# wangqiaoli/geometric_mapping

Measured on AMD Instinct MI355X. Metric: points/sec full segment+fit, 1M-pt synthetic tunnel frame, higher is better.
Workload: dtype f32; 1 GPU; 1000000-pt synthetic tunnel frame (R=2 m, L=12 m, sigma=0.01), rows resident in HBM; k_regime=fixed-k (~256 neighbours), mode=frames, frames_in_flight=4, GPU_MAX_HW_QUEUES=4, ransac_model=cylinder, H=1024, tau=0.03 (extension), parallelism=framesx1

## Files before the change

geometric_mapping_amd/_lib.py:

```python
from __future__ import annotations

import ctypes as C
import importlib.util
import os
import re

_HERE = os.path.dirname(os.path.abspath(__file__))
LIB_PATH = os.path.join(_HERE, "libgm_hip.so")
if os.environ.get("GM_LIB_PATH"):
    LIB_PATH = os.environ["GM_LIB_PATH"]
HEADER_PATH = os.path.join(os.path.dirname(_HERE), "include", "gm_hip.h")

GM_OK = 0
GM_ERR_INVALID_ARG = 1
GM_ERR_TOO_FEW_POINTS = 2
GM_ERR_DEVICE = 3
GM_ERR_OOM = 4
GM_ERR_CAPACITY = 5
GM_ERR_NOT_READY = 6
GM_ERR_UNSUPPORTED = 7
GM_ERR_COMM = 8
GM_GROUP_LOOPBACK = 1
GM_GROUP_N_TIMINGS = 5

# ... 236 lines not shown
    return C.CDLL(path, mode=C.RTLD_GLOBAL)


def load():
    global _lib
    if _lib is not None:
        return _lib
    _preload_hip_runtime()
    if not os.path.exists(LIB_PATH):
        raise FileNotFoundError(
            f"{LIB_PATH} is missing: build it with `python -c 'import __graft_entry__ as g; g.build()'` "
            "(make -C geometric_mapping_amd/csrc).  There is no CPU fallback.")
    L = C.CDLL(LIB_PATH)
    vp, u32, u32p, fp, dp, i32p, u8p = (C.c_void_p, C.c_uint32, C.POINTER(C.c_uint32), C.POINTER(C.c_float),
                                         C.POINTER(C.c_double), C.POINTER(C.c_int32), C.POINTER(C.c_uint8))
    cfgp, cloudp, resp = C.POINTER(Config), C.POINTER(Cloud), C.POINTER(FrameResult)
    fitp = C.POINTER(CylinderFit)
    sprmp, scellp, sinfop = C.POINTER(SurfaceParams), C.POINTER(SurfaceCell), C.POINTER(SurfaceInfo)
    wprmp, wrawp, waddp, winfop = C.POINTER(WallParams), C.POINTER(WallRawCell), C.POINTER(WallAddInfo), C.POINTER(WallInfo)
    u64, u64p = C.c_uint64, C.POINTER(C.c_uint64)
    wregp, wrprmp, wrinfop, wrmetp = (C.POINTER(WallRegion), C.POINTER(WallRegionParams), C.POINTER(WallRegionsInfo),
                                      C.POINTER(WallRegionMetrics))
    wcprmp, wcptp, wcinfop = C.POINTER(WallCloudParams), C.POINTER(WallCloudPoint), C.POINTER(WallCloudInfo)
    wkprmp, wkptp, wkinfop = C.POINTER(WallCheckParams), C.POINTER(WallCheckPoint), C.POINTER(WallCheckInfo)
    woprmp, wobjp, woinfop, wometp = (C.POINTER(WallObjectParams), C.POINTER(WallObject), C.POINTER(WallObjectsInfo),
                                      C.POINTER(WallObjectMetrics))
    proto = {
        "gm_create": (C.c_int, [cfgp, C.POINTER(vp)]),
        "gm_destroy": (None, [vp]),
        "gm_default_config": (None, [cfgp]),
        "gm_host_alloc": (C.c_int, [vp, C.c_size_t, C.POINTER(vp)]),
        "gm_host_free": (C.c_int, [vp, vp]),
        "gm_host_register": (C.c_int, [vp, vp, C.c_size_t]),
        "gm_host_unregister": (C.c_int, [vp, vp]),
        "gm_abi_version": (u32, []),
        "gm_debug_live_buffers": (C.c_longlong, []),
        "gm_status_string": (C.c_char_p, [C.c_int]),
        "gm_last_error": (C.c_char_p, [vp]),
        "gm_process_frame": (C.c_int, [vp, cloudp, resp]),
        "gm_submit_frame": (C.c_int, [vp, u32, cloudp]),
        "gm_wait_frame": (C.c_int, [vp, u32, resp]),
        "gm_poll_frame": (C.c_int, [vp, u32]),
        "gm_set_cloud_output": (C.c_int, [vp, u32, fp, u32]),
        "gm_get_cropped_xyz": (C.c_int, [vp, u32, fp, u32, u32p]),
        "gm_get_normals": (C.c_int, [vp, u32, fp, u32, u32p]),
        "gm_get_voxel_centroids": (C.c_int, [vp, u32, fp, u32, u32p]),
        "gm_get_voxel_nearest": (C.c_int, [vp, u32, i32p, u32, u32p]),
        "gm_get_voxel_normals": (C.c_int, [vp, u32, fp, u32, u32p]),
        "gm_get_neighbor_counts": (C.c_int, [vp, u32, i32p, u32, u32p]),
        "gm_get_labels": (C.c_int, [vp, u32, u8p, u32, u32p]),
        "gm_chop_cloud": (C.c_int, [vp, cloudp, C.c_double, fp, u32, u32p]),
        "gm_get_normals_stage": (C.c_int, [vp, fp, u32, C.c_double, fp, fp, u32, u32p]),
        "gm_get_local_frame": (C.c_int, [vp, fp, u32, C.c_double, fp, fp, dp]),
        "gm_voxel_grid": (C.c_int, [vp, fp, u32, C.c_double, fp, u32, u32p, u32p]),
        "gm_nearest": (C.c_int, [vp, fp, u32, fp, u32, i32p]),
        "gm_solve_local_frame": (C.c_int, [dp, fp, fp]),
        "gm_set_owned_range": (C.c_int, [vp, C.c_double, C.c_double]),
        "gm_ext_available": (C.c_int, []),
        "gm_score_frame": (C.c_int, [vp, u32, C.c_int, fp, u32, C.c_double, u32, i32p]),
        "gm_score_planes": (C.c_int, [vp, fp, u32, u8p, u32, fp, u32, C.c_double, i32p]),
        "gm_score_cylinders": (C.c_int, [vp, fp, u32, u8p, u32, fp, u32, C.c_double, i32p]),
        "gm_plane_hypotheses": (C.c_int, [vp, fp, u32, u8p, u32, C.c_uint64, u32, fp]),
        "gm_cylinder_hypotheses": (C.c_int, [vp, fp, fp, u32, u8p, u32, C.c_uint64, u32, fp]),
        "gm_segment_moments": (C.c_int, [vp, fp, fp, u8p, u32, u32, dp]),
        "gm_get_compressed_map": (C.c_int, [vp, u32, vp, C.c_size_t, C.POINTER(C.c_size_t)]),
        "gm_get_cylinder_fit": (C.c_int, [vp, u32, fitp]),
        "gm_fit_cylinder": (C.c_int, [vp, fp, u32, u8p, u32, fp, C.c_double, fitp, u8p]),
        "gm_surface_default_params": (None, [sprmp]),
        "gm_set_surface_params": (C.c_int, [vp, sprmp]),
        "gm_get_surface_map": (C.c_int, [vp, u32, sinfop, scellp, u32, u32p]),
        "gm_get_surface_points": (C.c_int, [vp, u32, fp, i32p, u32, u32p]),
        "gm_surface_map": (C.c_int, [vp, fp, u32, u8p, fp, sprmp, sinfop, scellp, u32, fp, i32p]),
        "gm_wall_default_params": (None, [wprmp]),
        "gm_wall_map_create": (C.c_int, [vp, wprmp, C.POINTER(vp)]),
        "gm_wall_map_destroy": (None, [vp]),
        "gm_wall_map_add_frame": (C.c_int, [vp, vp, u32, dp, waddp]),
        "gm_wall_map_add_points": (C.c_int, [vp, fp, u32, u8p, dp, waddp, fp, i32p]),
        "gm_wall_map_sync": (C.c_int, [vp]),
        "gm_wall_map_info": (C.c_int, [vp, winfop]),
        "gm_wall_map_read": (C.c_int, [vp, u32, u32, scellp, u64, u64p]),
        "gm_wall_map_read_raw": (C.c_int, [vp, u32, u32, wrawp, u64, u64p]),
        "gm_wall_map_add_raw": (C.c_int, [vp, u32, u32, wrawp]),
        "gm_wall_map_clear": (C.c_int, [vp, u32, u32]),
        "gm_wall_region_default_params": (None, [wrprmp]),
        "gm_wall_map_regions": (C.c_int, [vp, vp, u32, u32, wrprmp, wrinfop, wregp, u32, u32p, i32p]),
        "gm_wall_region_metrics": (C.c_int, [wprmp, wregp, wrmetp]),
        "gm_wall_cloud_default_params": (None, [wcprmp]),
        "gm_wall_cloud_directions": (C.c_int, [wprmp, wcprmp, dp, u32, u32p]),
        "gm_wall_map_cloud": (C.c_int, [vp, u32, u32, wcprmp, wcinfop, wcptp, u64, u64p]),
        "gm_wall_check_default_params": (None, [wkprmp]),
        "gm_wall_check_classify": (C.c_int, [wkprmp, wrawp, C.c_float, C.POINTER(C.c_int64), u32p]),
        "gm_wall_map_check_frame": (C.c_int, [vp, vp, u32, dp, wkprmp, waddp]),
        "gm_wall_map_get_check": (C.c_int, [vp, u32, wkinfop, wkptp, u32, u32p]),
        "gm_wall_map_check_points": (C.c_int, [vp, fp, u32, u8p, dp, wkprmp, waddp, wkinfop, wkptp, u32, u32p, fp, i32p, i32p, u8p]),
        "gm_wall_object_default_params": (None, [woprmp]),
        "gm_wall_map_check_objects": (C.c_int, [vp, u32, woprmp, woinfop, wobjp, u32, u32p, i32p, u32]),
        "gm_wall_check_objects": (C.c_int, [vp, wkptp, u32, C.c_int64, woprmp, woinfop, wobjp, u32, u32p, i32p]),
        "gm_wall_object_metrics": (C.c_int, [wprmp, woprmp, wobjp, wometp]),
        "gm_group_create": (C.c_int, [cfgp, i32p, u32, u32, C.POINTER(vp)]),
        "gm_group_destroy": (None, [vp]),
        "gm_group_size": (u32, [vp]),
        "gm_group_ctx": (vp, [vp, u32]),
        "gm_group_last_error": (C.c_char_p, [vp]),
        "gm_group_process_frame": (C.c_int, [vp, cloudp, resp]),
        "gm_group_get_cropped_xyz": (C.c_int, [vp, fp, u32, u32p]),
        "gm_group_get_voxel_centroids": (C.c_int, [vp, fp, u32, u32p]),
# ... 20 lines not shown
```

geometric_mapping_amd/api.py:

```python
from __future__ import annotations

import ctypes as C

import numpy as np

from . import _lib
from ._lib import (GM_CFG_CYLINDER_FIT, GM_CFG_DEFAULT, GM_CFG_KEEP_COUNTS, GM_CFG_STAGE_TIMING, GM_CFG_VOXEL_GRID,
                   GM_CLOUD_BIGENDIAN, GM_CLOUD_DEVICE, GM_CLOUD_PINNED, GM_ERR_CAPACITY, GM_ERR_NOT_READY, GM_OK, Cloud, Config,
                   CylinderFit, FrameResult, GmError, STAGE_NAMES)

__all__ = ["GeometricMapping", "GeometricMappingGroup", "WallMap", "GmError", "solve_local_frame", "decode_compressed_map",
           "GM_CFG_CYLINDER_FIT"]


def _f32(a):
    return a.ctypes.data_as(C.POINTER(C.c_float))


class GeometricMapping:

    def __init__(self, boxFilterBound=5.0, voxelGridLeafSize=0.5, neighborRadius=0.5, weightingFactor=0.2,
                 device=0, flags=GM_CFG_DEFAULT, n_slots=1, max_points=0,
                 ransac_hypotheses=1024, ransac_threshold=0.03, ransac_seed=1):
        self._L = _lib.load()
# ... 182 lines not shown

    def labels(self, slot=0):
        return self._fetch(self._L.gm_get_labels, slot, 1, np.uint8)

    def compressed_map(self, slot=0):
        n = C.c_size_t(0)
        st = self._L.gm_get_compressed_map(self._ctx, slot, None, 0, C.byref(n))
        if st not in (GM_OK, GM_ERR_CAPACITY):
            self._check(st)
        buf = np.zeros(n.value, dtype=np.uint8)
        self._check(self._L.gm_get_compressed_map(self._ctx, slot, buf.ctypes.data, n.value, C.byref(n)))
        return buf

    def set_owned_range(self, lo, hi):
        self._check(self._L.gm_set_owned_range(self._ctx, float(lo), float(hi)))

    def chopCloud(self, bound, cloud):
        c, keep = self._as_cloud(cloud)
        cap = max(c.n_points, 1)
        out = np.empty((cap, 4), dtype=np.float32)
        n = C.c_uint32(0)
        self._check(self._L.gm_chop_cloud(self._ctx, C.byref(c), float(bound), _f32(out), cap, C.byref(n)))
        out = out[:n.value]
        return out[:, :3].copy(), out[:, 3].copy().view(np.int32)

    def getNormals(self, neighborRadius, cloud):
        xyz = np.ascontiguousarray(cloud, dtype=np.float32)
        if xyz.ndim != 2 or xyz.shape[1] != 3:
            raise ValueError("cloud must be [n,3]")
        n0 = xyz.shape[0]
        cap = max(n0, 1)
        oc = np.empty((cap, 4), dtype=np.float32)
        on = np.empty((cap, 4), dtype=np.float32)
        n = C.c_uint32(0)
        self._check(self._L.gm_get_normals_stage(self._ctx, _f32(xyz), n0, float(neighborRadius), _f32(oc), _f32(on),
                                                 cap, C.byref(n)))
        oc, on = oc[:n.value], on[:n.value]
        return on.copy(), oc[:, :3].copy(), oc[:, 3].copy().view(np.int32)

    def getLocalFrame(self, cloudSize, weightingFactor, cloud_normals):
        nrm = np.ascontiguousarray(cloud_normals, dtype=np.float32)
        if nrm.ndim != 2 or nrm.shape[1] != 4:
            raise ValueError("normals must be [n,4] (nx,ny,nz,curvature)")
        if cloudSize > nrm.shape[0]:
            raise ValueError("cloudSize exceeds the normals cloud (the reference's .at() would throw)")
        ev = np.zeros(3, dtype=np.float32)
        V = np.zeros(9, dtype=np.float32)
        sc = np.zeros(6, dtype=np.float64)
        self._check(self._L.gm_get_local_frame(self._ctx, _f32(nrm), int(cloudSize), float(weightingFactor), _f32(ev),
                                               _f32(V), sc.ctypes.data_as(C.POINTER(C.c_double))))
        M = np.array([[sc[0], sc[1], sc[2]], [sc[1], sc[3], sc[4]], [sc[2], sc[4], sc[5]]])
        return ev, V.reshape(3, 3).T.copy(), M

    def voxelGrid(self, leafSize, cloud):
        xyz = np.ascontiguousarray(cloud, dtype=np.float32)
        if xyz.ndim != 2 or xyz.shape[1] != 3:
            raise ValueError("cloud must be [n,3]")
        cap = max(xyz.shape[0], 1)
        out = np.empty((cap, 4), dtype=np.float32)
        n = C.c_uint32(0)
        fl = C.c_uint32(0)
        self._check(self._L.gm_voxel_grid(self._ctx, _f32(xyz), xyz.shape[0], float(leafSize), _f32(out), cap,
                                          C.byref(n), C.byref(fl)))
        out = out[:n.value]
        return out[:, :3].copy(), out[:, 3].astype(np.int32), bool(fl.value & _lib.GM_RES_VOXEL_PASSTHROUGH)


    @staticmethod
    def _u8(a):
        if a is None:
            return None, None
        a = np.ascontiguousarray(a, dtype=np.uint8)
        return a, a.ctypes.data_as(C.POINTER(C.c_uint8))

    def nearest(self, cloud, queries):
        xyz = np.ascontiguousarray(cloud, dtype=np.float32)
        q = np.ascontiguousarray(queries, dtype=np.float32)
        idx = np.empty(max(len(q), 1), dtype=np.int32)
        self._check(self._L.gm_nearest(self._ctx, _f32(xyz), len(xyz), _f32(q), len(q),
                                       idx.ctypes.data_as(C.POINTER(C.c_int32))))
        return idx[:len(q)].copy()

    def plane_hypotheses(self, cloud, seed, H, labels=None, want=0):
        xyz = np.ascontiguousarray(cloud, dtype=np.float32)
        lab, lp = self._u8(labels)
        out = np.empty((H, 4), dtype=np.float32)
        self._check(self._L.gm_plane_hypotheses(self._ctx, _f32(xyz), len(xyz), lp, want, seed, H, _f32(out)))
        return out

    def cylinder_hypotheses(self, cloud, normals, seed, H, labels=None, want=0):
        xyz = np.ascontiguousarray(cloud, dtype=np.float32)
        nrm = np.ascontiguousarray(normals, dtype=np.float32)
        lab, lp = self._u8(labels)
        out = np.empty((H, 7), dtype=np.float32)
        self._check(self._L.gm_cylinder_hypotheses(self._ctx, _f32(xyz), _f32(nrm), len(xyz), lp, want, seed, H, _f32(out)))
        return out

    def _score(self, fn, cloud, hyp, tau, labels, want):
        xyz = np.ascontiguousarray(cloud, dtype=np.float32)
        hyp = np.ascontiguousarray(hyp, dtype=np.float32)
        lab, lp = self._u8(labels)
        cnt = np.zeros(len(hyp), dtype=np.int32)
        self._check(fn(self._ctx, _f32(xyz), len(xyz), lp, want, _f32(hyp), len(hyp), float(tau),
                       cnt.ctypes.data_as(C.POINTER(C.c_int32))))
        return cnt

# ... 693 lines not shown
```

geometric_mapping_amd/csrc/gm_api.hip:

```cpp
#include <math.h>
#include <stdlib.h>
#include <string.h>

#include <limits>
#include <new>

#include "gm_compact.hpp"
#include "gm_internal.hpp"

using namespace gm;

namespace {

thread_local std::string g_create_err;

#define GM_HIP(ctx, call)                                                                 \
    do {                                                                                  \
        hipError_t e__ = (call);                                                          \
        if (e__ != hipSuccess) {                                                          \
            (ctx)->err = std::string(#call) + ": " + hipGetErrorString(e__);              \
            return (e__ == hipErrorOutOfMemory) ? GM_ERR_OOM : GM_ERR_DEVICE;             \
        }                                                                                 \
    } while (0)

// ... 104 lines not shown
    const double dim = b - a + 1.0;
    if (std::isfinite(dim) && dim >= 1.0 && dim * dim * dim <= (double)kVoxDenseMaxCells && fabs(a) < 1e9) {
        vd.enabled = 1;
        vd.i_lo = (int32_t)a;
        vd.dim = (int32_t)dim;
        const double ext = fmax((double)hi - (double)lo, 1e-30);
        int k = (int)floor(log2(9.0e18 / (ext * 268435456.0)));
        if (k > 40) k = 40;
        if (k < 8 || n_cap > 268435456u) { vd.enabled = 0; k = 0; }
        vd.scale = ldexp(1.0, k);
        vd.inv_scale = ldexp(1.0, -k);
    }
    return vd;
}

int bits_for(uint64_t count)
{
    int b = 1;
    while ((1ull << b) < count && b < 32) ++b;
    return b;
}

int voxel_key_bits(double lo, double hi, double leaf)
{
    const float inv = 1.0f / (float)leaf;
    double d = floor((double)((float)hi * inv)) - floor((double)((float)lo * inv)) + 2.0;
    if (!(d > 0) || !std::isfinite(d)) return 32;
    double prod = d * d * d;
    if (prod > 2147483647.0) return 32;
    return bits_for((uint64_t)prod);
}

gm_status ensure_capacity(gm_ctx *ctx, Slot &sl, uint32_t n, size_t raw_bytes, bool need_raw)
{
    uint32_t *gen = &sl.alloc_gen;
    if (need_raw && raw_bytes > sl.raw_cap) {
        const size_t cap = raw_bytes + raw_bytes / 4 + 4096;
        sl.raw_cap = 0;
        GM_HIP(ctx, sl.h_raw.reserve(cap));
        GM_HIP(ctx, sl.d_raw.reserve(cap));
        sl.raw_cap = cap;
    }
    if (n <= sl.cap) return GM_OK;
    GM_HIP(ctx, hipStreamSynchronize(sl.stream));
    uint32_t cap = n + n / 4 + 1024;
    if (cap < ctx->cfg.max_points) cap = ctx->cfg.max_points;
    cap = (cap + 3u) & ~3u;
    sl.cap = 0;
    GM_HIP(ctx, sl.crop4.reserve(cap, gen));
    GM_HIP(ctx, sl.keys_a.reserve(cap, gen)); GM_HIP(ctx, sl.keys_b.reserve(cap, gen));
    GM_HIP(ctx, sl.vals_a.reserve(cap, gen)); GM_HIP(ctx, sl.vals_b.reserve(cap, gen));
    GM_HIP(ctx, sl.spts4.reserve(cap, gen)); GM_HIP(ctx, sl.normals4.reserve(cap, gen));
    GM_HIP(ctx, sl.counts.reserve(cap, gen));
    GM_HIP(ctx, sl.valid4.reserve(cap, gen)); GM_HIP(ctx, sl.vnorm4.reserve(cap, gen));
    GM_HIP(ctx, sl.seg_start.reserve(cap, gen)); GM_HIP(ctx, sl.vox4.reserve(cap, gen));
    GM_HIP(ctx, sl.vox_nn.reserve(cap, gen)); GM_HIP(ctx, sl.labels.reserve(cap, gen)); GM_HIP(ctx, sl.inl_mask.reserve(cap, gen));
    sl.tiles_cap = cap + 2u;
    sl.tile_seg = cap / 2u + 2u;
    GM_HIP(ctx, sl.tiles.reserve((size_t)(kTileListClasses - 1) * sl.tile_seg + sl.tiles_cap, gen));
    GM_HIP(ctx, sl.row_bounds.reserve((size_t)1024 * 1024, gen));
    sl.blk_cap = compact_records(cap > kVoxDenseMaxCells ? cap : kVoxDenseMaxCells) + 1;
    GM_HIP(ctx, sl.tile_partials.reserve((size_t)compact_blocks(cap) * 6, gen));
    GM_HIP(ctx, sl.blk.reserve((size_t)sl.blk_cap + 1, gen));
    GM_HIP(ctx, hipMemsetAsync(sl.blk, 0, sizeof(unsigned long long) * ((size_t)sl.blk_cap + 1), sl.stream));
    {
        static const char *e = getenv("GM_TEST_SCAN_EPOCH");
        sl.scan_epoch = e ? (uint32_t)strtoul(e, nullptr, 0) : 0u;
    }
    GM_HIP(ctx, sl.sort.totals.reserve(radix_totals_bytes() / sizeof(uint32_t), gen));
    sl.sort.rec_words = (radix_record_words_max(cap) + 1u) & ~(size_t)1u;
    GM_HIP(ctx, sl.sort.rec.reserve(sl.sort.rec_words, gen));
    GM_HIP(ctx, sl.sort.ticket.reserve(4, gen));
    GM_HIP(ctx, hipMemsetAsync(sl.sort.ticket, 0, 16, sl.stream));
    sl.tile_rec_words = (size_t)(tile_cutter_blocks(cap) + 1) * (size_t)kTileListClasses;
    GM_HIP(ctx, sl.tile_rec.reserve(sl.tile_rec_words, gen));
    GM_HIP(ctx, hipMemsetAsync(sl.tile_rec, 0, sizeof(unsigned long long) * sl.tile_rec_words, sl.stream));
    sl.cap = cap;
    return GM_OK;
}

gm_status check_layout(gm_ctx *ctx, const gm_cloud *c)
{
    const uint64_t step = c->point_step;
    if (c->n_points && (step < 12 || (uint64_t)c->off_x + 4 > step || (uint64_t)c->off_y + 4 > step ||
                        (uint64_t)c->off_z + 4 > step))
        return fail(ctx, GM_ERR_INVALID_ARG, "gm_cloud: x/y/z offsets do not fit in point_step");
    return GM_OK;
}

gm_status make_rows(gm_ctx *ctx, const gm_cloud *c, const uint8_t *dev_data, RowLayout &rows)
{
    const gm_status lst = check_layout(ctx, c);
    if (lst != GM_OK) return lst;
    memset(&rows, 0, sizeof(rows));
    rows.data = dev_data;
    rows.step = c->point_step; rows.ox = c->off_x; rows.oy = c->off_y; rows.oz = c->off_z;
    rows.bswap = (c->flags & GM_CLOUD_BIGENDIAN) ? 1u : 0u;
    const bool al4 = ((c->point_step | c->off_x | c->off_y | c->off_z) & 3u) == 0 && (((uintptr_t)dev_data) & 3u) == 0;
    const bool al16 = al4 && c->point_step == 16 && c->off_x == 0 && c->off_y == 4 && c->off_z == 8 &&
                      (((uintptr_t)dev_data) & 15u) == 0;
    rows.mode = al16 ? 0u : (al4 ? 1u : 2u);
    return GM_OK;
}

void record(gm_ctx *ctx, Slot &sl, int idx)
{
    if (ctx->cfg.flags & GM_CFG_STAGE_TIMING) hipEventRecord(sl.ev[idx], sl.stream);
}

gm_status reset_counters(gm_ctx *ctx, Slot &sl)
{
    GM_HIP(ctx, hipMemsetAsync(sl.ctr, 0, sizeof(DevCounters), sl.stream));
    return GM_OK;
}

// ... 12 lines not shown
    return hipSuccess;
}

static uint32_t size_bucket(uint32_t n)
{
    if (n == 0) return 0;
    uint32_t p2 = 1024;
    while (p2 < n && p2 < 0x80000000u) p2 <<= 1;
    const uint32_t step = p2 / 16 < 1024u ? 1024u : p2 / 16;
    const uint64_t b = ((uint64_t)n + step - 1) / step * step;
    return b > 0xFFFFFFFFull ? 0xFFFFFFFFu : (uint32_t)b;
}

static gm_status enqueue_launches(gm_ctx *ctx, Slot &sl, const RowLayout &rows, uint32_t n, uint32_t ns, const GridParams &g,
                                  const VoxDense &vd, float lo, float hi)
{
    const gm_config &cf = ctx->cfg;
    hipStream_t s = sl.stream;
    const uint32_t *n_dev = nullptr;
    if (sl.capturing) {
        sl.scan_seq = 0;
        GM_HIP(ctx, hipMemcpyAsync(sl.frame_in, sl.h_frame_in, 4 * sizeof(uint32_t), hipMemcpyHostToDevice, s));
        n_dev = sl.frame_in;
    }
    {
        ZeroJobs z;
        memset(&z, 0, sizeof(z));
        z.ptr[0] = sl.ctr; z.words8[0] = sizeof(DevCounters) / 8;
        if (vd.enabled) { z.ptr[1] = sl.vox_table; z.words8[1] = (uint64_t)vd.dim * vd.dim * vd.dim * sizeof(VoxCell) / 8; }
        if (sl.row_bounds) { z.ptr[2] = sl.row_bounds; z.words8[2] = (uint64_t)g.ny * (uint64_t)g.nz; }
        if (sl.sort.totals) {
            z.ptr[3] = sl.sort.totals; z.words8[3] = radix_totals_bytes() / 8;
            z.ptr[4] = sl.sort.rec; z.words8[4] = (radix_record_words(ns, cell_key_bits(g)) + 1) / 2;
        }
        z.frame_counter = sl.frame_in + 4;
        launch_zero_fill(z, s);
    }
    launch_crop(rows, n, lo, hi, g, sl, s, ns, n_dev, true);
    const bool cloud_overlap = sl.cloud_out && n && !sl.capturing && sl.cloud_out_dev;
    if (cloud_overlap) {
        GM_HIP(ctx, hipEventRecord(sl.ev_crop, s));
        GM_HIP(ctx, hipStreamWaitEvent(sl.copy_stream, sl.ev_crop, 0));
        GM_HIP(ctx, hipMemcpyAsync(sl.cloud_out, sl.crop4, (size_t)n * sizeof(float4), hipMemcpyDeviceToHost, sl.copy_stream));
    }
    record(ctx, sl, 2);
    launch_grid_and_normals(g, vd, sl, ns, (cf.flags & GM_CFG_KEEP_COUNTS) != 0, true, s);
    record(ctx, sl, 3);
    uint32_t row_tile = kCpTile;
    const uint32_t nparts = launch_compact_valid(sl, ns, cf.weightingFactor, s, &row_tile);
    bool cloud_copy_pending = false;
    if (cloud_overlap) {
        GM_HIP(ctx, hipEventRecord(sl.ev_valid, s));
        GM_HIP(ctx, hipStreamWaitEvent(sl.copy_stream, sl.ev_valid, 0));
        launch_rows_to_host(sl.valid4, sl.cloud_out_dev, &sl.ctr->first_drop_enc, &sl.ctr->n_valid, sl.copy_stream);
        GM_HIP(ctx, hipEventRecord(sl.ev_copied, sl.copy_stream));
        cloud_copy_pending = true;
    } else if (sl.cloud_out && n) {
        const size_t frozen = (size_t)(ns < sl.cloud_out_cap ? ns : sl.cloud_out_cap) * sizeof(float4);
        GM_HIP(ctx, hipMemcpyAsync(sl.cloud_out, sl.valid4, frozen, hipMemcpyDeviceToHost, s));
    }
    record(ctx, sl, 4);
    record(ctx, sl, 5);
    sl.vox_sort_path = (cf.flags & GM_CFG_VOXEL_GRID) && !vd.enabled;
    if (cf.flags & GM_CFG_VOXEL_GRID) {
        if (vd.enabled) {
            launch_voxel_dense_finalize(vd, sl, s);
        } else {
            launch_minmax(sl.valid4, &sl.ctr->n_valid, ns, sl.ctr, s);
            launch_voxel_grid(sl, ns, (float)cf.voxelGridLeafSize, voxel_key_bits(lo, hi, cf.voxelGridLeafSize), s);
        }
    }
    record(ctx, sl, 6);
    if (cf.flags & (GM_CFG_RANSAC_PLANE | GM_CFG_RANSAC_CYLINDER)) {
        const gm_status st = gm_enqueue_ransac(ctx, sl, ns, nparts, row_tile);
        if (st != GM_OK) return st;
    }
    if ((cf.flags & GM_CFG_NEAREST) && (cf.flags & GM_CFG_VOXEL_GRID)) {
        const uint32_t nq_cap = vd.enabled ? (uint32_t)vd.dim * vd.dim * vd.dim : ns;
        launch_nearest(sl.valid4, &sl.ctr->n_valid, ns, sl.vox4, &sl.ctr->n_voxels, nq_cap < ns ? nq_cap : ns, sl.nn_best,
                       sl.vox_nn, s, sl.vnorm4, sl.vox_nrm4);
    }
    record(ctx, sl, 7);
    if (!(cf.flags & (GM_CFG_RANSAC_PLANE | GM_CFG_RANSAC_CYLINDER)))
        launch_frame_finalize(sl.tile_partials, nparts, row_tile, sl, s);
    if (cloud_copy_pending) GM_HIP(ctx, hipStreamWaitEvent(s, sl.ev_copied, 0));
    GM_HIP(ctx, hipMemcpyAsync(sl.h_out, sl.d_out, sizeof(FrameOut), hipMemcpyDeviceToHost, s));
    return GM_OK;
}

gm_status enqueue_frame(gm_ctx *ctx, Slot &sl, const gm_cloud *cloud, bool blocking_call)
{
    const uint32_t n = cloud->n_points;
    const uint32_t ns = size_bucket(n);
    const size_t raw_bytes = (size_t)n * cloud->point_step;
    const bool on_dev = (cloud->flags & GM_CLOUD_DEVICE) != 0;
    if (n && !cloud->data) return fail(ctx, GM_ERR_INVALID_ARG, "gm_cloud.data is NULL");
    if (sl.cloud_out && n > sl.cloud_out_cap) return fail(ctx, GM_ERR_CAPACITY, "gm_set_cloud_output: the frame has more points than the cloud buffer has rows");
    gm_status st = check_layout(ctx, cloud);
    if (st != GM_OK) return st;
    st = ensure_capacity(ctx, sl, ns ? ns : 1u, raw_bytes, !on_dev);
    if (st != GM_OK) return st;
    if (ctx->cfg.flags & (GM_CFG_RANSAC_PLANE | GM_CFG_RANSAC_CYLINDER | GM_CFG_NEAREST)) {
        st = gm_ensure_ext(ctx, sl, ctx->cfg.ransac_hypotheses ? ctx->cfg.ransac_hypotheses : 1);
        if (st != GM_OK) return st;
    }
    if (ctx->cfg.flags & GM_CFG_SURFACE_MAP) {
        st = gm_ensure_surface(ctx, sl);
        if (st != GM_OK) return st;
    }
    hipStream_t s = sl.stream;
    sl.n_in = n;
    if ((++sl.frames_enqueued & 0x7FFFFFu) == 0u && sl.blk) {
        GM_HIP(ctx, hipMemsetAsync(sl.blk, 0, sizeof(unsigned long long) * (size_t)sl.blk_cap, s));
        GM_HIP(ctx, hipMemsetAsync(sl.tile_rec, 0, sizeof(unsigned long long) * sl.tile_rec_words, s));
    }
    record(ctx, sl, 0);
    const uint8_t *dev_rows = (const uint8_t *)cloud->data;
    if (!on_dev && n) {
        static const char *zc = getenv("GM_PINNED_ZERO_COPY");
        const int zmode = zc ? atoi(zc) : 0;
        void *mapped = nullptr;
        if ((cloud->flags & GM_CLOUD_PINNED) && (zmode == 2 || (zmode == 1 && blocking_call)) &&
            hipHostGetDevicePointer(&mapped, const_cast<void *>(cloud->data), 0) == hipSuccess && mapped) {
            dev_rows = (const uint8_t *)mapped;
        } else {
            (void)hipGetLastError();
            GM_HIP(ctx, upload_rows(sl, cloud, raw_bytes, blocking_call, s));
            dev_rows = sl.d_raw;
        }
    }
    record(ctx, sl, 1);
    RowLayout rows;
    st = make_rows(ctx, cloud, dev_rows, rows);
// ... 184 lines not shown
    GM_HIP(ctx, sl.score_partial.reserve(4096, gen));
    GM_HIP(ctx, sl.cnt_plane.reserve(HH, gen)); GM_HIP(ctx, sl.cnt_cyl.reserve(HH, gen));
    GM_HIP(ctx, sl.best_plane.reserve(2, gen)); GM_HIP(ctx, sl.best_cyl.reserve(2, gen));
    GM_HIP(ctx, sl.mom_partial.reserve((size_t)kScatterBlocks * 16 * 2, gen));
    GM_HIP(ctx, sl.mom_plane.reserve(16, gen)); GM_HIP(ctx, sl.mom_cyl.reserve(16, gen));
    GM_HIP(ctx, sl.nn_best.reserve(pts, gen));
    GM_HIP(ctx, sl.vox_nrm4.reserve(pts, gen));
    GM_HIP(ctx, sl.fit_partial.reserve((size_t)kFitBlocks * 24, gen)); GM_HIP(ctx, sl.fit_ticket.reserve(1, gen));
    GM_HIP(ctx, sl.fit_work.reserve(1, gen)); GM_HIP(ctx, sl.fit_init.reserve(8, gen)); GM_HIP(ctx, sl.fit_stage.reserve(1, gen));
    GM_HIP(ctx, hipMemset(sl.fit_ticket, 0, sizeof(uint32_t)));
    GM_HIP(ctx, hipMemset(sl.score_partial, 0, sizeof(uint32_t) * 4096));
    GM_HIP(ctx, hipMemset(sl.best_plane, 0xFF, 8));
    GM_HIP(ctx, hipMemset(sl.best_cyl, 0xFF, 8));
    sl.ext_H = HH; sl.ext_cap = sl.cap;
    return GM_OK;
}

gm_status gm_ensure_surface(gm_ctx *ctx, Slot &sl)
{
    uint32_t *gen = &sl.alloc_gen;
    if (!sl.surf_table) {
        GM_HIP(ctx, hipStreamSynchronize(sl.stream));
        GM_HIP(ctx, sl.surf_prm.reserve(2, gen)); GM_HIP(ctx, sl.surf_cells.reserve(GM_SURF_MAX_CELLS, gen));
        GM_HIP(ctx, sl.surf_info.reserve(1, gen)); GM_HIP(ctx, sl.surf_fit.reserve(1, gen));
        GM_HIP(ctx, hipMemsetAsync(sl.surf_info, 0, sizeof(gm_surface_info), sl.stream));
        const SurfParams prm[2] = {surface_device_params(ctx->surf), surface_device_params(ctx->surf)};
        GM_HIP(ctx, hipMemcpyAsync(sl.surf_prm, prm, sizeof(prm), hipMemcpyHostToDevice, sl.stream));
        GM_HIP(ctx, sl.surf_table.reserve(surface_table_bytes(), gen));
        GM_HIP(ctx, hipMemsetAsync(sl.surf_table, 0, surface_table_bytes(), sl.stream));
        GM_HIP(ctx, hipStreamSynchronize(sl.stream));
    }
    if (sl.surf_cap < sl.cap || !sl.surf_res) {
        GM_HIP(ctx, hipStreamSynchronize(sl.stream));
        const uint32_t pts = sl.cap ? sl.cap : 1u;
        sl.surf_cap = 0;
        GM_HIP(ctx, sl.surf_res.reserve(pts, gen)); GM_HIP(ctx, sl.surf_cell.reserve(pts, gen));
        sl.surf_cap = sl.cap;
    }
    return GM_OK;
}

gm_status gm_enqueue_ransac(gm_ctx *ctx, Slot &sl, uint32_t n_cap, uint32_t scatter_rows, uint32_t row_tile)
{
    const gm_config &cf = ctx->cfg;
    const bool do_plane = (cf.flags & GM_CFG_RANSAC_PLANE) != 0, do_cyl = (cf.flags & GM_CFG_RANSAC_CYLINDER) != 0;
    if (!do_plane && !do_cyl) return GM_OK;
    const uint32_t H = cf.ransac_hypotheses;
    hipStream_t s = sl.stream;
    const uint32_t *n_ptr = &sl.ctr->n_valid;
    bool first = true;
    uint32_t mom_rows = 0;
    if (do_plane) {
        uint8_t *lab = first ? nullptr : sl.labels;
        launch_plane_hypotheses(sl.valid4, lab, 0, n_ptr, n_cap, cf.ransac_seed, H, sl.hyp_plane, sl.cnt_plane, s);
        const uint32_t *fsel = nullptr; const int32_t *fcnt = nullptr; uint32_t fk = 0; bool fmask = false, frep = false;
        launch_score_preemptive(0, sl.valid4, lab, 0, n_ptr, n_cap, sl.hyp_plane, sl.band, H, cf.ransac_threshold,
                                sl.score_partial, sl.cnt_plane, sl.best_plane, true, &fsel, &fcnt, &fk, s, sl.inl_mask, &fmask, &frep);
        mom_rows = launch_label(0, sl.valid4, sl.labels, 0, 1, n_ptr, n_cap, sl.hyp_plane, sl.band, sl.best_plane,
                                cf.ransac_threshold, first ? 1 : 0, fsel, fcnt, fk, s, sl.vnorm4, sl.mom_partial, fmask ? sl.inl_mask : nullptr, frep);
        first = false;
    }
    if (do_cyl) {
        uint8_t *lab = first ? nullptr : sl.labels;
        launch_cylinder_hypotheses(sl.valid4, sl.vnorm4, lab, 0, n_ptr, n_cap, cf.ransac_seed + 1, H, sl.hyp_cyl,
                                   sl.cnt_cyl, sl.band, cf.ransac_threshold, s);
        const uint32_t *fsel = nullptr; const int32_t *fcnt = nullptr; uint32_t fk = 0; bool fmask = false, frep = false;
        launch_score_preemptive(1, sl.valid4, lab, 0, n_ptr, n_cap, sl.hyp_cyl, sl.band, H, cf.ransac_threshold,
                                sl.score_partial, sl.cnt_cyl, sl.best_cyl, true, &fsel, &fcnt, &fk, s, sl.inl_mask, &fmask, &frep);
        mom_rows = launch_label(1, sl.valid4, sl.labels, 0, 2, n_ptr, n_cap, sl.hyp_cyl, sl.band, sl.best_cyl,
                                cf.ransac_threshold, first ? 1 : 0, fsel, fcnt, fk, s, sl.vnorm4, sl.mom_partial, fmask ? sl.inl_mask : nullptr, frep);
        first = false;
        if (cf.flags & GM_CFG_CYLINDER_FIT) {
            CylFitArgs a;
            a.pts = sl.valid4; a.labels = sl.labels; a.out = sl.labels;
            a.want = 0; a.want2 = 2; a.mask_mode = 0;
            a.n_ptr = n_ptr; a.n_host = n_cap;
            a.init = sl.hyp_cyl; a.best = sl.best_cyl;
            a.work = sl.fit_work; a.fit = &sl.d_out->fit; a.partial = sl.fit_partial; a.ticket = sl.fit_ticket;
            a.tau = cf.ransac_threshold;
            launch_cylinder_fit(a, s);
            if (cf.flags & GM_CFG_SURFACE_MAP) {
                SurfArgs m;
                m.pts = sl.valid4; m.labels = sl.labels; m.n_ptr = n_ptr; m.n_host = n_cap;
                m.fit = &sl.d_out->fit; m.prm = sl.surf_prm;
                m.table = sl.surf_table; m.cells = sl.surf_cells; m.info = sl.surf_info; m.res = sl.surf_res; m.cell = sl.surf_cell;
                launch_surface_map(m, n_cap, s);
            }
        }
    }
    launch_ext_finalize(sl.hyp_plane, do_plane ? sl.best_plane : nullptr, sl.hyp_cyl, do_cyl ? sl.best_cyl : nullptr,
                        sl.mom_plane, sl.mom_cyl, &sl.d_out->ext, sl.mom_partial, mom_rows, s, sl.tile_partials, scatter_rows, row_tile,
                        sl.ctr, sl.voxp, sl.d_out);
    return GM_OK;
}

}

extern "C" {

int gm_debug_graph_captures(gm_ctx *ctx, uint32_t slot)
{
    if (!ctx || slot >= ctx->n_slots) return -1;
    return (int)ctx->slots[slot].graph_captures;
}

long long gm_debug_live_buffers(void) { return g_live_buffers.load(std::memory_order_relaxed); }

gm_status gm_host_alloc(gm_ctx *ctx, size_t bytes, void **out)
{
    if (!ctx || !out) return fail(ctx, GM_ERR_INVALID_ARG, "gm_host_alloc: NULL argument");
    *out = nullptr;
    if (hipSetDevice(ctx->cfg.device) != hipSuccess) return fail(ctx, GM_ERR_DEVICE, "hipSetDevice failed");
    if (hipHostMalloc(out, bytes ? bytes : 1, hipHostMallocDefault) != hipSuccess) {
        *out = nullptr;
        return fail(ctx, GM_ERR_OOM, "gm_host_alloc: hipHostMalloc failed");
    }
    return GM_OK;
}

gm_status gm_host_free(gm_ctx *ctx, void *ptr)
{
    if (!ptr) return GM_OK;
    if (hipHostFree(ptr) != hipSuccess) return fail(ctx, GM_ERR_INVALID_ARG, "gm_host_free: not a gm_host_alloc pointer");
    return GM_OK;
}

gm_status gm_host_register(gm_ctx *ctx, void *ptr, size_t bytes)
{
    if (!ctx || !ptr || !bytes) return fail(ctx, GM_ERR_INVALID_ARG, "gm_host_register: NULL argument");
    if (hipSetDevice(ctx->cfg.device) != hipSuccess) return fail(ctx, GM_ERR_DEVICE, "hipSetDevice failed");
    if (hipHostRegister(ptr, bytes, hipHostRegisterDefault) != hipSuccess) {
        (void)hipGetLastError();
        return fail(ctx, GM_ERR_INVALID_ARG, "gm_host_register: hipHostRegister failed (already registered, or not host memory)");
    }
    return GM_OK;
}
// ... 193 lines not shown
    if (!sl.submitted) return GM_ERR_NOT_READY;
    if (sl.complete) return GM_OK;
    if (hipSetDevice(ctx->device) != hipSuccess) return fail(ctx, GM_ERR_DEVICE, "hipSetDevice failed");
    const hipError_t e = hipStreamQuery(sl.stream);
    if (e == hipSuccess) return GM_OK;
    if (e == hipErrorNotReady) { (void)hipGetLastError(); return GM_ERR_NOT_READY; }
    ctx->err = std::string("hipStreamQuery: ") + hipGetErrorString(e);
    return GM_ERR_DEVICE;
}

gm_status gm_set_cloud_output(gm_ctx *ctx, uint32_t slot, float *xyzw, uint32_t capacity)
{
    if (!ctx) return GM_ERR_INVALID_ARG;
    if (slot >= ctx->n_slots) return fail(ctx, GM_ERR_INVALID_ARG, "slot out of range");
    if (hipSetDevice(ctx->device) != hipSuccess) return fail(ctx, GM_ERR_DEVICE, "hipSetDevice failed");
    Slot &sl = ctx->slots[slot];
    if (sl.submitted && !sl.complete) GM_HIP(ctx, hipStreamSynchronize(sl.stream));
    if (xyzw) {
        hipPointerAttribute_t a;
        if (hipPointerGetAttributes(&a, xyzw) != hipSuccess || a.type != hipMemoryTypeHost) {
            (void)hipGetLastError();
            return fail(ctx, GM_ERR_INVALID_ARG, "gm_set_cloud_output: the buffer must be page-locked (gm_host_alloc / gm_host_register)");
        }
    }
    if (xyzw && !sl.copy_stream) {
        GM_HIP(ctx, hipStreamCreateWithFlags(&sl.copy_stream, hipStreamNonBlocking));
        GM_HIP(ctx, hipEventCreateWithFlags(&sl.ev_crop, hipEventDisableTiming));
        GM_HIP(ctx, hipEventCreateWithFlags(&sl.ev_valid, hipEventDisableTiming));
        GM_HIP(ctx, hipEventCreateWithFlags(&sl.ev_copied, hipEventDisableTiming));
    }
    sl.cloud_out_dev = nullptr;
    if (xyzw) {
        void *dp = nullptr;
        if (hipHostGetDevicePointer(&dp, xyzw, 0) == hipSuccess) sl.cloud_out_dev = reinterpret_cast<float4 *>(dp);
        else (void)hipGetLastError();
    }
    sl.cloud_out = reinterpret_cast<float4 *>(xyzw);
    sl.cloud_out_cap = xyzw ? capacity : 0u;
    return GM_OK;
}

gm_status gm_process_frame(gm_ctx *ctx, const gm_cloud *cloud, gm_frame_result *res)
{
    gm_status st = submit(ctx, 0, cloud, true);
    if (st != GM_OK) return st;
    return gm_wait_frame(ctx, 0, res);
}

gm_status gm_get_cropped_xyz(gm_ctx *ctx, uint32_t slot, float *xyzw, uint32_t capacity, uint32_t *n_out)
{
    gm_status st = check_slot(ctx, slot);
    if (st != GM_OK) return st;
    Slot &sl = ctx->slots[slot];
    return fetch(ctx, slot, (const float4 *)sl.valid4, sl.last.n_valid, (float4 *)xyzw, capacity, n_out);
}

gm_status gm_get_normals(gm_ctx *ctx, uint32_t slot, float *nxyzc, uint32_t capacity, uint32_t *n_out)
{
    gm_status st = check_slot(ctx, slot);
    if (st != GM_OK) return st;
    Slot &sl = ctx->slots[slot];
    return fetch(ctx, slot, (const float4 *)sl.vnorm4, sl.last.n_valid, (float4 *)nxyzc, capacity, n_out);
}

gm_status gm_get_voxel_centroids(gm_ctx *ctx, uint32_t slot, float *xyzc, uint32_t capacity, uint32_t *n_out)
{
    gm_status st = check_slot(ctx, slot);
    if (st != GM_OK) return st;
    Slot &sl = ctx->slots[slot];
    if (!(ctx->cfg.flags & GM_CFG_VOXEL_GRID)) return fail(ctx, GM_ERR_NOT_READY, "context created without GM_CFG_VOXEL_GRID");
    return fetch(ctx, slot, (const float4 *)sl.vox4, sl.last.n_voxels, (float4 *)xyzc, capacity, n_out);
}

gm_status gm_get_neighbor_counts(gm_ctx *ctx, uint32_t slot, int32_t *counts, uint32_t capacity, uint32_t *n_out)
{
    gm_status st = check_slot(ctx, slot);
    if (st != GM_OK) return st;
    Slot &sl = ctx->slots[slot];
    if (!(ctx->cfg.flags & GM_CFG_KEEP_COUNTS)) return fail(ctx, GM_ERR_NOT_READY, "context created without GM_CFG_KEEP_COUNTS");
    return fetch(ctx, slot, (const int32_t *)sl.counts, sl.last.n_cropped, counts, capacity, n_out);
}


gm_status gm_chop_cloud(gm_ctx *ctx, const gm_cloud *cloud, double bound, float *xyzw_out, uint32_t capacity,
                        uint32_t *n_out)
{
    Slot *slp;
    gm_status st = begin_stage(ctx, slp);
    if (st != GM_OK) return st;
    if (!cloud) return fail(ctx, GM_ERR_INVALID_ARG, "cloud is NULL");
    if (!std::isfinite(bound) || bound < 0) return fail(ctx, GM_ERR_INVALID_ARG, "bound must be finite and >= 0");
    Slot &sl = *slp;
    const uint32_t n = cloud->n_points;
    const size_t raw_bytes = (size_t)n * cloud->point_step;
    const bool on_dev = (cloud->flags & GM_CLOUD_DEVICE) != 0;
    if (n && !cloud->data) return fail(ctx, GM_ERR_INVALID_ARG, "gm_cloud.data is NULL");
    st = check_layout(ctx, cloud);
    if (st != GM_OK) return st;
    st = ensure_capacity(ctx, sl, n ? n : 1u, raw_bytes, !on_dev);
    if (st != GM_OK) return st;
    st = reset_counters(ctx, sl);
    if (st != GM_OK) return st;
    const uint8_t *dev_rows = (const uint8_t *)cloud->data;
    if (!on_dev && n) {
        GM_HIP(ctx, upload_rows(sl, cloud, raw_bytes, true, sl.stream));
        dev_rows = sl.d_raw;
    }
    RowLayout rows;
    st = make_rows(ctx, cloud, dev_rows, rows);
    if (st != GM_OK) return st;
    const float lo = (float)(-bound), hi = (float)bound;
    const GridParams g = make_grid(lo, lo, lo, hi - lo, hi - lo, hi - lo, ctx->cfg.neighborRadius, n);
    launch_crop(rows, n, lo, hi, g, sl, sl.stream);
    uint32_t m = 0;
    GM_HIP(ctx, hipMemcpyAsync(&m, &sl.ctr->n_cropped, 4, hipMemcpyDeviceToHost, sl.stream));
    GM_HIP(ctx, hipStreamSynchronize(sl.stream));
    return fetch(ctx, 0, (const float4 *)sl.crop4, m, (float4 *)xyzw_out, capacity, n_out);
}

gm_status gm_get_normals_stage(gm_ctx *ctx, const float *xyz, uint32_t n, double radius, float *xyzw_out,
                               float *nxyzc_out, uint32_t capacity, uint32_t *n_out)
{
    Slot *slp;
    gm_status st = begin_stage(ctx, slp);
    if (st != GM_OK) return st;
    if (n && !xyz) return fail(ctx, GM_ERR_INVALID_ARG, "xyz is NULL");
    if (!radius_ok(radius)) return fail(ctx, GM_ERR_INVALID_ARG, "radius must be 0 or within [1e-15, 1e15]");
    Slot &sl = *slp;
    const size_t raw_bytes = (size_t)n * 12;
    st = ensure_capacity(ctx, sl, n, raw_bytes, true);
    if (st != GM_OK) return st;
    st = reset_counters(ctx, sl);
    if (st != GM_OK) return st;
    float mn[3] = {3e38f, 3e38f, 3e38f}, mx[3] = {-3e38f, -3e38f, -3e38f};
    for (uint32_t i = 0; i < n; ++i) {
        const float *p = xyz + 3 * (size_t)i;
        if (!(std::isfinite(p[0]) && std::isfinite(p[1]) && std::isfinite(p[2]))) continue;
        for (int k = 0; k < 3; ++k) { mn[k] = fminf(mn[k], p[k]); mx[k] = fmaxf(mx[k], p[k]); }
    }
    if (mn[0] > mx[0]) { for (int k = 0; k < 3; ++k) { mn[k] = 0; mx[k] = 0; } }
    if (n) {
        memcpy(sl.h_raw, xyz, raw_bytes);
        GM_HIP(ctx, hipMemcpyAsync(sl.d_raw, sl.h_raw, raw_bytes, hipMemcpyHostToDevice, sl.stream));
    }
    gm_cloud c = {sl.d_raw, n, 12, 0, 4, 8, GM_CLOUD_DEVICE};
    RowLayout rows;
    st = make_rows(ctx, &c, sl.d_raw, rows);
    if (st != GM_OK) return st;
    const GridParams g = make_grid(mn[0], mn[1], mn[2], mx[0] - mn[0], mx[1] - mn[1], mx[2] - mn[2], radius, n);
    const float big = std::numeric_limits<float>::max();
    launch_crop(rows, n, -big, big, g, sl, sl.stream);
    VoxDense vd_off;
    memset(&vd_off, 0, sizeof(vd_off));
    vd_off.own_lo = -std::numeric_limits<float>::infinity();
    vd_off.own_hi = std::numeric_limits<float>::infinity();
    launch_grid_and_normals(g, vd_off, sl, n, (ctx->cfg.flags & GM_CFG_KEEP_COUNTS) != 0, false, sl.stream);
    launch_compact_valid(sl, n, 1.0, sl.stream);
    uint32_t m[2] = {0, 0};
    GM_HIP(ctx, hipMemcpyAsync(m, &sl.ctr->n_cropped, 8, hipMemcpyDeviceToHost, sl.stream));
    GM_HIP(ctx, hipStreamSynchronize(sl.stream));
    GM_HIP(ctx, hipGetLastError());
    sl.last.n_cropped = m[0];
    sl.last.n_valid = m[1];
    sl.submitted = true;
    sl.complete = true;
    st = fetch(ctx, 0, (const float4 *)sl.valid4, m[1], (float4 *)xyzw_out, capacity, n_out);
    if (st != GM_OK) return st;
    return fetch(ctx, 0, (const float4 *)sl.vnorm4, m[1], (float4 *)nxyzc_out, capacity, n_out);
}

gm_status gm_get_local_frame(gm_ctx *ctx, const float *nxyzc, uint32_t n, double wf, float eigenvalues[3],
                             float eigenvectors[9], double scatter6[6])
{
    Slot *slp;
    gm_status st = begin_stage(ctx, slp);
    if (st != GM_OK) return st;
    if (n && !nxyzc) return fail(ctx, GM_ERR_INVALID_ARG, "normals pointer is NULL");
    if (!(wf != 0.0)) return fail(ctx, GM_ERR_INVALID_ARG, "weighting factor must be non-zero");
    Slot &sl = *slp;
    st = ensure_capacity(ctx, sl, n, 0, false);
    if (st != GM_OK) return st;
    st = reset_counters(ctx, sl);
    if (st != GM_OK) return st;
    if (n) GM_HIP(ctx, hipMemcpyAsync(sl.vnorm4, nxyzc, (size_t)n * 16, hipMemcpyHostToDevice, sl.stream));
    const uint32_t np = launch_scatter_partials(sl.vnorm4, nullptr, n, wf, sl, sl.stream);
    launch_frame_finalize(sl.partials, np, 0, sl, sl.stream);
    GM_HIP(ctx, hipMemcpyAsync(sl.h_out, sl.d_out, sizeof(FrameOut), hipMemcpyDeviceToHost, sl.stream));
    GM_HIP(ctx, hipStreamSynchronize(sl.stream));
    GM_HIP(ctx, hipGetLastError());
    if (eigenvalues) for (int k = 0; k < 3; ++k) eigenvalues[k] = sl.h_out->evals[k];
    if (eigenvectors) for (int k = 0; k < 9; ++k) eigenvectors[k] = sl.h_out->evecs[k];
    if (scatter6) for (int k = 0; k < 6; ++k) scatter6[k] = sl.h_out->scatter[k];
    return GM_OK;
}

gm_status gm_voxel_grid(gm_ctx *ctx, const float *xyz, uint32_t n, double leaf, float *xyzc_out, uint32_t capacity,
                        uint32_t *n_out, uint32_t *status_flags)
{
    Slot *slp;
    gm_status st = begin_stage(ctx, slp);
    if (st != GM_OK) return st;
    if (n && !xyz) return fail(ctx, GM_ERR_INVALID_ARG, "xyz is NULL");
    if (!(leaf > 0.0) || !std::isfinite(leaf)) return fail(ctx, GM_ERR_INVALID_ARG, "leaf must be finite and > 0");
    Slot &sl = *slp;
    st = ensure_capacity(ctx, sl, n, (size_t)n * 16, true);
    if (st != GM_OK) return st;
    st = reset_counters(ctx, sl);
    if (st != GM_OK) return st;
    float mn = 3e38f, mx = -3e38f;
    float4 *stage = (float4 *)sl.h_raw.p;
    for (uint32_t i = 0; i < n; ++i) {
        const float *p = xyz + 3 * (size_t)i;
        stage[i] = make_float4(p[0], p[1], p[2], 0.f);
        for (int k = 0; k < 3; ++k) { mn = fminf(mn, p[k]); mx = fmaxf(mx, p[k]); }
    }
    if (n) GM_HIP(ctx, hipMemcpyAsync(sl.valid4, stage, (size_t)n * 16, hipMemcpyHostToDevice, sl.stream));
    GM_HIP(ctx, hipMemcpyAsync(&sl.ctr->vox_n, &n, 4, hipMemcpyHostToDevice, sl.stream));
    launch_minmax(sl.valid4, nullptr, n, sl.ctr, sl.stream);
    launch_voxel_grid(sl, n, (float)leaf, n ? voxel_key_bits(mn, mx, leaf) : 1, sl.stream);
    uint32_t V = 0, pass = 0;
    GM_HIP(ctx, hipMemcpyAsync(&V, &sl.ctr->n_voxels, 4, hipMemcpyDeviceToHost, sl.stream));
    GM_HIP(ctx, hipMemcpyAsync(&pass, &sl.voxp->passthrough, 4, hipMemcpyDeviceToHost, sl.stream));
    GM_HIP(ctx, hipStreamSynchronize(sl.stream));
    GM_HIP(ctx, hipGetLastError());
    if (status_flags) *status_flags = pass ? GM_RES_VOXEL_PASSTHROUGH : 0u;
    return fetch(ctx, 0, (const float4 *)sl.vox4, V, (float4 *)xyzc_out, capacity, n_out);
}

gm_status gm_solve_local_frame(const double scatter6[6], float eigenvalues[3], float eigenvectors[9])
{
    if (!scatter6 || !eigenvalues || !eigenvectors) return GM_ERR_INVALID_ARG;
    double w[3], V[9];
    eig3_sym_eigen_signs(scatter6, w, V);
    for (int k = 0; k < 3; ++k) eigenvalues[k] = (float)w[k];
    for (int k = 0; k < 9; ++k) eigenvectors[k] = (float)V[k];
    return GM_OK;
}

}
```

geometric_mapping_amd/csrc/gm_compact.hpp:

```cpp
#pragma once

#include "gm_device.hpp"

namespace gm {

struct NoPayload {};

#ifndef GM_CPTHREADS
#define GM_CPTHREADS 512
#endif
constexpr int kCpThreads = GM_CPTHREADS;
#ifndef GM_CPITEMS
#define GM_CPITEMS 8
#endif
constexpr int kCpItems = GM_CPITEMS;
constexpr int kCpTile = kCpThreads * kCpItems;
constexpr int kCpWaves = kCpThreads / kWave;

inline uint32_t compact_blocks(uint32_t n) { return (n + kCpTile - 1) / kCpTile; }
constexpr int kCpMinTile = 2048;
inline uint32_t compact_records(uint32_t n) { return (n + kCpMinTile - 1) / kCpMinTile; }
inline uint32_t compact_grid(uint32_t n) { return compact_blocks(n); }

template <class Pred, class Emit, int THREADS = kCpThreads, int ITEMS = kCpItems>
__global__ __launch_bounds__(THREADS) void k_compact(Pred pred, Emit emit, const uint32_t *__restrict__ n_ptr,
                                                            uint32_t n_host, ScanState st,
                                                            uint32_t *__restrict__ total_out,
                                                            uint32_t *__restrict__ total_out2)
{
    static_assert(THREADS * ITEMS >= kCpMinTile, "tile below the size the record arrays are laid out for");
    constexpr uint64_t kAggregate = 1ull << 32, kInclusive = 2ull << 32;
    __shared__ uint32_t lb_sum[(THREADS / kWave)], lb_state[(THREADS / kWave)];
    __shared__ uint32_t wcnt[(THREADS / kWave)];
    const uint32_t n = n_ptr ? *n_ptr : n_host;
    const uint32_t ntiles = (n + (uint32_t)(THREADS * ITEMS) - 1u) / (uint32_t)(THREADS * ITEMS);
    const int w = threadIdx.x / kWave, lane = lane_id();
    const uint32_t epoch = scan_epoch(st);
    const uint64_t tag = (uint64_t)epoch << 34;
    if (n == 0) {
        if (blockIdx.x == 0 && threadIdx.x == 0) {
            if (total_out) *total_out = 0;
            if (total_out2) *total_out2 = 0;
        }
        return;
    }
    __shared__ uint32_t s_tile;
    if constexpr (Emit::kHasPrepare) emit.prepare();
#ifdef GM_CP_DIAG_NOTICKET
    if (threadIdx.x == 0) s_tile = blockIdx.x;
#else
    if (threadIdx.x == 0) {
        const uint32_t t = atomicAdd(st.ticket, 1u);
        if (t == gridDim.x - 1) atomicExch(st.ticket, 0u);
        s_tile = t;
    }
#endif
    __syncthreads();
    const uint32_t tile = s_tile;
    if (tile < ntiles) {
        const uint32_t base = tile * (uint32_t)(THREADS * ITEMS);
        uint64_t mask[ITEMS];
        typename Pred::Payload pay[ITEMS];
        const uint32_t wbase = base + (uint32_t)w * (uint32_t)(kWave * ITEMS);
        uint32_t wtotal = 0;
#pragma unroll
        for (int j = 0; j < ITEMS; ++j) {
            const uint32_t i = wbase + j * kWave + lane;
            const bool v = (i < n) && pred(i, pay[j]);
            mask[j] = __ballot(v);
            wtotal += (uint32_t)__popcll(mask[j]);
        }
        if (lane == 0) wcnt[w] = wtotal;
        __syncthreads();
        uint32_t total = 0, woff = 0;
#pragma unroll
        for (int k = 0; k < (THREADS / kWave); ++k) {
            const uint32_t c = wcnt[k];
            if (k < w) woff += c;
            total += c;
        }
        if (threadIdx.x == 0)
            __hip_atomic_store(&st.status[tile], tag | (tile == 0 ? kInclusive : kAggregate) | total, __ATOMIC_RELAXED,
                               __HIP_MEMORY_SCOPE_AGENT);
        uint32_t before = 0;
#ifdef GM_CP_DIAG_NOLOOKBACK
        before = base;
        if (false) {
#else
        if (tile > 0) {
#endif
            int32_t top = (int32_t)tile - 1;
            for (;;) {
                const int32_t idx = top - (int32_t)threadIdx.x;
                const uint64_t sv = idx >= 0 ? __hip_atomic_load(&st.status[idx], __ATOMIC_RELAXED, __HIP_MEMORY_SCOPE_AGENT)
                                             : (tag | kInclusive);
                const bool ready = (sv >> 34) == (uint64_t)epoch && ((sv >> 32) & 3u) != 0u;
                const bool incl = ready && ((sv >> 32) & 3u) == 2u;
                const uint64_t im = __ballot(incl), rm = __ballot(ready);
                const int first = im ? (int)__builtin_ctzll(im) : kWave;
                const uint64_t need = first >= kWave - 1 ? ~0ull : ((2ull << first) - 1ull);
                const uint32_t part = wave_sum(lane <= first ? (uint32_t)sv : 0u);
                __syncthreads();
                if (lane == 0) { lb_sum[w] = part; lb_state[w] = ((rm & need) != need) ? 2u : (im ? 1u : 0u); }
                __syncthreads();
                uint32_t acc = 0;
                bool retry = false, done = false;
#pragma unroll
                for (int k = 0; k < (THREADS / kWave); ++k) {
                    if (!done && !retry) {
                        if (lb_state[k] == 2u) retry = true;
                        else { acc += lb_sum[k]; done = lb_state[k] == 1u; }
                    }
                }
                if (retry) { __builtin_amdgcn_s_sleep(2); continue; }
                before += acc;
                if (done) break;
                top -= THREADS;
            }
            if (threadIdx.x == 0)
                __hip_atomic_store(&st.status[tile], tag | kInclusive | (uint64_t)(before + total), __ATOMIC_RELAXED,
                                   __HIP_MEMORY_SCOPE_AGENT);
        }
        if (threadIdx.x == 0 && tile == ntiles - 1) {
#ifdef GM_CP_DIAG_NOLOOKBACK
            if (total_out) *total_out = 0;
            if (total_out2) *total_out2 = 0;
#else
            if (total_out) *total_out = before + total;
            if (total_out2) *total_out2 = before + total;
#endif
        }
        uint32_t running = before + woff;
#pragma unroll
        for (int j = 0; j < ITEMS; ++j) {
            const uint32_t i = wbase + j * kWave + lane;
            if ((mask[j] >> lane) & 1ull) emit(i, running + (uint32_t)__popcll(mask[j] & lanemask_lt()), pay[j]);
            running += (uint32_t)__popcll(mask[j]);
        }
        if constexpr (Emit::kHasFinish) emit.finish(tile);
    }
}

}
```

geometric_mapping_amd/csrc/gm_ext.hip:

```cpp
#include <math.h>
#include <string.h>

#include <vector>

#include "gm_internal.hpp"

using namespace gm;

namespace {

#define GMX_HIP(ctx, call)                                                           \
    do {                                                                             \
        hipError_t e__ = (call);                                                     \
        if (e__ != hipSuccess) {                                                     \
            (ctx)->err = std::string(#call) + ": " + hipGetErrorString(e__);         \
            return (e__ == hipErrorOutOfMemory) ? GM_ERR_OOM : GM_ERR_DEVICE;        \
        }                                                                            \
    } while (0)

gm_status upload_xyz(gm_ctx *ctx, Slot &sl, const float *xyz, uint32_t n, float4 *dst)
{
    if (!n) return GM_OK;
    float4 *stage = (float4 *)sl.h_raw.p;
    for (uint32_t i = 0; i < n; ++i) stage[i] = make_float4(xyz[3 * (size_t)i], xyz[3 * (size_t)i + 1], xyz[3 * (size_t)i + 2], 0.f);
    GMX_HIP(ctx, hipMemcpyAsync(dst, stage, (size_t)n * 16, hipMemcpyHostToDevice, sl.stream));
    GMX_HIP(ctx, hipStreamSynchronize(sl.stream));
    return GM_OK;
}

gm_status prepare(gm_ctx *ctx, Slot *&sl, uint32_t n, uint32_t H)
{
    gm_status st = gm_begin_stage(ctx, sl);
    if (st != GM_OK) return st;
    st = gm_ensure_capacity(ctx, *sl, n, (size_t)n * 16, true);
    if (st != GM_OK) return st;
    return gm_ensure_ext(ctx, *sl, H ? H : 1);
}

gm_status upload_labels(gm_ctx *ctx, Slot &sl, const uint8_t *labels, uint32_t n)
{
    if (labels && n) GMX_HIP(ctx, hipMemcpyAsync(sl.labels, labels, n, hipMemcpyHostToDevice, sl.stream));
    return GM_OK;
}

gm_status score(gm_ctx *ctx, int model, const float *xyz, uint32_t n, const uint8_t *labels, uint32_t want,
                const float *hyp, uint32_t H, double tau, int32_t *counts)
{
    Slot *slp;
    if (!ctx) return GM_ERR_INVALID_ARG;
    if ((n && !xyz) || !hyp || !counts) return gm_fail(ctx, GM_ERR_INVALID_ARG, "NULL argument");
    gm_status st = prepare(ctx, slp, n, H);
    if (st != GM_OK) return st;
    Slot &sl = *slp;
    st = upload_xyz(ctx, sl, xyz, n, sl.valid4);
    if (st != GM_OK) return st;
    st = upload_labels(ctx, sl, labels, n);
    if (st != GM_OK) return st;
    const int w = model == 0 ? 4 : 7;
    float *stage = (float *)sl.h_raw.p;
    if ((size_t)H * 32 > sl.raw_cap) {
        st = gm_ensure_capacity(ctx, sl, n, (size_t)H * 32, true);
        if (st != GM_OK) return st;
        stage = (float *)sl.h_raw.p;
    }
    memset(stage, 0, (size_t)H * 32);
    for (uint32_t h = 0; h < H; ++h)
        for (int k = 0; k < w; ++k) stage[8 * (size_t)h + k] = hyp[(size_t)w * h + k];
    float *dh = model == 0 ? sl.hyp_plane : sl.hyp_cyl;
    GMX_HIP(ctx, hipMemcpyAsync(dh, stage, (size_t)H * 32, hipMemcpyHostToDevice, sl.stream));
    launch_score(model, sl.valid4, labels ? sl.labels : nullptr, want, nullptr, n, dh, sl.band, H, tau, sl.score_partial,
                 sl.cnt_plane, sl.best_plane, sl.stream);
    GMX_HIP(ctx, hipMemcpyAsync(counts, sl.cnt_plane, (size_t)H * 4, hipMemcpyDeviceToHost, sl.stream));
    GMX_HIP(ctx, hipStreamSynchronize(sl.stream));
    GMX_HIP(ctx, hipGetLastError());
    return GM_OK;
}

}

namespace gm {
gm_status gm_upload_xyz(gm_ctx *ctx, Slot &sl, const float *xyz, uint32_t n, float4 *dst) { return upload_xyz(ctx, sl, xyz, n, dst); }
}

extern "C" {

int gm_ext_available(void) { return 1; }

gm_status gm_score_planes(gm_ctx *ctx, const float *xyz, uint32_t n, const uint8_t *labels, uint32_t want,
                          const float *hyp4, uint32_t H, double tau, int32_t *counts)
{
    return score(ctx, 0, xyz, n, labels, want, hyp4, H, tau, counts);
}

gm_status gm_score_cylinders(gm_ctx *ctx, const float *xyz, uint32_t n, const uint8_t *labels, uint32_t want,
                             const float *hyp7, uint32_t H, double tau, int32_t *counts)
{
    return score(ctx, 1, xyz, n, labels, want, hyp7, H, tau, counts);
}

gm_status gm_score_frame(gm_ctx *ctx, uint32_t slot, int model, const float *hyp, uint32_t H, double tau,
                         uint32_t unlabelled_only, int32_t *counts)
{
    gm_status st = gm_check_slot(ctx, slot);
    if (st != GM_OK) return st;
    if (!hyp || !counts || (model != 0 && model != 1)) return gm_fail(ctx, GM_ERR_INVALID_ARG, "gm_score_frame: bad argument");
    if (unlabelled_only && !(ctx->cfg.flags & (GM_CFG_RANSAC_PLANE | GM_CFG_RANSAC_CYLINDER)))
        return gm_fail(ctx, GM_ERR_NOT_READY, "unlabelled_only needs a context created with a GM_CFG_RANSAC_* flag");
    Slot &sl = ctx->slots[slot];
    st = gm_ensure_ext(ctx, sl, H);
    if (st != GM_OK) return st;
    const int w = model == 0 ? 4 : 7;
    std::vector<float> rows((size_t)H * 8, 0.f);
    for (uint32_t h = 0; h < H; ++h)
        for (int k = 0; k < w; ++k) rows[8 * (size_t)h + k] = hyp[(size_t)w * h + k];
    float *dh = model == 0 ? sl.hyp_plane : sl.hyp_cyl;
    GMX_HIP(ctx, hipMemcpyAsync(dh, rows.data(), rows.size() * 4, hipMemcpyHostToDevice, sl.stream));
    GMX_HIP(ctx, hipStreamSynchronize(sl.stream));
    launch_score(model, sl.valid4, unlabelled_only ? sl.labels : nullptr, 0, &sl.ctr->n_valid, sl.last.n_valid, dh, sl.band,
                 H, tau, nullptr, sl.cnt_plane, sl.score_partial + 600, sl.stream);
    GMX_HIP(ctx, hipMemcpyAsync(counts, sl.cnt_plane, (size_t)H * 4, hipMemcpyDeviceToHost, sl.stream));
    GMX_HIP(ctx, hipStreamSynchronize(sl.stream));
    GMX_HIP(ctx, hipGetLastError());
    return GM_OK;
}

gm_status gm_plane_hypotheses(gm_ctx *ctx, const float *xyz, uint32_t n, const uint8_t *labels, uint32_t want,
                              uint64_t seed, uint32_t H, float *hyp4)
{
    Slot *slp;
    if (!ctx) return GM_ERR_INVALID_ARG;
    if ((n && !xyz) || !hyp4) return gm_fail(ctx, GM_ERR_INVALID_ARG, "NULL argument");
    gm_status st = prepare(ctx, slp, n, H);
    if (st != GM_OK) return st;
    Slot &sl = *slp;
    st = upload_xyz(ctx, sl, xyz, n, sl.valid4);
    if (st != GM_OK) return st;
    st = upload_labels(ctx, sl, labels, n);
    if (st != GM_OK) return st;
    launch_plane_hypotheses(sl.valid4, labels ? sl.labels : nullptr, want, nullptr, n, seed, H, sl.hyp_plane, nullptr,
                            sl.stream);
    if ((size_t)H * 32 > sl.raw_cap) {
        st = gm_ensure_capacity(ctx, sl, n, (size_t)H * 32, true);
        if (st != GM_OK) return st;
    }
    float *stage = (float *)sl.h_raw.p;
    GMX_HIP(ctx, hipMemcpyAsync(stage, sl.hyp_plane, (size_t)H * 32, hipMemcpyDeviceToHost, sl.stream));
    GMX_HIP(ctx, hipStreamSynchronize(sl.stream));
    GMX_HIP(ctx, hipGetLastError());
    for (uint32_t h = 0; h < H; ++h)
        for (int k = 0; k < 4; ++k) hyp4[4 * (size_t)h + k] = stage[8 * (size_t)h + k];
    return GM_OK;
}

gm_status gm_cylinder_hypotheses(gm_ctx *ctx, const float *xyz, const float *nxyzc, uint32_t n, const uint8_t *labels,
                                 uint32_t want, uint64_t seed, uint32_t H, float *hyp7)
{
    Slot *slp;
    if (!ctx) return GM_ERR_INVALID_ARG;
    if ((n && (!xyz || !nxyzc)) || !hyp7) return gm_fail(ctx, GM_ERR_INVALID_ARG, "NULL argument");
    gm_status st = prepare(ctx, slp, n, H);
    if (st != GM_OK) return st;
    Slot &sl = *slp;
    st = upload_xyz(ctx, sl, xyz, n, sl.valid4);
    if (st != GM_OK) return st;
    if (n) GMX_HIP(ctx, hipMemcpyAsync(sl.vnorm4, nxyzc, (size_t)n * 16, hipMemcpyHostToDevice, sl.stream));
    st = upload_labels(ctx, sl, labels, n);
    if (st != GM_OK) return st;
    launch_cylinder_hypotheses(sl.valid4, sl.vnorm4, labels ? sl.labels : nullptr, want, nullptr, n, seed, H, sl.hyp_cyl,
                               nullptr, nullptr, 0.0, sl.stream);
    if ((size_t)H * 32 > sl.raw_cap) {
        st = gm_ensure_capacity(ctx, sl, n, (size_t)H * 32, true);
        if (st != GM_OK) return st;
    }
    float *stage = (float *)sl.h_raw.p;
    GMX_HIP(ctx, hipMemcpyAsync(stage, sl.hyp_cyl, (size_t)H * 32, hipMemcpyDeviceToHost, sl.stream));
    GMX_HIP(ctx, hipStreamSynchronize(sl.stream));
    GMX_HIP(ctx, hipGetLastError());
    for (uint32_t h = 0; h < H; ++h)
        for (int k = 0; k < 7; ++k) hyp7[7 * (size_t)h + k] = stage[8 * (size_t)h + k];
    return GM_OK;
}

gm_status gm_segment_moments(gm_ctx *ctx, const float *xyz, const float *nxyzc, const uint8_t *labels, uint32_t n,
                             uint32_t label, double mom16[16])
{
    Slot *slp;
    if (!ctx) return GM_ERR_INVALID_ARG;
    if ((n && !xyz) || !mom16) return gm_fail(ctx, GM_ERR_INVALID_ARG, "NULL argument");
    gm_status st = prepare(ctx, slp, n, 1);
    if (st != GM_OK) return st;
    Slot &sl = *slp;
    st = upload_xyz(ctx, sl, xyz, n, sl.valid4);
    if (st != GM_OK) return st;
    if (n && nxyzc) GMX_HIP(ctx, hipMemcpyAsync(sl.vnorm4, nxyzc, (size_t)n * 16, hipMemcpyHostToDevice, sl.stream));
    st = upload_labels(ctx, sl, labels, n);
    if (st != GM_OK) return st;
    launch_segment_moments(sl.valid4, nxyzc ? sl.vnorm4 : nullptr, labels ? sl.labels : nullptr, label, nullptr, n,
                           sl.mom_partial, sl.mom_plane, sl.stream);
    GMX_HIP(ctx, hipMemcpyAsync(mom16, sl.mom_plane, 16 * sizeof(double), hipMemcpyDeviceToHost, sl.stream));
    GMX_HIP(ctx, hipStreamSynchronize(sl.stream));
    GMX_HIP(ctx, hipGetLastError());
    return GM_OK;
}

gm_status gm_nearest(gm_ctx *ctx, const float *xyz, uint32_t n, const float *queries, uint32_t nq, int32_t *idx_out)
{
    Slot *slp;
    if (!ctx) return GM_ERR_INVALID_ARG;
    if ((n && !xyz) || (nq && (!queries || !idx_out))) return gm_fail(ctx, GM_ERR_INVALID_ARG, "NULL argument");
    const uint32_t m = n > nq ? n : nq;
    gm_status st = prepare(ctx, slp, m, 1);
    if (st != GM_OK) return st;
    Slot &sl = *slp;
    st = upload_xyz(ctx, sl, xyz, n, sl.valid4);
    if (st != GM_OK) return st;
    st = upload_xyz(ctx, sl, queries, nq, sl.vox4);
    if (st != GM_OK) return st;
    launch_nearest(sl.valid4, nullptr, n, sl.vox4, nullptr, nq, sl.nn_best, sl.vox_nn, sl.stream);
    if (nq) GMX_HIP(ctx, hipMemcpyAsync(idx_out, sl.vox_nn, (size_t)nq * 4, hipMemcpyDeviceToHost, sl.stream));
    GMX_HIP(ctx, hipStreamSynchronize(sl.stream));
    GMX_HIP(ctx, hipGetLastError());
    return GM_OK;
}

static gm_status fetch_bytes(gm_ctx *ctx, Slot &sl, const void *dev, uint32_t avail, size_t elem, void *out,
                             uint32_t capacity, uint32_t *n_out)
{
    if (n_out) *n_out = avail;
    if (avail > capacity) return gm_fail(ctx, GM_ERR_CAPACITY, "output buffer too small");
    if (!avail) return GM_OK;
    if (!out) return gm_fail(ctx, GM_ERR_INVALID_ARG, "output pointer is NULL");
    GMX_HIP(ctx, hipMemcpyAsync(out, dev, (size_t)avail * elem, hipMemcpyDeviceToHost, sl.stream));
    GMX_HIP(ctx, hipStreamSynchronize(sl.stream));
    return GM_OK;
}

gm_status gm_get_voxel_nearest(gm_ctx *ctx, uint32_t slot, int32_t *idx, uint32_t capacity, uint32_t *n_out)
{
    gm_status st = gm_check_slot(ctx, slot);
    if (st != GM_OK) return st;
    if ((ctx->cfg.flags & (GM_CFG_NEAREST | GM_CFG_VOXEL_GRID)) != (GM_CFG_NEAREST | GM_CFG_VOXEL_GRID))
        return gm_fail(ctx, GM_ERR_NOT_READY, "context created without GM_CFG_NEAREST | GM_CFG_VOXEL_GRID");
    Slot &sl = ctx->slots[slot];
    return fetch_bytes(ctx, sl, sl.vox_nn, sl.last.n_voxels, 4, idx, capacity, n_out);
}

gm_status gm_get_voxel_normals(gm_ctx *ctx, uint32_t slot, float *nxyzc, uint32_t capacity, uint32_t *n_out)
{
    gm_status st = gm_check_slot(ctx, slot);
    if (st != GM_OK) return st;
    if ((ctx->cfg.flags & (GM_CFG_NEAREST | GM_CFG_VOXEL_GRID)) != (GM_CFG_NEAREST | GM_CFG_VOXEL_GRID))
        return gm_fail(ctx, GM_ERR_NOT_READY, "context created without GM_CFG_NEAREST | GM_CFG_VOXEL_GRID");
    Slot &sl = ctx->slots[slot];
    return fetch_bytes(ctx, sl, sl.vox_nrm4, sl.last.n_voxels, 16, nxyzc, capacity, n_out);
}

gm_status gm_get_labels(gm_ctx *ctx, uint32_t slot, uint8_t *labels, uint32_t capacity, uint32_t *n_out)
{
    gm_status st = gm_check_slot(ctx, slot);
    if (st != GM_OK) return st;
    if (!(ctx->cfg.flags & (GM_CFG_RANSAC_PLANE | GM_CFG_RANSAC_CYLINDER)))
        return gm_fail(ctx, GM_ERR_NOT_READY, "context created without a GM_CFG_RANSAC_* flag");
    Slot &sl = ctx->slots[slot];
    return fetch_bytes(ctx, sl, sl.labels, sl.last.n_valid, 1, labels, capacity, n_out);
}

gm_status gm_get_cylinder_fit(gm_ctx *ctx, uint32_t slot, gm_cylinder_fit *out)
{
    if (!ctx) return GM_ERR_INVALID_ARG;
    if (!(ctx->cfg.flags & GM_CFG_CYLINDER_FIT))
        return gm_fail(ctx, GM_ERR_UNSUPPORTED, "gm_get_cylinder_fit: context created without GM_CFG_CYLINDER_FIT");
    gm_status st = gm_check_slot(ctx, slot);
    if (st != GM_OK) return st;
    if (!out) return gm_fail(ctx, GM_ERR_INVALID_ARG, "gm_get_cylinder_fit: NULL argument");
    *out = ctx->slots[slot].last_fit;
    return GM_OK;
}

gm_status gm_fit_cylinder(gm_ctx *ctx, const float *xyz, uint32_t n, const uint8_t *labels, uint32_t want,
                          const float init7[7], double tau, gm_cylinder_fit *out, uint8_t *inlier_out)
{
    Slot *slp;
    if (!ctx) return GM_ERR_INVALID_ARG;
    if ((n && !xyz) || !init7 || !out) return gm_fail(ctx, GM_ERR_INVALID_ARG, "gm_fit_cylinder: NULL argument");
    if (!(tau > 0.0) || !isfinite(tau)) return gm_fail(ctx, GM_ERR_INVALID_ARG, "gm_fit_cylinder: tau must be > 0");
    gm_status st = prepare(ctx, slp, n, 1);
    if (st != GM_OK) return st;
    Slot &sl = *slp;
    st = upload_xyz(ctx, sl, xyz, n, sl.valid4);
    if (st != GM_OK) return st;
    st = upload_labels(ctx, sl, labels, n);
    if (st != GM_OK) return st;
    float row[8] = {0, 0, 0, 0, 0, 0, 0, 0};
    for (int k = 0; k < 7; ++k) row[k] = init7[k];
    GMX_HIP(ctx, hipMemcpyAsync(sl.fit_init, row, sizeof(row), hipMemcpyHostToDevice, sl.stream));
    if (n) GMX_HIP(ctx, hipMemsetAsync(sl.inl_mask, 0, n, sl.stream));
    CylFitArgs a;
    a.pts = sl.valid4; a.labels = labels ? sl.labels : nullptr; a.out = sl.inl_mask;
    a.want = want; a.want2 = want; a.mask_mode = 1;
    a.n_ptr = nullptr; a.n_host = n;
    a.init = sl.fit_init; a.best = nullptr;
    a.work = sl.fit_work; a.fit = sl.fit_stage; a.partial = sl.fit_partial; a.ticket = sl.fit_ticket;
    a.tau = tau;
    launch_cylinder_fit(a, sl.stream);
    gm_cylinder_fit f;
    GMX_HIP(ctx, hipMemcpyAsync(&f, sl.fit_stage, sizeof(f), hipMemcpyDeviceToHost, sl.stream));
    if (inlier_out && n) GMX_HIP(ctx, hipMemcpyAsync(inlier_out, sl.inl_mask, n, hipMemcpyDeviceToHost, sl.stream));
    GMX_HIP(ctx, hipStreamSynchronize(sl.stream));
    GMX_HIP(ctx, hipGetLastError());
    f.struct_size = (uint32_t)sizeof(gm_cylinder_fit);
    *out = f;
    return GM_OK;
}


void gm_surface_default_params(gm_surface_params *p)
{
    if (!p) return;
    memset(p, 0, sizeof(*p));
    p->struct_size = (uint32_t)sizeof(gm_surface_params);
    p->n_stations = 40;
    p->n_sectors = 90;
    p->station_length = 0.25;
    p->t_min = -5.0;
    p->gate = 0.25;
    p->up[2] = 1.0;
    p->forward[0] = 1.0;
}

gm_status gm_set_surface_params(gm_ctx *ctx, const gm_surface_params *p)
{
    if (!ctx) return GM_ERR_INVALID_ARG;
    if (gm_check_surface_params(p) != GM_OK)
        return gm_fail(ctx, GM_ERR_INVALID_ARG, "gm_set_surface_params: NULL, struct_size mismatch or a parameter outside its limits");
    for (uint32_t i = 0; i < ctx->n_slots; ++i)
        if (ctx->slots[i].submitted && !ctx->slots[i].complete)
            return gm_fail(ctx, GM_ERR_NOT_READY, "gm_set_surface_params: a slot holds a submitted frame that has not been waited for");
    if (hipSetDevice(ctx->device) != hipSuccess) return gm_fail(ctx, GM_ERR_DEVICE, "hipSetDevice failed");
    ctx->surf = *p;
    const SurfParams d = surface_device_params(*p);
    for (uint32_t i = 0; i < ctx->n_slots; ++i) {
        Slot &sl = ctx->slots[i];
        if (!sl.surf_prm) continue;
        GMX_HIP(ctx, hipMemcpyAsync(sl.surf_prm, &d, sizeof(d), hipMemcpyHostToDevice, sl.stream));
        GMX_HIP(ctx, hipStreamSynchronize(sl.stream));
    }
    return GM_OK;
}

gm_status gm_get_surface_map(gm_ctx *ctx, uint32_t slot, gm_surface_info *info, gm_surface_cell *cells, uint32_t capacity,
                             uint32_t *n_out)
// ... 9 lines not shown
    GMX_HIP(ctx, hipMemcpyAsync(&inf, sl.surf_info, sizeof(inf), hipMemcpyDeviceToHost, sl.stream));
    GMX_HIP(ctx, hipStreamSynchronize(sl.stream));
    *info = inf;
    const uint32_t nc = inf.n_stations * inf.n_sectors;
    if (n_out) *n_out = nc;
    if (nc > capacity) return gm_fail(ctx, GM_ERR_CAPACITY, "gm_get_surface_map: cell buffer too small");
    if (!nc) return GM_OK;
    if (!cells) return gm_fail(ctx, GM_ERR_INVALID_ARG, "gm_get_surface_map: NULL cells");
    GMX_HIP(ctx, hipMemcpyAsync(cells, sl.surf_cells, (size_t)nc * sizeof(gm_surface_cell), hipMemcpyDeviceToHost, sl.stream));
    GMX_HIP(ctx, hipStreamSynchronize(sl.stream));
    return GM_OK;
}

gm_status gm_get_surface_points(gm_ctx *ctx, uint32_t slot, float *residual, int32_t *cell, uint32_t capacity, uint32_t *n_out)
{
    if (!ctx) return GM_ERR_INVALID_ARG;
    if (!(ctx->cfg.flags & GM_CFG_SURFACE_MAP))
        return gm_fail(ctx, GM_ERR_UNSUPPORTED, "gm_get_surface_points: context created without GM_CFG_SURFACE_MAP");
    gm_status st = gm_check_slot(ctx, slot);
    if (st != GM_OK) return st;
    Slot &sl = ctx->slots[slot];
    const uint32_t n = sl.last.n_valid;
    if (n_out) *n_out = n;
    if (n > capacity) return gm_fail(ctx, GM_ERR_CAPACITY, "gm_get_surface_points: output buffer too small");
    if (!n) return GM_OK;
    if (residual) GMX_HIP(ctx, hipMemcpyAsync(residual, sl.surf_res, (size_t)n * 4, hipMemcpyDeviceToHost, sl.stream));
    if (cell) GMX_HIP(ctx, hipMemcpyAsync(cell, sl.surf_cell, (size_t)n * 4, hipMemcpyDeviceToHost, sl.stream));
    GMX_HIP(ctx, hipStreamSynchronize(sl.stream));
    return GM_OK;
}

gm_status gm_surface_map(gm_ctx *ctx, const float *xyz, uint32_t n, const uint8_t *labels, const float model7[7],
                         const gm_surface_params *p, gm_surface_info *info, gm_surface_cell *cells, uint32_t capacity,
                         float *residual, int32_t *cell)
{
    if (!ctx) return GM_ERR_INVALID_ARG;
    if ((n && !xyz) || !model7 || !info) return gm_fail(ctx, GM_ERR_INVALID_ARG, "gm_surface_map: NULL argument");
    gm_surface_params prm;
    if (p) prm = *p;
    else gm_surface_default_params(&prm);
    if (gm_check_surface_params(&prm) != GM_OK)
        return gm_fail(ctx, GM_ERR_INVALID_ARG, "gm_surface_map: struct_size mismatch or a parameter outside its limits");
    const uint32_t nc = prm.n_stations * prm.n_sectors;
    if (nc > capacity) return gm_fail(ctx, GM_ERR_CAPACITY, "gm_surface_map: cell buffer too small");
    if (!cells) return gm_fail(ctx, GM_ERR_INVALID_ARG, "gm_surface_map: NULL cells");
    Slot *slp;
    gm_status st = gm_begin_stage(ctx, slp);
    if (st != GM_OK) return st;
    Slot &sl = *slp;
    st = gm_ensure_capacity(ctx, sl, n ? n : 1u, (size_t)(n ? n : 1u) * 16, true);
    if (st != GM_OK) return st;
    st = gm_ensure_surface(ctx, sl);
    if (st != GM_OK) return st;
    st = upload_xyz(ctx, sl, xyz, n, sl.valid4);
    if (st != GM_OK) return st;
    st = upload_labels(ctx, sl, labels, n);
    if (st != GM_OK) return st;
    gm_cylinder_fit f;
    memset(&f, 0, sizeof(f));
    f.status = GM_FIT_OK;
    for (int k = 0; k < 7; ++k) f.model[k] = model7[k];
    const SurfParams d = surface_device_params(prm);
    GMX_HIP(ctx, hipMemcpyAsync(sl.surf_fit, &f, sizeof(f), hipMemcpyHostToDevice, sl.stream));
    GMX_HIP(ctx, hipMemcpyAsync(sl.surf_prm + 1, &d, sizeof(d), hipMemcpyHostToDevice, sl.stream));
    SurfArgs a;
    a.pts = sl.valid4; a.labels = labels ? sl.labels : nullptr; a.n_ptr = nullptr; a.n_host = n;
    a.fit = sl.surf_fit; a.prm = sl.surf_prm + 1;
    a.table = sl.surf_table; a.cells = sl.surf_cells; a.info = sl.surf_info; a.res = sl.surf_res; a.cell = sl.surf_cell;
    launch_surface_map(a, n, sl.stream);
    GMX_HIP(ctx, hipGetLastError());
    gm_surface_info inf;
    GMX_HIP(ctx, hipMemcpyAsync(&inf, sl.surf_info, sizeof(inf), hipMemcpyDeviceToHost, sl.stream));
    GMX_HIP(ctx, hipMemcpyAsync(cells, sl.surf_cells, (size_t)nc * sizeof(gm_surface_cell), hipMemcpyDeviceToHost, sl.stream));
    if (residual && n) GMX_HIP(ctx, hipMemcpyAsync(residual, sl.surf_res, (size_t)n * 4, hipMemcpyDeviceToHost, sl.stream));
    if (cell && n) GMX_HIP(ctx, hipMemcpyAsync(cell, sl.surf_cell, (size_t)n * 4, hipMemcpyDeviceToHost, sl.stream));
    GMX_HIP(ctx, hipStreamSynchronize(sl.stream));
    *info = inf;
    return GM_OK;
}

gm_status gm_get_compressed_map(gm_ctx *ctx, uint32_t slot, void *buf, size_t capacity, size_t *n_bytes)
{
    gm_status st = gm_check_slot(ctx, slot);
    if (st != GM_OK) return st;
    Slot &sl = ctx->slots[slot];
    const gm_frame_result &r = sl.last;
    uint32_t nprim = 0;
    const bool has_plane = (ctx->cfg.flags & GM_CFG_RANSAC_PLANE) && r.plane_inliers > 0 && isfinite(r.plane[0]);
    const bool has_cyl = (ctx->cfg.flags & GM_CFG_RANSAC_CYLINDER) && r.cylinder_inliers > 0 && isfinite(r.cylinder[0]);
    nprim = (has_plane ? 1u : 0u) + (has_cyl ? 1u : 0u);
    const uint32_t nvox = (ctx->cfg.flags & GM_CFG_VOXEL_GRID) ? r.n_voxels : 0;
    const size_t need = sizeof(gm_map_header) + (size_t)nprim * sizeof(gm_map_primitive) + (size_t)nvox * 16;
    if (n_bytes) *n_bytes = need;
    if (need > capacity) return gm_fail(ctx, GM_ERR_CAPACITY, "map buffer too small");
    if (!buf) return gm_fail(ctx, GM_ERR_INVALID_ARG, "map buffer is NULL");
    uint8_t *p = (uint8_t *)buf;
    gm_map_header h;
    memset(&h, 0, sizeof(h));
    memcpy(h.magic, "GMAP", 4);
    h.version = 1;
    h.n_primitives = nprim;
    h.n_voxels = nvox;
    h.leaf = (float)ctx->cfg.voxelGridLeafSize;
    h.bound = (float)ctx->cfg.boxFilterBound;
    h.n_points = r.n_valid;
    for (int k = 0; k < 3; ++k) { h.eigenvalues[k] = r.eigenvalues[k]; h.center_axis[k] = r.center_axis[k]; }
    memcpy(p, &h, sizeof(h)); p += sizeof(h);
    if (has_plane) {
        gm_map_primitive q;
        memset(&q, 0, sizeof(q));
        q.type = 1; q.inliers = r.plane_inliers;
        for (int k = 0; k < 4; ++k) q.params[k] = (float)r.plane_refit[k];
        memcpy(p, &q, sizeof(q)); p += sizeof(q);
    }
    if (has_cyl) {
        gm_map_primitive q;
        memset(&q, 0, sizeof(q));
        q.type = 2; q.inliers = r.cylinder_inliers;
        for (int k = 0; k < 7; ++k) q.params[k] = r.cylinder[k];
// ... 15 lines not shown
```

geometric_mapping_amd/csrc/gm_group.hip:

```cpp
#include <dlfcn.h>
#include <math.h>
#include <rccl/rccl.h>
#include <stddef.h>
#include <stdlib.h>
#include <string.h>

#include <algorithm>
#include <chrono>
#include <deque>
#include <limits>
#include <new>
#include <string>
#include <thread>
#include <vector>

#include "gm_internal.hpp"

using namespace gm;

namespace {

constexpr int kRecLen = 24;

struct Rccl {
// ... 612 lines not shown
    }
    const uint32_t total = G.last.n_valid;
    if (n_out) *n_out = total;
    if (total > capacity) return gfail(grp, GM_ERR_CAPACITY, "output buffer too small");
    if (!total) return GM_OK;
    if (!labels) return gfail(grp, GM_ERR_INVALID_ARG, "output pointer is NULL");
    std::vector<MergedRow> all;
    const gm_status st = merged_rows(G, true, all);
    if (st != GM_OK) return st;
    for (size_t i = 0; i < all.size() && i < capacity; ++i) labels[i] = all[i].label;
    return GM_OK;
}

gm_status gm_group_get_voxel_centroids(gm_group *grp, float *xyzc, uint32_t capacity, uint32_t *n_out)
{
    if (!grp) return GM_ERR_INVALID_ARG;
    gm_group &G = *grp;
    if (!G.have_frame) { if (n_out) *n_out = 0; return gfail(grp, GM_ERR_NOT_READY, "gm_group: no completed sharded frame"); }
    if (!(G.cfg.flags & GM_CFG_VOXEL_GRID)) return gfail(grp, GM_ERR_NOT_READY, "group created without GM_CFG_VOXEL_GRID");
    const uint32_t V = (uint32_t)(G.vox_cen.size() / 4);
    if (n_out) *n_out = V;
    if (V > capacity) return gfail(grp, GM_ERR_CAPACITY, "output buffer too small");
    if (V && !xyzc) return gfail(grp, GM_ERR_INVALID_ARG, "output pointer is NULL");
    if (V) memcpy(xyzc, G.vox_cen.data(), (size_t)V * 16);
    return GM_OK;
}

gm_status gm_group_get_voxel_normals(gm_group *grp, float *nxyzc, uint32_t capacity, uint32_t *n_out)
{
    if (!grp) return GM_ERR_INVALID_ARG;
    gm_group &G = *grp;
    if (!G.have_frame) { if (n_out) *n_out = 0; return gfail(grp, GM_ERR_NOT_READY, "gm_group: no completed sharded frame"); }
    if ((G.cfg.flags & (GM_CFG_NEAREST | GM_CFG_VOXEL_GRID)) != (GM_CFG_NEAREST | GM_CFG_VOXEL_GRID))
        return gfail(grp, GM_ERR_NOT_READY, "group created without GM_CFG_NEAREST | GM_CFG_VOXEL_GRID");
    const uint32_t V = (uint32_t)(G.vox_cen.size() / 4);
    if (n_out) *n_out = V;
    if (V > capacity) return gfail(grp, GM_ERR_CAPACITY, "output buffer too small");
    if (!V) return GM_OK;
    if (!nxyzc) return gfail(grp, GM_ERR_INVALID_ARG, "output pointer is NULL");
    if (!G.vox_nrm_valid) {
        G.vox_nrm.assign((size_t)V * 4, std::numeric_limits<float>::quiet_NaN());
        std::vector<unsigned long long> best_key(V, ~0ull);
        std::vector<unsigned long long> keys;
        std::vector<float> nrm, pts;
        for (uint32_t r = 0; r < G.n; ++r) {
            gm_ctx *c = G.ctx[r];
            Slot &sl = c->slots[0];
            if (hipSetDevice(G.devices[r]) != hipSuccess) return gfail(grp, GM_ERR_DEVICE, "hipSetDevice failed");
            if (sl.last.n_valid == 0) continue;
            for (uint32_t q0 = 0; q0 < V; q0 += sl.cap) {
                const uint32_t nq = V - q0 < sl.cap ? V - q0 : sl.cap;
                if (hipMemcpyAsync(sl.vox4, &G.vox_cen[(size_t)q0 * 4], (size_t)nq * 16, hipMemcpyHostToDevice, sl.stream) != hipSuccess)
                    return gfail(grp, GM_ERR_DEVICE, "gm_group: upload of the merged centroids failed");
                launch_nearest(sl.valid4, &sl.ctr->n_valid, sl.cap, sl.vox4, nullptr, nq, sl.nn_best, sl.vox_nn, sl.stream, sl.vnorm4, sl.vox_nrm4);
                hipLaunchKernelGGL(k_gather_nearest, dim3((nq + 255) / 256), dim3(256), 0, sl.stream, (const int32_t *)sl.vox_nn, nq,
                                   (const float4 *)sl.valid4, sl.spts4);
                keys.resize(nq); nrm.resize((size_t)nq * 4); pts.resize((size_t)nq * 4);
                if (hipMemcpyAsync(keys.data(), sl.nn_best, (size_t)nq * 8, hipMemcpyDeviceToHost, sl.stream) != hipSuccess ||
                    hipMemcpyAsync(nrm.data(), sl.vox_nrm4, (size_t)nq * 16, hipMemcpyDeviceToHost, sl.stream) != hipSuccess ||
                    hipMemcpyAsync(pts.data(), sl.spts4, (size_t)nq * 16, hipMemcpyDeviceToHost, sl.stream) != hipSuccess ||
                    hipStreamSynchronize(sl.stream) != hipSuccess)
                    return gfail(grp, GM_ERR_DEVICE, "gm_group: nearest-point search failed");
                for (uint32_t i = 0; i < nq; ++i) {
                    if (keys[i] == ~0ull) continue;
                    uint32_t local;
                    memcpy(&local, &pts[4 * (size_t)i + 3], 4);
                    if (local >= G.row_ids[r].size()) return gfail(grp, GM_ERR_DEVICE, "gm_group: a rank's row index is out of range");
                    const unsigned long long k = (keys[i] & 0xFFFFFFFF00000000ull) | G.row_ids[r][local];
                    if (k < best_key[q0 + i]) {
                        best_key[q0 + i] = k;
                        memcpy(&G.vox_nrm[4 * (size_t)(q0 + i)], &nrm[4 * (size_t)i], 16);
                    }
                }
            }
        }
        G.vox_near.assign(V, -1);
        {
            std::vector<uint32_t> valid_rows;
            valid_rows.reserve(G.last.n_valid);
            std::vector<float> buf;
            for (uint32_t r = 0; r < G.n; ++r) {
                uint32_t m = G.ctx[r]->slots[0].last.n_valid;
                buf.resize((size_t)(m ? m : 1) * 4);
                const gm_status st = gm_get_cropped_xyz(G.ctx[r], 0, buf.data(), m ? m : 1, &m);
                if (st != GM_OK) return gfail(grp, st, gm_last_error(G.ctx[r]));
                for (uint32_t i = 0; i < m; ++i) {
                    uint32_t local;
                    memcpy(&local, &buf[4 * (size_t)i + 3], 4);
                    if (local < G.row_ids[r].size()) valid_rows.push_back(G.row_ids[r][local]);
                }
            }
            std::sort(valid_rows.begin(), valid_rows.end());
            for (uint32_t i = 0; i < V; ++i) {
                if (best_key[i] == ~0ull) continue;
                const uint32_t row = (uint32_t)(best_key[i] & 0xFFFFFFFFull);
                G.vox_near[i] = (int32_t)(std::lower_bound(valid_rows.begin(), valid_rows.end(), row) - valid_rows.begin());
            }
        }
        G.vox_nrm_valid = true;
    }
    memcpy(nxyzc, G.vox_nrm.data(), (size_t)V * 16);
    return GM_OK;
}

gm_status gm_group_get_voxel_nearest(gm_group *grp, int32_t *idx, uint32_t capacity, uint32_t *n_out)
{
    if (!grp) return GM_ERR_INVALID_ARG;
    gm_group &G = *grp;
    if (!G.have_frame) { if (n_out) *n_out = 0; return gfail(grp, GM_ERR_NOT_READY, "gm_group: no completed sharded frame"); }
// ... 6 lines not shown
        std::vector<float> tmp((size_t)V * 4);
        const gm_status st = gm_group_get_voxel_normals(grp, tmp.data(), V, nullptr);
        if (st != GM_OK) return st;
    }
    memcpy(idx, G.vox_near.data(), (size_t)V * 4);
    return GM_OK;
}

gm_status gm_group_fit_cylinder(gm_group *grp, const float init7[7], gm_cylinder_fit *out)
{
    if (!grp) return GM_ERR_INVALID_ARG;
    gm_group &G = *grp;
    if (G.dead) return gfail(grp, GM_ERR_COMM, "gm_group: an earlier collective failed; destroy the group");
    if (!out) return gfail(grp, GM_ERR_INVALID_ARG, "gm_group_fit_cylinder: NULL argument");
    if (!G.have_frame) return gfail(grp, GM_ERR_NOT_READY, "gm_group: no completed sharded frame");
    G.have_fit = false;
    const uint32_t R = G.n;
    const double tau = G.cfg.ransac_threshold;
    if (!(tau > 0.0) || !std::isfinite(tau)) return gfail(grp, GM_ERR_INVALID_ARG, "gm_group_fit_cylinder: ransac_threshold must be > 0");
    G.fitr.resize(R);
    for (uint32_t r = 0; r < R; ++r) {
        gm_group::FitRank &f = G.fitr[r];
        if (f.rows) continue;
        if (hipSetDevice(G.devices[r]) != hipSuccess) return gfail(grp, GM_ERR_DEVICE, "hipSetDevice failed");
        hipError_t e = f.partial.reserve((size_t)kFitBlocks * kFitRowLen);
        if (e == hipSuccess) e = f.ticket.reserve(1);
        if (e == hipSuccess) e = hipMemset(f.ticket, 0, sizeof(uint32_t));
        if (e == hipSuccess) e = f.work.reserve(1);
        if (e == hipSuccess) e = f.fit.reserve(1);
        if (e == hipSuccess) e = f.rows8.reserve(16);
        if (e == hipSuccess) e = f.plane_best.reserve(1);
        if (e == hipSuccess) e = f.row.reserve((size_t)4 * kFitRowLen);
        if (e == hipSuccess) e = f.rows.reserve((size_t)4 * kFitRowLen * R);
        if (e != hipSuccess) return gfail(grp, GM_ERR_OOM, "gm_group_fit_cylinder: device allocation failed");
    }
    if (G.h_fit.reserve(R) != hipSuccess) return gfail(grp, GM_ERR_OOM, "gm_group_fit_cylinder: hipHostMalloc failed");
    const float nanf_ = std::numeric_limits<float>::quiet_NaN();
    float rows8[16];
    for (int k = 0; k < 16; ++k) rows8[k] = 0.f;
    const bool has_cyl = (G.cfg.flags & GM_CFG_RANSAC_CYLINDER) && G.last.cylinder_inliers > 0;
    for (int k = 0; k < 7; ++k) rows8[k] = init7 ? init7[k] : (has_cyl ? G.last.cylinder[k] : nanf_);
    bool has_plane = (G.cfg.flags & GM_CFG_RANSAC_PLANE) && G.last.plane_inliers > 0;
    for (int k = 0; k < 4; ++k) { rows8[8 + k] = G.last.plane[k]; has_plane = has_plane && std::isfinite(G.last.plane[k]); }
    const uint32_t plane_best = has_plane ? 0u : 0xFFFFFFFFu;
    std::vector<CylFitArgs> args(R);
    auto fail_enqueued = [&](gm_status s, const std::string &msg) { drain(G); return gfail(grp, s, msg); };
    for (uint32_t r = 0; r < R; ++r) {
        gm_group::FitRank &f = G.fitr[r];
        Slot &sl = G.ctx[r]->slots[0];
        if (hipSetDevice(G.devices[r]) != hipSuccess ||
            hipMemcpyAsync(f.rows8, rows8, sizeof(rows8), hipMemcpyHostToDevice, sl.stream) != hipSuccess ||
            hipMemcpyAsync(f.plane_best, &plane_best, sizeof(uint32_t), hipMemcpyHostToDevice, sl.stream) != hipSuccess)
            return fail_enqueued(GM_ERR_DEVICE, "gm_group_fit_cylinder: upload of the starting rows failed");
        launch_label(0, sl.valid4, sl.labels, 0, 1, &sl.ctr->n_valid, sl.last.n_valid, f.rows8 + 8, nullptr, f.plane_best,
                     tau, 1, nullptr, nullptr, 0, sl.stream);
        CylFitArgs &a = args[r];
        a.pts = sl.valid4; a.labels = sl.labels; a.out = sl.labels;
        a.want = 0; a.want2 = 0; a.mask_mode = 0;
        a.n_ptr = &sl.ctr->n_valid; a.n_host = sl.last.n_valid;
        a.init = f.rows8; a.best = nullptr;
        a.work = f.work; a.fit = f.fit; a.partial = f.partial; a.ticket = f.ticket;
        a.tau = tau;
    }
    for (int pass = 0; pass < 4; ++pass) {
        for (uint32_t r = 0; r < R; ++r) {
            hipSetDevice(G.devices[r]);
            hipStream_t s = G.ctx[r]->slots[0].stream;
            CylFitArgs a = args[r];
            a.rank_row = G.fitr[r].row + (size_t)pass * kFitRowLen;
            launch_cylinder_fit_pass(a, pass, s);
            if (G.loopback) hipEventRecord(G.ev[r], s);
        }
        if (!G.loopback) {
            ncclResult_t rc = G.rccl.GroupStart();
            for (uint32_t r = 0; r < R && rc == ncclSuccess; ++r) {
                hipSetDevice(G.devices[r]);
                rc = G.rccl.AllGather(G.fitr[r].row + (size_t)pass * kFitRowLen, G.fitr[r].rows + (size_t)pass * kFitRowLen * R, kFitRowLen,
                                      ncclDouble, G.comms[r], G.ctx[r]->slots[0].stream);
            }
            const ncclResult_t rc2 = G.rccl.GroupEnd();
            if (rc == ncclSuccess) rc = rc2;
            if (rc != ncclSuccess) {
                G.dead = true;
                return gfail(grp, GM_ERR_COMM, std::string("ncclAllGather: ") + G.rccl.GetErrorString(rc));
            }
        } else {
            for (uint32_t r = 0; r < R; ++r) {
                hipSetDevice(G.devices[r]);
                hipStream_t s = G.ctx[r]->slots[0].stream;
                double *dst = G.fitr[r].rows + (size_t)pass * kFitRowLen * R;
                for (uint32_t q = 0; q < R; ++q) {
                    if (q != r) hipStreamWaitEvent(s, G.ev[q], 0);
                    hipMemcpyAsync(dst + (size_t)q * kFitRowLen, G.fitr[q].row + (size_t)pass * kFitRowLen, sizeof(double) * kFitRowLen,
                                   hipMemcpyDeviceToDevice, s);
                }
            }
        }
        for (uint32_t r = 0; r < R; ++r) {
            hipSetDevice(G.devices[r]);
            launch_cylinder_fit_merge(args[r], pass, G.fitr[r].rows + (size_t)pass * kFitRowLen * R, R, G.ctx[r]->slots[0].stream);
        }
    }
    for (uint32_t r = 0; r < R; ++r) {
        hipSetDevice(G.devices[r]);
        if (hipMemcpyAsync(&G.h_fit[r], G.fitr[r].fit, sizeof(gm_cylinder_fit), hipMemcpyDeviceToHost, G.ctx[r]->slots[0].stream) != hipSuccess)
            return fail_enqueued(GM_ERR_DEVICE, "gm_group_fit_cylinder: D2H of a rank's fit failed");
    }
    for (uint32_t r = 0; r < R; ++r) {
        hipSetDevice(G.devices[r]);
        if (hipStreamSynchronize(G.ctx[r]->slots[0].stream) != hipSuccess || hipGetLastError() != hipSuccess)
// ... 82 lines not shown
```

geometric_mapping_amd/csrc/gm_internal.hpp:

```cpp
#pragma once

#include <hip/hip_runtime.h>
#include <stdint.h>

#include <string>
#include <vector>

#include "../../include/gm_hip.h"
#include "gm_dev_array.hpp"
#include "gm_device.hpp"

namespace gm {

struct RowLayout {
    const uint8_t *data;
    const uint8_t *const *data_at;
    uint32_t step, ox, oy, oz;
    uint32_t mode;
    uint32_t bswap;
};

struct SortScratch {
    DevArray<uint32_t> totals;
    DevArray<uint32_t> rec;
    size_t rec_words = 0;
    DevArray<uint32_t> ticket;
};

struct SortPlan { int passes, bits; };

struct Slot {
    hipStream_t stream = nullptr;
    hipEvent_t ev[GM_N_STAGES + 1] = {};
    hipEvent_t ev_k0 = nullptr, ev_k1 = nullptr;
    uint32_t cap = 0;
    size_t raw_cap = 0;
    HostArray<uint8_t> h_raw;
    DevArray<uint8_t> d_raw;
    DevArray<float4> crop4;
    DevArray<uint32_t> keys_a, keys_b, vals_a, vals_b;
    DevArray<float4> spts4;
    uint32_t *skeys = nullptr;
    DevArray<float4> normals4;
    DevArray<int32_t> counts;
    DevArray<float4> valid4;
    DevArray<float4> vnorm4;
    DevArray<uint2> tiles;
    uint32_t tiles_cap = 0;
    uint32_t tile_seg = 0;
    DevArray<uint2> row_bounds;
    DevArray<unsigned long long> blk;
    uint32_t blk_cap = 0;
    uint32_t scan_epoch = 0;
    uint32_t scan_seq = 0;
    uint32_t frames_enqueued = 0;
    bool capturing = false;
    bool kernel_timed = false;
    DevArray<uint32_t> frame_in;
    HostArray<uint32_t> h_frame_in;
    static constexpr int kGraphs = 4;
    hipGraphExec_t graph_exec[kGraphs] = {};
    unsigned char graph_key[kGraphs][512] = {};
    uint32_t graph_key_len[kGraphs] = {};
    uint64_t graph_used[kGraphs] = {};
    uint64_t graph_clock = 0;
    uint32_t graph_captures = 0;
    uint32_t alloc_gen = 0;
    SortScratch sort;
    DevArray<unsigned long long> tile_rec;
    size_t tile_rec_words = 0;
    DevArray<uint32_t> seg_start;
    DevArray<float4> vox4;
    DevArray<VoxCell> vox_table;
    DevArray<int32_t> vox_nn;
    DevArray<double> partials;
    DevArray<double> tile_partials;
    DevArray<uint8_t> labels;
    DevArray<uint8_t> inl_mask;
    DevArray<DevCounters> ctr;
    DevArray<VoxelParams> voxp;
    DevArray<FrameOut> d_out;
    HostArray<FrameOut> h_out;
    uint32_t ext_H = 0, ext_cap = 0;
    DevArray<float> hyp_plane, hyp_cyl;
    DevArray<float2> band;
    DevArray<uint32_t> score_partial;
    DevArray<int32_t> cnt_plane, cnt_cyl;
    DevArray<uint32_t> best_plane, best_cyl;
    DevArray<double> mom_partial;
    DevArray<double> mom_plane, mom_cyl;
    DevArray<unsigned long long> nn_best;
    DevArray<float4> vox_nrm4;
    DevArray<double> fit_partial;
    DevArray<uint32_t> fit_ticket;
    DevArray<CylFitWork> fit_work;
    DevArray<float> fit_init;
    DevArray<gm_cylinder_fit> fit_stage;
    gm_cylinder_fit last_fit = {};
    DevArray<SurfParams> surf_prm;
// ... 23 lines not shown
    if (sl.capturing) {
        st.epoch = sl.scan_seq++ & 31u;
        st.frame_ptr = sl.frame_in + 4;
    } else {
        if (sl.scan_epoch >= 0x1FFFFFFEu) {
            (void)hipMemsetAsync(sl.blk, 0, sizeof(unsigned long long) * (size_t)sl.blk_cap, sl.stream);
            if (sl.tile_rec) (void)hipMemsetAsync(sl.tile_rec, 0, sizeof(unsigned long long) * sl.tile_rec_words, sl.stream);
            sl.scan_epoch = 0;
        }
        sl.scan_epoch += 1u;
        st.epoch = sl.scan_epoch;
        st.frame_ptr = nullptr;
    }
    st.ticket = reinterpret_cast<uint32_t *>(sl.blk + sl.blk_cap);
    return st;
}

}

struct gm_ctx {
    gm_config cfg;
    int device = 0;
    uint32_t n_slots = 1;
    gm::Slot *slots = nullptr;
    double own_lo, own_hi;
    bool force_voxel_sort = false;
    gm_surface_params surf;
    std::vector<gm_wall_map *> walls;
    std::string err;
};

namespace gm {

constexpr int kScatterBlocks = 1024;


void launch_crop(const RowLayout &rows, uint32_t n, float lo, float hi, const GridParams &g, Slot &sl, hipStream_t s,
                 uint32_t n_size = 0, const uint32_t *n_dev = nullptr, bool count_digits = false);
size_t radix_totals_bytes();
size_t radix_record_words(uint32_t n_cap, int key_bits);
size_t radix_record_words_max(uint32_t n_cap);
SortPlan radix_plan(int key_bits);
int cell_key_bits(const GridParams &g);
int launch_radix_sort(uint32_t *keys_a, uint32_t *vals_a, uint32_t *keys_b, uint32_t *vals_b,
                      const uint32_t *n_ptr, uint32_t n_cap, int key_bits, Slot &sl, bool prepared,
                      hipStream_t s, const float4 *rows_in = nullptr, float4 *rows_out = nullptr);
void launch_grid_and_normals(const GridParams &g, const VoxDense &vd, Slot &sl, uint32_t n_cap, bool keep_counts,
                             bool scratch_cleared, hipStream_t s);
struct ZeroJobs { void *ptr[6]; uint64_t words8[6]; uint32_t *frame_counter; };
void launch_zero_fill(const ZeroJobs &jobs, hipStream_t s);
uint32_t max_tiles(uint32_t n_cap, const GridParams &g);
uint32_t tile_cutter_blocks(uint32_t n_cap);
uint32_t launch_compact_valid(Slot &sl, uint32_t n_cap, double weightingFactor, hipStream_t s, uint32_t *row_tile = nullptr);
uint32_t launch_scatter_partials(const float4 *vnorm4, const uint32_t *n_ptr, uint32_t n_cap, double wf, Slot &sl,
                                 hipStream_t s);
void launch_rows_to_host(const float4 *src, float4 *dst_mapped, const uint32_t *begin_enc, const uint32_t *end_ptr, hipStream_t s);
void launch_frame_finalize(const double *partials, uint32_t n_partials, uint32_t row_tile, Slot &sl, hipStream_t s);
void launch_voxel_grid(Slot &sl, uint32_t n_cap, float leaf, int key_bits, hipStream_t s);
void launch_voxel_dense_finalize(const VoxDense &vd, Slot &sl, hipStream_t s);
constexpr uint32_t kVoxDenseMaxCells = 1u << 18;
constexpr uint32_t kMaxHypotheses = 8192;
uint32_t score_blocks(uint32_t n_cap);
void launch_plane_hypotheses(const float4 *pts, const uint8_t *labels, uint32_t want, const uint32_t *n_ptr,
                             uint32_t n_host, uint64_t seed, uint32_t H, float *hyp8, int32_t *zero_counts,
                             hipStream_t s);
void launch_cylinder_hypotheses(const float4 *pts, const float4 *nrm, const uint8_t *labels, uint32_t want,
                                const uint32_t *n_ptr, uint32_t n_host, uint64_t seed, uint32_t H, float *hyp8,
                                int32_t *zero_counts, float2 *band, double tau, hipStream_t s);
void launch_score(int model, const float4 *pts, const uint8_t *labels, uint32_t want, const uint32_t *n_ptr,
                  uint32_t n_cap, const float *hyp8, float2 *band, uint32_t H, double tau, uint32_t *partial,
                  int32_t *counts, uint32_t *best, hipStream_t s);
bool launch_score_preemptive(int model, const float4 *pts, const uint8_t *labels, uint32_t want,
                             const uint32_t *n_ptr, uint32_t n_cap, const float *hyp8, float2 *band, uint32_t H,
                             double tau, uint32_t *scratch, int32_t *counts, uint32_t *best, bool prepared,
                             const uint32_t **sel_out, const int32_t **cnt_out, uint32_t *k_out, hipStream_t s,
                             uint8_t *masks = nullptr, bool *masks_written = nullptr, bool *replicated_counts = nullptr);
uint32_t launch_label(int model, const float4 *pts, uint8_t *labels, uint32_t want, uint32_t label, const uint32_t *n_ptr,
                      uint32_t n_cap, const float *hyp8, const float2 *band, uint32_t *best, double tau, int init,
                      const uint32_t *sel, const int32_t *counts_k, uint32_t K, hipStream_t s,
                      const float4 *nrm = nullptr, double *mom_partial = nullptr,
                      const uint8_t *masks = nullptr, bool replicated_counts = false);
void launch_segment_moments(const float4 *pts, const float4 *nrm, const uint8_t *labels, uint32_t label,
                            const uint32_t *n_ptr, uint32_t n_cap, double *partial, double *mom16, hipStream_t s);
void launch_ext_finalize(const float *hyp_plane, const uint32_t *best_plane, const float *hyp_cyl,
                         const uint32_t *best_cyl, double *mom_plane, double *mom_cyl, FrameExt *ext,
                         const double *partial32, uint32_t mom_rows, hipStream_t s,
                         const double *scatter_partials = nullptr, uint32_t scatter_rows = 0, uint32_t row_tile = 0,
                         const DevCounters *ctr = nullptr, const VoxelParams *voxp = nullptr, FrameOut *frame_out = nullptr);
constexpr uint32_t kFitBlocks = 512;
constexpr int kFitRowLen = 24;
struct CylFitArgs {
    const float4 *pts;
    const uint8_t *labels;
    uint8_t *out;
    uint32_t want, want2, mask_mode;
    const uint32_t *n_ptr;
    uint32_t n_host;
    const float *init;
    const uint32_t *best;
    CylFitWork *work;
    gm_cylinder_fit *fit;
    double *partial;
    uint32_t *ticket;
    double tau;
    double *rank_row = nullptr;
};
void launch_cylinder_fit(const CylFitArgs &a, hipStream_t s);
// ... 212 lines not shown
```

geometric_mapping_amd/csrc/gm_wall.hip:

```cpp
#include <math.h>
#include <stdio.h>
#include <stdlib.h>
#include <string.h>

#include <algorithm>

#include "gm_compact.hpp"
#include "gm_internal.hpp"

using namespace gm;

#define GMW_HIP(ctx, call)                                                           \
    do {                                                                             \
        hipError_t e__ = (call);                                                     \
        if (e__ != hipSuccess) {                                                     \
            (ctx)->err = std::string(#call) + ": " + hipGetErrorString(e__);         \
            return (e__ == hipErrorOutOfMemory) ? GM_ERR_OOM : GM_ERR_DEVICE;        \
        }                                                                            \
    } while (0)
#define GMW_OK(call)                       \
    do {                                   \
        const gm_status s__ = (call);      \
        if (s__ != GM_OK) return s__;      \
    } while (0)
// ... 231 lines not shown
    GMW_HIP(ctx, hipStreamSynchronize(m->stream));
    return GM_OK;
}

gm_status check_window(gm_wall_map *m, uint32_t station0, uint32_t n, uint64_t capacity, uint64_t *n_out, const char *who)
{
    if ((uint64_t)station0 + n > m->prm.n_stations)
        return gm_fail(m->ctx, GM_ERR_INVALID_ARG, "gm_wall_map: the window leaves [0, n_stations]");
    const uint64_t nc = (uint64_t)n * m->prm.n_sectors;
    if (n_out) *n_out = nc;
    if (nc > capacity) return gm_fail(m->ctx, GM_ERR_CAPACITY, who);
    return GM_OK;
}

void free_map(gm_wall_map *m)
{
    hipSetDevice(m->ctx->device);
    for (uint32_t i = 0; i < m->ctx->n_slots; ++i)
        if (m->pending[i] && m->ctx->slots[i].stream) hipStreamSynchronize(m->ctx->slots[i].stream);
    for (WallCheckSlot &c : m->checks) {
        if (c.outstanding) hipEventSynchronize(c.done);
        if (c.done) hipEventDestroy(c.done);
        if (c.adds) hipEventDestroy(c.adds);
    }
    if (m->stream) { hipStreamSynchronize(m->stream); hipStreamDestroy(m->stream); }
    delete m;
}

struct StageCall {
    gm_wall_map *map;
    uint32_t n;
    float *residual;
    int32_t *cell, *delta;
    uint8_t *cls;
    Slot *sl = nullptr;
    gm_status open()
    {
        gm_ctx *ctx = map->ctx;
        GMW_OK(gm_begin_stage(ctx, sl));
        GMW_OK(gm_ensure_capacity(ctx, *sl, n ? n : 1u, (size_t)(n ? n : 1u) * 16, true));
        if (residual || cell) {
            GMW_HIP(ctx, map->pt_res.reserve(n));
            GMW_HIP(ctx, map->pt_cell.reserve(n));
        }
        if (delta || cls) {
            GMW_HIP(ctx, map->ck_delta.reserve(n));
            GMW_HIP(ctx, map->ck_cls.reserve(n));
        }
        return GM_OK;
    }
    gm_status upload(const float *xyz, const uint8_t *labels, WallArgs &w)
    {
        gm_ctx *ctx = map->ctx;
        GMW_OK(gm_upload_xyz(ctx, *sl, xyz, n, sl->valid4));
        if (labels && n) GMW_HIP(ctx, hipMemcpyAsync(sl->labels, labels, n, hipMemcpyHostToDevice, sl->stream));
        w.pts = sl->valid4;
        w.labels = labels ? sl->labels : nullptr;
        w.n_ptr = nullptr;
        w.n_host = n;
        w.res = residual ? map->pt_res.p : nullptr;
        w.cell = cell ? map->pt_cell.p : nullptr;
        return GM_OK;
    }
    gm_status close()
    {
        gm_ctx *ctx = map->ctx;
        if (residual && n) GMW_HIP(ctx, hipMemcpyAsync(residual, map->pt_res.p, (size_t)n * 4, hipMemcpyDeviceToHost, sl->stream));
        if (cell && n) GMW_HIP(ctx, hipMemcpyAsync(cell, map->pt_cell.p, (size_t)n * 4, hipMemcpyDeviceToHost, sl->stream));
        if (delta && n) GMW_HIP(ctx, hipMemcpyAsync(delta, map->ck_delta.p, (size_t)n * 4, hipMemcpyDeviceToHost, sl->stream));
        if (cls && n) GMW_HIP(ctx, hipMemcpyAsync(cls, map->ck_cls.p, (size_t)n, hipMemcpyDeviceToHost, sl->stream));
        GMW_HIP(ctx, hipStreamSynchronize(sl->stream));
        return GM_OK;
    }
};

template <class P>
P params_or(const P *prm, void (*defaults)(P *))
{
    P p;
    defaults(&p);
    if (prm) p = *prm;
    return p;
}

template <class R, class M>
bool extent_metrics(const gm_wall_params &p, const R &r, M *out)
{
    const uint32_t ns = p.n_sectors, half = ns / 2u;
    if (r.sector_min > r.sector_max || r.sector_max >= ns || r.sector_min_turned > r.sector_max_turned ||
        r.sector_max_turned >= ns || r.station_min > r.station_max)
        return false;
    const double from = (double)r.station_min * p.station_length;
    const double to = (double)(r.station_max + 1.0) * p.station_length;
    out->chainage_from = p.t_min + from;
    out->chainage_to = p.t_min + to;
    const uint32_t plain = r.sector_max - r.sector_min + 1u, turned = r.sector_max_turned - r.sector_min_turned + 1u;
    uint32_t k_from = r.sector_min, k_end = r.sector_max + 1u;
    if (turned < plain) {
        k_from = (r.sector_min_turned + ns - half) % ns;
        k_end = (r.sector_max_turned + ns - half) % ns + 1u;
    }
    const double a0 = 360.0 * (double)k_from;
    const double a1 = 360.0 * (double)k_end;
    out->angle_from_deg = a0 / (double)ns;
    out->angle_to_deg = a1 / (double)ns;
    return true;
}

gm_status read_window(gm_wall_map *m, uint32_t station0, uint32_t n, void *cells, bool raw)
// ... 310 lines not shown
            m->region_tk = tk;
        }
    }
    if (const char *e = getenv("GM_WALL_OBJECT_TILE")) {
        unsigned tr = 0, tc = 0;
        if (sscanf(e, "%ux%u", &tr, &tc) == 2 && tr >= 1u && tc >= 1u && (uint64_t)tr * tc <= kWallObjectTileBlocks) {
            m->object_tr = tr;
            m->object_tc = tc;
        }
    }
    if (const char *e = getenv("GM_WALL_CLOUD_CHUNK")) {
        const unsigned long long v = strtoull(e, nullptr, 10);
        m->cloud_chunk = v < kStageCells ? (uint32_t)v : 0u;
    }
    design_frame(m);
    auto body = [&]() -> gm_status {
        GMW_HIP(ctx, hipStreamCreateWithFlags(&m->stream, hipStreamNonBlocking));
        GMW_HIP(ctx, m->base.reserve(wall_table_bytes(m->ncell)));
        GMW_HIP(ctx, m->stage.reserve(std::min(kStageCells, m->ncell) * sizeof(gm_wall_raw_cell)));
        GMW_HIP(ctx, hipMemsetAsync(m->base.p, 0, wall_table_bytes(m->ncell), m->stream));
        GMW_HIP(ctx, hipStreamSynchronize(m->stream));
        return GM_OK;
    };
    const gm_status st = body();
    if (st != GM_OK) {
        (void)hipGetLastError();
        free_map(m);
        return st;
    }
    m->table = wall_table(m->base.p, m->ncell);
    ctx->walls.push_back(m);
    *map = m;
    return GM_OK;
}

void gm_wall_map_destroy(gm_wall_map *map)
{
    if (!map) return;
    std::vector<gm_wall_map *> &w = map->ctx->walls;
    w.erase(std::remove(w.begin(), w.end(), map), w.end());
    free_map(map);
}

gm_status gm_wall_map_add_frame(gm_wall_map *map, gm_ctx *ctx, uint32_t slot, const double pose[12], gm_wall_add_info *add_info)
{
    if (!map || !ctx) return GM_ERR_INVALID_ARG;
    if (ctx != map->ctx) return gm_fail(ctx, GM_ERR_INVALID_ARG, "gm_wall_map_add_frame: the map belongs to another context");
    if (slot >= ctx->n_slots) return gm_fail(ctx, GM_ERR_INVALID_ARG, "slot out of range");
    Slot &sl = ctx->slots[slot];
    if (!sl.submitted) return gm_fail(ctx, GM_ERR_NOT_READY, "gm_wall_map_add_frame: the slot holds no frame");
    WallArgs w;
    GMW_OK(add_frame_args(map, pose, add_info, w));
    if (hipSetDevice(ctx->device) != hipSuccess) return gm_fail(ctx, GM_ERR_DEVICE, "hipSetDevice failed");
    w.pts = sl.valid4;
    w.labels = (ctx->cfg.flags & GM_CFG_RANSAC_PLANE) ? sl.labels : nullptr;
    w.n_ptr = &sl.ctr->n_valid;
    w.n_host = sl.n_in;
    for (uint32_t i = 0; i < ctx->n_slots; ++i)
        if (i != slot && map->checks[i].outstanding) GMW_HIP(ctx, hipStreamWaitEvent(sl.stream, map->checks[i].done, 0));
    launch_wall_add(w, sl.n_in, map->points_per_block, sl.stream);
    GMW_HIP(ctx, hipGetLastError());
    map->pending[slot] = 1;
    ++map->frames;
    return GM_OK;
}

gm_status gm_wall_map_add_points(gm_wall_map *map, const float *xyz, uint32_t n, const uint8_t *labels, const double pose[12],
                                 gm_wall_add_info *add_info, float *residual, int32_t *cell)
{
    if (!map) return GM_ERR_INVALID_ARG;
    gm_ctx *ctx = map->ctx;
    if (n && !xyz) return gm_fail(ctx, GM_ERR_INVALID_ARG, "gm_wall_map_add_points: NULL xyz");
    WallArgs w;
    GMW_OK(add_frame_args(map, pose, add_info, w));
    StageCall sc{map, n, residual, cell, nullptr, nullptr};
    GMW_OK(sc.open());
    GMW_OK(sc.upload(xyz, labels, w));
    hipStream_t s = sc.sl->stream;
    for (uint32_t i = 1; i < ctx->n_slots; ++i)
        if (map->checks[i].outstanding) GMW_HIP(ctx, hipStreamWaitEvent(s, map->checks[i].done, 0));
    launch_wall_add(w, n, map->points_per_block, s);
    GMW_HIP(ctx, hipGetLastError());
    GMW_OK(sc.close());
    ++map->frames;
    return GM_OK;
}

gm_status gm_wall_map_sync(gm_wall_map *map)
{
    if (!map) return GM_ERR_INVALID_ARG;
    return sync_map(map);
}

gm_status gm_wall_map_info(gm_wall_map *map, gm_wall_info *info)
{
    if (!map) return GM_ERR_INVALID_ARG;
    gm_ctx *ctx = map->ctx;
    if (!info) return gm_fail(ctx, GM_ERR_INVALID_ARG, "gm_wall_map_info: NULL info");
    GMW_OK(sync_map(map));
    unsigned long long tot[kWallTotals];
    GMW_HIP(ctx, hipMemsetAsync(map->table.totals + 4, 0, 8, map->stream));
    launch_wall_count(map->table, map->ncell, map->stream);
    GMW_HIP(ctx, hipGetLastError());
    GMW_HIP(ctx, hipMemcpyAsync(tot, map->table.totals, sizeof(tot), hipMemcpyDeviceToHost, map->stream));
    GMW_HIP(ctx, hipStreamSynchronize(map->stream));
    memset(info, 0, sizeof(*info));
    info->struct_size = (uint32_t)sizeof(gm_wall_info);
// ... 322 lines not shown
    info->below_min_count = ctr[1];
    if (n_out) *n_out = total;
    if (points && total > capacity) return gm_fail(ctx, GM_ERR_CAPACITY, "gm_wall_map_cloud: point buffer too small");
    return GM_OK;
}

void gm_wall_check_default_params(gm_wall_check_params *p)
{
    if (!p) return;
    memset(p, 0, sizeof(*p));
    p->struct_size = (uint32_t)sizeof(gm_wall_check_params);
    p->reference = GM_WALL_CHECK_MEAN;
    p->min_count = 8;
    p->threshold = 0.05;
    p->gate = 1.0;
}

gm_status gm_wall_check_classify(const gm_wall_check_params *prm, const gm_wall_raw_cell *cell, float e, int64_t *delta, uint32_t *cls)
{
    long long T;
    if (!prm || !cell || !delta || !cls || !check_prm_ok(*prm, T)) return GM_ERR_INVALID_ARG;
    *delta = 0;
    if (!(fabsf(e) <= (float)prm->gate)) {
        *cls = GM_WALL_CHECK_CLS_BEYOND_GATE;
        return GM_OK;
    }
    long long d;
    *cls = wall_check_rule(prm->reference, prm->min_count, T, cell->sum, cell->count, cell->min_key, cell->max_key, e, d);
    *delta = d;
    return GM_OK;
}

gm_status gm_wall_map_check_frame(gm_wall_map *map, gm_ctx *ctx, uint32_t slot, const double pose[12],
                                  const gm_wall_check_params *prm, gm_wall_add_info *add_info)
{
    if (!map || !ctx) return GM_ERR_INVALID_ARG;
    if (ctx != map->ctx) return gm_fail(ctx, GM_ERR_INVALID_ARG, "gm_wall_map_check_frame: the map belongs to another context");
    if (slot >= ctx->n_slots) return gm_fail(ctx, GM_ERR_INVALID_ARG, "slot out of range");
    const gm_wall_check_params cp = params_or(prm, gm_wall_check_default_params);
    WallCheckArgs a;
    memset(&a, 0, sizeof(a));
    if (!check_prm_ok(cp, a.T))
        return gm_fail(ctx, GM_ERR_INVALID_ARG, "gm_wall_map_check_frame: struct_size mismatch or a parameter outside its limits");
    Slot &sl = ctx->slots[slot];
    if (!sl.submitted) return gm_fail(ctx, GM_ERR_NOT_READY, "gm_wall_map_check_frame: the slot holds no frame");
    GMW_OK(add_frame_args(map, pose, add_info, a.w));
    a.w.gate = (float)cp.gate;
    if (add_info) add_info->gate = a.w.gate;
    if (hipSetDevice(ctx->device) != hipSuccess) return gm_fail(ctx, GM_ERR_DEVICE, "hipSetDevice failed");
    const uint32_t n_cap = sl.n_in ? sl.n_in : 1u;
    ScanState scan;
    GMW_OK(check_prepare(map, slot, n_cap, sl.stream, scan));
    GMW_OK(check_wait_adds(map, slot, sl.stream));
    a.w.pts = sl.valid4;
    a.w.labels = (ctx->cfg.flags & GM_CFG_RANSAC_PLANE) ? sl.labels : nullptr;
    a.w.n_ptr = &sl.ctr->n_valid;
    a.w.n_host = sl.n_in;
    a.reference = cp.reference;
    a.min_count = cp.min_count;
    a.out = map->checks[slot].stage.p;
    a.ctr = map->checks[slot].ctr.p;
    return check_enqueue(map, slot, a, n_cap, scan, sl.stream);
}

gm_status gm_wall_map_get_check(gm_wall_map *map, uint32_t slot, gm_wall_check_info *info, gm_wall_check_point *points,
                                uint32_t capacity, uint32_t *n_out)
{
    if (!map) return GM_ERR_INVALID_ARG;
    gm_ctx *ctx = map->ctx;
    if (n_out) *n_out = 0;
    if (slot >= ctx->n_slots) return gm_fail(ctx, GM_ERR_INVALID_ARG, "slot out of range");
    if (!map->checks[slot].have) return gm_fail(ctx, GM_ERR_NOT_READY, "gm_wall_map_get_check: no check was enqueued on this map and slot");
    if (hipSetDevice(ctx->device) != hipSuccess) return gm_fail(ctx, GM_ERR_DEVICE, "hipSetDevice failed");
    return check_result(map, slot, info, points, capacity, n_out);
}

gm_status gm_wall_map_check_points(gm_wall_map *map, const float *xyz, uint32_t n, const uint8_t *labels, const double pose[12],
                                   const gm_wall_check_params *prm, gm_wall_add_info *add_info, gm_wall_check_info *info,
                                   gm_wall_check_point *points, uint32_t capacity, uint32_t *n_out, float *residual,
                                   int32_t *cell, int32_t *delta, uint8_t *cls)
{
    if (!map) return GM_ERR_INVALID_ARG;
    gm_ctx *ctx = map->ctx;
    if (n_out) *n_out = 0;
    if (n && !xyz) return gm_fail(ctx, GM_ERR_INVALID_ARG, "gm_wall_map_check_points: NULL xyz");
    if (!points && capacity) return gm_fail(ctx, GM_ERR_INVALID_ARG, "gm_wall_map_check_points: NULL points with a capacity");
    const gm_wall_check_params cp = params_or(prm, gm_wall_check_default_params);
    WallCheckArgs a;
    memset(&a, 0, sizeof(a));
    if (!check_prm_ok(cp, a.T))
        return gm_fail(ctx, GM_ERR_INVALID_ARG, "gm_wall_map_check_points: struct_size mismatch or a parameter outside its limits");
    GMW_OK(add_frame_args(map, pose, add_info, a.w));
    a.w.gate = (float)cp.gate;
    if (add_info) add_info->gate = a.w.gate;
    StageCall sc{map, n, residual, cell, delta, cls};
    GMW_OK(sc.open());
    hipStream_t s = sc.sl->stream;
    const uint32_t n_cap = n ? n : 1u;
    ScanState scan;
    GMW_OK(check_prepare(map, 0, n_cap, s, scan));
    GMW_OK(check_wait_adds(map, 0, s));
    GMW_OK(sc.upload(xyz, labels, a.w));
    a.delta = delta ? map->ck_delta.p : nullptr;
    a.cls = cls ? map->ck_cls.p : nullptr;
    a.reference = cp.reference;
    a.min_count = cp.min_count;
    a.row_is_index = 1u;
// ... 106 lines not shown
```

geometric_mapping_amd/csrc/k_frame.hip:

```cpp
#include "gm_compact.hpp"
#include "gm_internal.hpp"

namespace gm {

struct ValidPred {
    const float4 *__restrict__ normals4;
    uint32_t *__restrict__ first_drop_enc;
    typedef float4 Payload;
    __device__ __forceinline__ bool operator()(uint32_t i, Payload &p) const
    {
        p = normals4[i];
        const bool ok = finite3(p.x, p.y, p.z);
        if (!ok) {
            const uint32_t enc = 0xFFFFFFFFu - i;
            if (*first_drop_enc < enc) atomicMax(first_drop_enc, enc);
        }
        return ok;
    }
};

__global__ __launch_bounds__(256) void k_rows_to_host(const float4 *__restrict__ src, float4 *__restrict__ dst,
                                                      const uint32_t *__restrict__ begin_enc, const uint32_t *__restrict__ end_ptr)
{
    const uint32_t end = *end_ptr;
    uint32_t begin = 0;
    if (begin_enc) {
        const uint32_t e = *begin_enc;
        if (e == 0u) return;
        begin = 0xFFFFFFFFu - e;
    }
    for (uint32_t i = begin + blockIdx.x * blockDim.x + threadIdx.x; i < end; i += gridDim.x * blockDim.x)
        dst[i] = src[i];
}

void launch_rows_to_host(const float4 *src, float4 *dst_mapped, const uint32_t *begin_enc, const uint32_t *end_ptr, hipStream_t s)
{
    hipLaunchKernelGGL(k_rows_to_host, dim3(64), dim3(256), 0, s, src, dst_mapped, begin_enc, end_ptr);
}

__device__ __forceinline__ void scatter_term(const float4 v , double k_wf, double m[6])
{
    const double t = (double)v.w + k_wf;
    const float wgt = (float)exp(t * t);
    const double a = (double)(wgt * v.x), b = (double)(wgt * v.y), c = (double)(wgt * v.z);
    m[0] += a * a; m[1] += a * b; m[2] += a * c; m[3] += b * b; m[4] += b * c; m[5] += c * c;
}

__device__ __forceinline__ void scatter_row_store(const double m[6], double *__restrict__ row)
{
    __shared__ double red[16][6];
    const int w = threadIdx.x / kWave, nw = blockDim.x / kWave;
#pragma unroll
    for (int k = 0; k < 6; ++k) {
        const double r = wave_sum(m[k]);
        if (lane_id() == 0) red[w][k] = r;
    }
    __syncthreads();
    if (threadIdx.x < 6) {
        double r = 0;
#pragma unroll
        for (int j = 0; j < nw; ++j) r += red[j][threadIdx.x];
        row[threadIdx.x] = r;
    }
}

struct ValidEmit {
    static constexpr bool kHasFinish = true, kHasPrepare = false;
    const float4 *__restrict__ crop4;
    float4 *__restrict__ valid4;
    float4 *__restrict__ vnorm4;
    double k_wf;
    double *__restrict__ partials;
    double m[6];
    __device__ __forceinline__ void operator()(uint32_t src, uint32_t dst, const float4 &v)
    {
        valid4[dst] = crop4[src];
        vnorm4[dst] = v;
        scatter_term(v, k_wf, m);
    }
    __device__ __forceinline__ void finish(uint32_t tile)
    {
        scatter_row_store(m, partials + (size_t)tile * 6);
#pragma unroll
        for (int k = 0; k < 6; ++k) m[k] = 0;
    }
};

__global__ __launch_bounds__(256) void k_minmax(const float4 *__restrict__ pts, const uint32_t *__restrict__ n_ptr,
                                                uint32_t n_host, DevCounters *__restrict__ ctr)
{
    __shared__ float red[6][256 / kWave];
    const uint32_t n = n_ptr ? *n_ptr : n_host;
    float mn[3] = {3.0e38f, 3.0e38f, 3.0e38f}, mx[3] = {-3.0e38f, -3.0e38f, -3.0e38f};
    for (uint32_t i = blockIdx.x * blockDim.x + threadIdx.x; i < n; i += gridDim.x * blockDim.x) {
        const float4 p = pts[i];
        mn[0] = fminf(mn[0], p.x); mn[1] = fminf(mn[1], p.y); mn[2] = fminf(mn[2], p.z);
        mx[0] = fmaxf(mx[0], p.x); mx[1] = fmaxf(mx[1], p.y); mx[2] = fmaxf(mx[2], p.z);
    }
    const int w = threadIdx.x / kWave;
#pragma unroll
    for (int k = 0; k < 3; ++k) {
        const float a = wave_min(mn[k]), b = wave_max(mx[k]);
        if (lane_id() == 0) { red[k][w] = a; red[3 + k][w] = b; }
    }
    __syncthreads();
    if (threadIdx.x < 6) {
        const int k = threadIdx.x;
        float v = red[k][0];
        for (int j = 1; j < 256 / kWave; ++j) v = (k < 3) ? fminf(v, red[k][j]) : fmaxf(v, red[k][j]);
        if (blockIdx.x * blockDim.x < n) {
            if (k < 3) atomicMin(&ctr->mm[k], float_to_ordered(v));
            else atomicMax(&ctr->mm[k], float_to_ordered(v));
        }
    }
}

__global__ void k_init_minmax(DevCounters *ctr)
{
    if (threadIdx.x < 3) ctr->mm[threadIdx.x] = 0xFFFFFFFFu;
    else if (threadIdx.x < 6) ctr->mm[threadIdx.x] = 0u;
}

void launch_minmax(const float4 *pts, const uint32_t *n_ptr, uint32_t n_cap, DevCounters *ctr, hipStream_t s)
{
    hipLaunchKernelGGL(k_init_minmax, dim3(1), dim3(64), 0, s, ctr);
    if (n_cap == 0) return;
    uint32_t nb = (n_cap + 255) / 256;
    if (nb > 1024) nb = 1024;
    hipLaunchKernelGGL(k_minmax, dim3(nb), dim3(256), 0, s, pts, n_ptr, n_cap, ctr);
}

uint32_t launch_compact_valid(Slot &sl, uint32_t n_cap, double wf, hipStream_t s, uint32_t *row_tile)
{
    static const char *e = getenv("GM_VALID_TILE");
    int th = 512, it = 8;
    if (e) sscanf(e, "%dx%d", &th, &it);
    else if (n_cap > 2000000u) { th = 1024; it = 8; }
    const bool big = th == 1024 && it == 8;
    const uint32_t tile = big ? 8192u : (uint32_t)kCpTile;
    if (row_tile) *row_tile = tile;
    const uint32_t nb = (n_cap + tile - 1) / tile;
    if (nb == 0) return 0;
    ValidPred pred{sl.normals4, &sl.ctr->first_drop_enc};
    ValidEmit emit{sl.crop4, sl.valid4, sl.vnorm4, .001 / wf, sl.tile_partials, {0, 0, 0, 0, 0, 0}};
    if (big)
        hipLaunchKernelGGL((k_compact<ValidPred, ValidEmit, 1024, 8>), dim3(nb), dim3(1024), 0, s, pred, emit,
                           (const uint32_t *)&sl.ctr->n_cropped, 0u, next_scan(sl), &sl.ctr->n_valid, &sl.ctr->vox_n);
    else
        hipLaunchKernelGGL((k_compact<ValidPred, ValidEmit>), dim3(nb), dim3(kCpThreads), 0, s, pred, emit,
                           (const uint32_t *)&sl.ctr->n_cropped, 0u, next_scan(sl), &sl.ctr->n_valid, &sl.ctr->vox_n);
    return nb;
}

__global__ __launch_bounds__(256) void k_scatter_partials(const float4 *__restrict__ vnorm4,
                                                          const uint32_t *__restrict__ n_ptr, uint32_t n_host,
                                                          double k_wf ,
                                                          double *__restrict__ partials)
{
    const uint32_t n = n_ptr ? *n_ptr : n_host;
    double m[6] = {0, 0, 0, 0, 0, 0};
    for (uint32_t i = blockIdx.x * blockDim.x + threadIdx.x; i < n; i += gridDim.x * blockDim.x)
        scatter_term(vnorm4[i], k_wf, m);
    scatter_row_store(m, partials + (size_t)blockIdx.x * 6);
}

__global__ __launch_bounds__(256) void k_frame_finalize(const double *__restrict__ partials, uint32_t nblocks,
                                                        const DevCounters *__restrict__ ctr,
                                                        const VoxelParams *__restrict__ voxp,
                                                        FrameOut *__restrict__ out, uint32_t row_tile)
{
    __shared__ double red[256 * 6];
    frame_finalize_block(partials, nblocks, ctr, voxp, out, red, row_tile);
}

uint32_t launch_scatter_partials(const float4 *vnorm4, const uint32_t *n_ptr, uint32_t n_cap, double wf, Slot &sl,
                                 hipStream_t s)
{
    uint32_t nb = (n_cap + 4095) / 4096;
    if (nb < 64u) nb = (n_cap + 255) / 256 < 64u ? (n_cap + 255) / 256 : 64u;
    if (nb > (uint32_t)kScatterBlocks) nb = kScatterBlocks;
    if (nb == 0) nb = 1;
    hipLaunchKernelGGL(k_scatter_partials, dim3(nb), dim3(256), 0, s, vnorm4, n_ptr, n_cap, .001 / wf, sl.partials);
    return nb;
}

void launch_frame_finalize(const double *partials, uint32_t n_partials, uint32_t row_tile, Slot &sl, hipStream_t s)
{
    hipLaunchKernelGGL(k_frame_finalize, dim3(1), dim3(256), 0, s, partials, n_partials,
                       (const DevCounters *)sl.ctr, (const VoxelParams *)sl.voxp, sl.d_out, row_tile);
}

}
```

geometric_mapping_amd/csrc/k_voxel.hip:

```cpp
#include "gm_compact.hpp"
#include "gm_internal.hpp"

namespace gm {

__global__ void k_voxel_setup(const DevCounters *__restrict__ ctr, float leaf, VoxelParams *__restrict__ vp)
{
    if (threadIdx.x != 0 || blockIdx.x != 0) return;
    const float inv = 1.0f / leaf;
    vp->inv_leaf = inv;
    vp->passthrough = 0;
    if (ctr->vox_n == 0) {
        for (int k = 0; k < 3; ++k) { vp->min_b[k] = 0; vp->div_b[k] = 1; }
        vp->mul1 = 1; vp->mul2 = 1;
        return;
    }
    float mn[3], mx[3];
    for (int k = 0; k < 3; ++k) { mn[k] = ordered_to_float(ctr->mm[k]); mx[k] = ordered_to_float(ctr->mm[3 + k]); }
    const long long dx = (long long)((mx[0] - mn[0]) * inv) + 1;
    const long long dy = (long long)((mx[1] - mn[1]) * inv) + 1;
    const long long dz = (long long)((mx[2] - mn[2]) * inv) + 1;
    if (dx * dy * dz > 2147483647ll) vp->passthrough = 1;
    for (int k = 0; k < 3; ++k) {
        const int lo = (int)floorf(mn[k] * inv), hi = (int)floorf(mx[k] * inv);
        vp->min_b[k] = lo;
// ... 39 lines not shown
{
    const uint32_t n = ctr->vox_n, V = ctr->n_voxels;
    const uint32_t wave = (blockIdx.x * blockDim.x + threadIdx.x) / kWave;
    const uint32_t nwaves = gridDim.x * blockDim.x / kWave;
    for (uint32_t v = wave; v < V; v += nwaves) {
        const uint32_t b = seg_start[v], e = (v + 1 < V) ? seg_start[v + 1] : n;
        double sx = 0, sy = 0, sz = 0;
        for (uint32_t s = b + lane_id(); s < e; s += kWave) {
            const float4 p = pts[perm[s]];
            sx += p.x; sy += p.y; sz += p.z;
        }
        sx = wave_sum(sx); sy = wave_sum(sy); sz = wave_sum(sz);
        if (lane_id() == 0) {
            const double c = (double)(e - b);
            vox4[v] = make_float4((float)(sx / c), (float)(sy / c), (float)(sz / c), (float)(e - b));
        }
    }
}

struct DensePred {
    const VoxCell *__restrict__ table;
    typedef NoPayload Payload;
    __device__ __forceinline__ bool operator()(uint32_t i, Payload &) const { return table[i].cnt != 0; }
};
struct DenseEmit {
    static constexpr bool kHasFinish = false, kHasPrepare = false;
    const VoxCell *__restrict__ table;
    float4 *__restrict__ vox4;
    double lo, inv_scale;
    __device__ __forceinline__ void operator()(uint32_t src, uint32_t dst, const NoPayload &) const
    {
        const VoxCell c = table[src];
        const double inv = inv_scale / (double)c.cnt;
        vox4[dst] = make_float4((float)(lo + (double)c.sx * inv), (float)(lo + (double)c.sy * inv),
                                (float)(lo + (double)c.sz * inv), (float)c.cnt);
    }
};

void launch_voxel_dense_finalize(const VoxDense &vd, Slot &sl, hipStream_t s)
{
    const uint32_t cells = (uint32_t)vd.dim * vd.dim * vd.dim;
    DensePred pred{sl.vox_table};
    DenseEmit emit{sl.vox_table, sl.vox4, (double)vd.lo, vd.inv_scale};
    hipLaunchKernelGGL((k_compact<DensePred, DenseEmit>), dim3(compact_grid(cells)), dim3(kCpThreads), 0, s, pred, emit,
                       (const uint32_t *)nullptr, cells, next_scan(sl), &sl.ctr->n_voxels, (uint32_t *)nullptr);
}

void launch_voxel_grid(Slot &sl, uint32_t n_cap, float leaf, int key_bits, hipStream_t s)
{
    hipLaunchKernelGGL(k_voxel_setup, dim3(1), dim3(64), 0, s, (const DevCounters *)sl.ctr, leaf, sl.voxp);
    if (n_cap == 0) return;
    uint32_t gb = (n_cap + 255) / 256;
    if (gb > 2048) gb = 2048;
    hipLaunchKernelGGL(k_voxel_keys, dim3(gb), dim3(256), 0, s, (const float4 *)sl.valid4, (const DevCounters *)sl.ctr,
                       (const VoxelParams *)sl.voxp, sl.keys_a);
    const int where = launch_radix_sort(sl.keys_a, sl.vals_a, sl.keys_b, sl.vals_b, &sl.ctr->vox_n, n_cap, key_bits,
                                        sl, false, s);
    const uint32_t *skeys = where ? sl.keys_b : sl.keys_a;
    const uint32_t *perm = where ? sl.vals_b : sl.vals_a;
    HeadPred pred{skeys};
    HeadEmit emit{sl.seg_start};
    hipLaunchKernelGGL((k_compact<HeadPred, HeadEmit>), dim3(compact_grid(n_cap)), dim3(kCpThreads), 0, s, pred, emit,
                       (const uint32_t *)&sl.ctr->vox_n, 0u, next_scan(sl), &sl.ctr->n_voxels, (uint32_t *)nullptr);
    hipLaunchKernelGGL(k_voxel_centroids, dim3(gb), dim3(256), 0, s, (const float4 *)sl.valid4, perm,
                       (const uint32_t *)sl.seg_start, (const DevCounters *)sl.ctr, sl.vox4);
}

}
```

include/gm_hip.h:

```cpp
#ifndef GM_HIP_H
#define GM_HIP_H

#include <stddef.h>
#include <stdint.h>

#ifdef __cplusplus
extern "C" {
#endif

#define GM_ABI_VERSION 3u

typedef struct gm_ctx gm_ctx;

typedef enum gm_status {
    GM_OK = 0,
    GM_ERR_INVALID_ARG = 1,
    GM_ERR_TOO_FEW_POINTS = 2,
    GM_ERR_DEVICE = 3,
    GM_ERR_OOM = 4,
    GM_ERR_CAPACITY = 5,
    GM_ERR_NOT_READY = 6,
    GM_ERR_UNSUPPORTED = 7,
    GM_ERR_COMM = 8
} gm_status;
// ... 52 lines not shown
    uint32_t status_flags;
    double   scatter[6];
    uint32_t plane_inliers, cylinder_inliers;
    float    plane[4];
    float    cylinder[7];
    double   plane_refit[4];
    double   cylinder_axis_refit[3];
    float    stage_ms[GM_N_STAGES];
    float    normals_kernel_ms;
} gm_frame_result;


gm_status gm_create(const gm_config *cfg, gm_ctx **out);
void gm_destroy(gm_ctx *ctx);

gm_status gm_host_alloc(gm_ctx *ctx, size_t bytes, void **out);
gm_status gm_host_free(gm_ctx *ctx, void *ptr);
gm_status gm_host_register(gm_ctx *ctx, void *ptr, size_t bytes);
gm_status gm_host_unregister(gm_ctx *ctx, void *ptr);

void gm_default_config(gm_config *cfg);

uint32_t gm_abi_version(void);
long long gm_debug_live_buffers(void);
const char *gm_status_string(gm_status s);
const char *gm_last_error(const gm_ctx *ctx);


gm_status gm_process_frame(gm_ctx *ctx, const gm_cloud *cloud, gm_frame_result *res);

gm_status gm_submit_frame(gm_ctx *ctx, uint32_t slot, const gm_cloud *cloud);
gm_status gm_wait_frame(gm_ctx *ctx, uint32_t slot, gm_frame_result *res);
gm_status gm_poll_frame(gm_ctx *ctx, uint32_t slot);

gm_status gm_set_cloud_output(gm_ctx *ctx, uint32_t slot, float *xyzw, uint32_t capacity);

gm_status gm_get_cropped_xyz(gm_ctx *ctx, uint32_t slot, float *xyzw, uint32_t capacity, uint32_t *n_out);
gm_status gm_get_normals(gm_ctx *ctx, uint32_t slot, float *nxyzc, uint32_t capacity, uint32_t *n_out);
gm_status gm_get_voxel_centroids(gm_ctx *ctx, uint32_t slot, float *xyzc, uint32_t capacity, uint32_t *n_out);
gm_status gm_get_voxel_nearest(gm_ctx *ctx, uint32_t slot, int32_t *idx, uint32_t capacity, uint32_t *n_out);
gm_status gm_get_voxel_normals(gm_ctx *ctx, uint32_t slot, float *nxyzc, uint32_t capacity, uint32_t *n_out);
gm_status gm_get_neighbor_counts(gm_ctx *ctx, uint32_t slot, int32_t *counts, uint32_t capacity, uint32_t *n_out);
gm_status gm_get_labels(gm_ctx *ctx, uint32_t slot, uint8_t *labels, uint32_t capacity, uint32_t *n_out);


gm_status gm_chop_cloud(gm_ctx *ctx, const gm_cloud *cloud, double bound,
                        float *xyzw_out, uint32_t capacity, uint32_t *n_out);

gm_status gm_get_normals_stage(gm_ctx *ctx, const float *xyz, uint32_t n, double radius,
                               float *xyzw_out, float *nxyzc_out, uint32_t capacity, uint32_t *n_out);

gm_status gm_get_local_frame(gm_ctx *ctx, const float *nxyzc, uint32_t n, double weighting_factor,
                             float eigenvalues[3], float eigenvectors[9], double scatter6[6]);

gm_status gm_voxel_grid(gm_ctx *ctx, const float *xyz, uint32_t n, double leaf,
                        float *xyzc_out, uint32_t capacity, uint32_t *n_out, uint32_t *status_flags);

gm_status gm_nearest(gm_ctx *ctx, const float *xyz, uint32_t n, const float *queries, uint32_t nq,
                     int32_t *idx_out);


gm_status gm_solve_local_frame(const double scatter6[6], float eigenvalues[3], float eigenvectors[9]);

gm_status gm_set_owned_range(gm_ctx *ctx, double own_lo, double own_hi);


int gm_ext_available(void);


gm_status gm_score_planes(gm_ctx *ctx, const float *xyz, uint32_t n, const uint8_t *labels, uint32_t want,
                          const float *hyp4, uint32_t H, double tau, int32_t *counts);
gm_status gm_score_cylinders(gm_ctx *ctx, const float *xyz, uint32_t n, const uint8_t *labels, uint32_t want,
                             const float *hyp7, uint32_t H, double tau, int32_t *counts);
gm_status gm_score_frame(gm_ctx *ctx, uint32_t slot, int model, const float *hyp, uint32_t H, double tau,
                         uint32_t unlabelled_only, int32_t *counts);
gm_status gm_plane_hypotheses(gm_ctx *ctx, const float *xyz, uint32_t n, const uint8_t *labels, uint32_t want,
                              uint64_t seed, uint32_t H, float *hyp4);
gm_status gm_cylinder_hypotheses(gm_ctx *ctx, const float *xyz, const float *nxyzc, uint32_t n,
                                 const uint8_t *labels, uint32_t want, uint64_t seed, uint32_t H, float *hyp7);
gm_status gm_segment_moments(gm_ctx *ctx, const float *xyz, const float *nxyzc, const uint8_t *labels,
                             uint32_t n, uint32_t label, double mom16[16]);

#define GM_FIT_OK            0u
#define GM_FIT_NO_MODEL      1u
#define GM_FIT_DEGENERATE    2u
#define GM_FIT_SINGULAR      3u
#define GM_FIT_FAILED_MASK   0xFFu
#define GM_FIT_NOT_CONVERGED (1u << 8)
#define GM_FIT_STEP_BOUND    1e-2

typedef struct gm_cylinder_fit {
    uint32_t struct_size;
    uint32_t status;
    uint32_t inliers;
    uint32_t passes;
    double   point[3];
    double   axis[3];
    double   radius;
    double   rms;
    double   last_step;
    float    model[7];
} gm_cylinder_fit;

gm_status gm_get_cylinder_fit(gm_ctx *ctx, uint32_t slot, gm_cylinder_fit *out);
gm_status gm_fit_cylinder(gm_ctx *ctx, const float *xyz, uint32_t n, const uint8_t *labels, uint32_t want,
                          const float init7[7], double tau, gm_cylinder_fit *out, uint8_t *inlier_out);
// ... 350 lines not shown
```

Baseline: 5.092 billion points/s.

## Compact valid rows in place, dropping the separate valid4/vnorm4 buffers

Replaces the out-of-place valid-row compaction (crop4/normals4 copied into valid4/vnorm4) with a two-pass scheme. A scan kernel computes counts, the first-drop index and the scatter partials, then an in-place compaction moves only rows at or after the first dropped row. Tiles entirely before the first drop publish their status and exit without doing work, so a frame with all rows finite skips almost all compaction traffic and the two extra buffers are no longer allocated. In exchange it adds a second kernel launch and depends on in-place ordering guarantees in the decoupled look-back scan (a waitcnt or fence) for correctness. It also adds a new test/stage API entry point.

```diff
diff --git a/geometric_mapping_amd/_lib.py b/geometric_mapping_amd/_lib.py
--- a/geometric_mapping_amd/_lib.py
+++ b/geometric_mapping_amd/_lib.py
@@ -312,6 +312,7 @@
         "gm_chop_cloud": (C.c_int, [vp, cloudp, C.c_double, fp, u32, u32p]),
         "gm_get_normals_stage": (C.c_int, [vp, fp, u32, C.c_double, fp, fp, u32, u32p]),
         "gm_get_local_frame": (C.c_int, [vp, fp, u32, C.c_double, fp, fp, dp]),
+        "gm_compact_valid_stage": (C.c_int, [vp, fp, fp, u32, C.c_double, fp, fp, u32, u32p, dp]),
         "gm_voxel_grid": (C.c_int, [vp, fp, u32, C.c_double, fp, u32, u32p, u32p]),
         "gm_nearest": (C.c_int, [vp, fp, u32, fp, u32, i32p]),
         "gm_solve_local_frame": (C.c_int, [dp, fp, fp]),
diff --git a/geometric_mapping_amd/api.py b/geometric_mapping_amd/api.py
--- a/geometric_mapping_amd/api.py
+++ b/geometric_mapping_amd/api.py
@@ -258,6 +258,21 @@
         M = np.array([[sc[0], sc[1], sc[2]], [sc[1], sc[3], sc[4]], [sc[2], sc[4], sc[5]]])
         return ev, V.reshape(3, 3).T.copy(), M
 
+    def compactValid(self, weightingFactor, rows, normals):
+        r = np.ascontiguousarray(rows, dtype=np.float32)
+        nr = np.ascontiguousarray(normals, dtype=np.float32)
+        if r.ndim != 2 or r.shape[1] != 4 or nr.shape != r.shape:
+            raise ValueError("rows and normals must both be [n,4]")
+        n0 = r.shape[0]
+        cap = max(n0, 1)
+        oc = np.empty((cap, 4), dtype=np.float32)
+        on = np.empty((cap, 4), dtype=np.float32)
+        n = C.c_uint32(0)
+        sc = np.zeros(6, dtype=np.float64)
+        self._check(self._L.gm_compact_valid_stage(self._ctx, _f32(r), _f32(nr), n0, float(weightingFactor), _f32(oc),
+                                                   _f32(on), cap, C.byref(n), sc.ctypes.data_as(C.POINTER(C.c_double))))
+        return oc[:n.value].copy(), on[:n.value].copy(), sc
+
     def voxelGrid(self, leafSize, cloud):
         xyz = np.ascontiguousarray(cloud, dtype=np.float32)
         if xyz.ndim != 2 or xyz.shape[1] != 3:
diff --git a/geometric_mapping_amd/csrc/gm_api.hip b/geometric_mapping_amd/csrc/gm_api.hip
--- a/geometric_mapping_amd/csrc/gm_api.hip
+++ b/geometric_mapping_amd/csrc/gm_api.hip
@@ -180,7 +180,6 @@
     GM_HIP(ctx, sl.vals_a.reserve(cap, gen)); GM_HIP(ctx, sl.vals_b.reserve(cap, gen));
     GM_HIP(ctx, sl.spts4.reserve(cap, gen)); GM_HIP(ctx, sl.normals4.reserve(cap, gen));
     GM_HIP(ctx, sl.counts.reserve(cap, gen));
-    GM_HIP(ctx, sl.valid4.reserve(cap, gen)); GM_HIP(ctx, sl.vnorm4.reserve(cap, gen));
     GM_HIP(ctx, sl.seg_start.reserve(cap, gen)); GM_HIP(ctx, sl.vox4.reserve(cap, gen));
     GM_HIP(ctx, sl.vox_nn.reserve(cap, gen)); GM_HIP(ctx, sl.labels.reserve(cap, gen)); GM_HIP(ctx, sl.inl_mask.reserve(cap, gen));
     sl.tiles_cap = cap + 2u;
@@ -188,7 +187,7 @@
     GM_HIP(ctx, sl.tiles.reserve((size_t)(kTileListClasses - 1) * sl.tile_seg + sl.tiles_cap, gen));
     GM_HIP(ctx, sl.row_bounds.reserve((size_t)1024 * 1024, gen));
     sl.blk_cap = compact_records(cap > kVoxDenseMaxCells ? cap : kVoxDenseMaxCells) + 1;
-    GM_HIP(ctx, sl.tile_partials.reserve((size_t)compact_blocks(cap) * 6, gen));
+    GM_HIP(ctx, sl.tile_partials.reserve((size_t)compact_records(cap) * 6, gen));
     GM_HIP(ctx, sl.blk.reserve((size_t)sl.blk_cap + 1, gen));
     GM_HIP(ctx, hipMemsetAsync(sl.blk, 0, sizeof(unsigned long long) * ((size_t)sl.blk_cap + 1), sl.stream));
     {
@@ -307,12 +306,12 @@
     if (cloud_overlap) {
         GM_HIP(ctx, hipEventRecord(sl.ev_valid, s));
         GM_HIP(ctx, hipStreamWaitEvent(sl.copy_stream, sl.ev_valid, 0));
-        launch_rows_to_host(sl.valid4, sl.cloud_out_dev, &sl.ctr->first_drop_enc, &sl.ctr->n_valid, sl.copy_stream);
+        launch_rows_to_host(sl.crop4, sl.cloud_out_dev, &sl.ctr->first_drop_enc, &sl.ctr->n_valid, sl.copy_stream);
         GM_HIP(ctx, hipEventRecord(sl.ev_copied, sl.copy_stream));
         cloud_copy_pending = true;
     } else if (sl.cloud_out && n) {
         const size_t frozen = (size_t)(ns < sl.cloud_out_cap ? ns : sl.cloud_out_cap) * sizeof(float4);
-        GM_HIP(ctx, hipMemcpyAsync(sl.cloud_out, sl.valid4, frozen, hipMemcpyDeviceToHost, s));
+        GM_HIP(ctx, hipMemcpyAsync(sl.cloud_out, sl.crop4, frozen, hipMemcpyDeviceToHost, s));
     }
     record(ctx, sl, 4);
     record(ctx, sl, 5);
@@ -321,7 +320,7 @@
         if (vd.enabled) {
             launch_voxel_dense_finalize(vd, sl, s);
         } else {
-            launch_minmax(sl.valid4, &sl.ctr->n_valid, ns, sl.ctr, s);
+            launch_minmax(sl.crop4, &sl.ctr->n_valid, ns, sl.ctr, s);
             launch_voxel_grid(sl, ns, (float)cf.voxelGridLeafSize, voxel_key_bits(lo, hi, cf.voxelGridLeafSize), s);
         }
     }
@@ -332,8 +331,8 @@
     }
     if ((cf.flags & GM_CFG_NEAREST) && (cf.flags & GM_CFG_VOXEL_GRID)) {
         const uint32_t nq_cap = vd.enabled ? (uint32_t)vd.dim * vd.dim * vd.dim : ns;
-        launch_nearest(sl.valid4, &sl.ctr->n_valid, ns, sl.vox4, &sl.ctr->n_voxels, nq_cap < ns ? nq_cap : ns, sl.nn_best,
-                       sl.vox_nn, s, sl.vnorm4, sl.vox_nrm4);
+        launch_nearest(sl.crop4, &sl.ctr->n_valid, ns, sl.vox4, &sl.ctr->n_voxels, nq_cap < ns ? nq_cap : ns, sl.nn_best,
+                       sl.vox_nn, s, sl.normals4, sl.vox_nrm4);
     }
     record(ctx, sl, 7);
     if (!(cf.flags & (GM_CFG_RANSAC_PLANE | GM_CFG_RANSAC_CYLINDER)))
@@ -624,27 +623,27 @@
     uint32_t mom_rows = 0;
     if (do_plane) {
         uint8_t *lab = first ? nullptr : sl.labels;
-        launch_plane_hypotheses(sl.valid4, lab, 0, n_ptr, n_cap, cf.ransac_seed, H, sl.hyp_plane, sl.cnt_plane, s);
+        launch_plane_hypotheses(sl.crop4, lab, 0, n_ptr, n_cap, cf.ransac_seed, H, sl.hyp_plane, sl.cnt_plane, s);
         const uint32_t *fsel = nullptr; const int32_t *fcnt = nullptr; uint32_t fk = 0; bool fmask = false, frep = false;
-        launch_score_preemptive(0, sl.valid4, lab, 0, n_ptr, n_cap, sl.hyp_plane, sl.band, H, cf.ransac_threshold,
+        launch_score_preemptive(0, sl.crop4, lab, 0, n_ptr, n_cap, sl.hyp_plane, sl.band, H, cf.ransac_threshold,
                                 sl.score_partial, sl.cnt_plane, sl.best_plane, true, &fsel, &fcnt, &fk, s, sl.inl_mask, &fmask, &frep);
-        mom_rows = launch_label(0, sl.valid4, sl.labels, 0, 1, n_ptr, n_cap, sl.hyp_plane, sl.band, sl.best_plane,
-                                cf.ransac_threshold, first ? 1 : 0, fsel, fcnt, fk, s, sl.vnorm4, sl.mom_partial, fmask ? sl.inl_mask : nullptr, frep);
+        mom_rows = launch_label(0, sl.crop4, sl.labels, 0, 1, n_ptr, n_cap, sl.hyp_plane, sl.band, sl.best_plane,
+                                cf.ransac_threshold, first ? 1 : 0, fsel, fcnt, fk, s, sl.normals4, sl.mom_partial, fmask ? sl.inl_mask : nullptr, frep);
         first = false;
     }
     if (do_cyl) {
         uint8_t *lab = first ? nullptr : sl.labels;
-        launch_cylinder_hypotheses(sl.valid4, sl.vnorm4, lab, 0, n_ptr, n_cap, cf.ransac_seed + 1, H, sl.hyp_cyl,
+        launch_cylinder_hypotheses(sl.crop4, sl.normals4, lab, 0, n_ptr, n_cap, cf.ransac_seed + 1, H, sl.hyp_cyl,
                                    sl.cnt_cyl, sl.band, cf.ransac_threshold, s);
         const uint32_t *fsel = nullptr; const int32_t *fcnt = nullptr; uint32_t fk = 0; bool fmask = false, frep = false;
-        launch_score_preemptive(1, sl.valid4, lab, 0, n_ptr, n_cap, sl.hyp_cyl, sl.band, H, cf.ransac_threshold,
+        launch_score_preemptive(1, sl.crop4, lab, 0, n_ptr, n_cap, sl.hyp_cyl, sl.band, H, cf.ransac_threshold,
                                 sl.score_partial, sl.cnt_cyl, sl.best_cyl, true, &fsel, &fcnt, &fk, s, sl.inl_mask, &fmask, &frep);
-        mom_rows = launch_label(1, sl.valid4, sl.labels, 0, 2, n_ptr, n_cap, sl.hyp_cyl, sl.band, sl.best_cyl,
-                                cf.ransac_threshold, first ? 1 : 0, fsel, fcnt, fk, s, sl.vnorm4, sl.mom_partial, fmask ? sl.inl_mask : nullptr, frep);
+        mom_rows = launch_label(1, sl.crop4, sl.labels, 0, 2, n_ptr, n_cap, sl.hyp_cyl, sl.band, sl.best_cyl,
+                                cf.ransac_threshold, first ? 1 : 0, fsel, fcnt, fk, s, sl.normals4, sl.mom_partial, fmask ? sl.inl_mask : nullptr, frep);
         first = false;
         if (cf.flags & GM_CFG_CYLINDER_FIT) {
             CylFitArgs a;
-            a.pts = sl.valid4; a.labels = sl.labels; a.out = sl.labels;
+            a.pts = sl.crop4; a.labels = sl.labels; a.out = sl.labels;
             a.want = 0; a.want2 = 2; a.mask_mode = 0;
             a.n_ptr = n_ptr; a.n_host = n_cap;
             a.init = sl.hyp_cyl; a.best = sl.best_cyl;
@@ -653,7 +652,7 @@
             launch_cylinder_fit(a, s);
             if (cf.flags & GM_CFG_SURFACE_MAP) {
                 SurfArgs m;
-                m.pts = sl.valid4; m.labels = sl.labels; m.n_ptr = n_ptr; m.n_host = n_cap;
+                m.pts = sl.crop4; m.labels = sl.labels; m.n_ptr = n_ptr; m.n_host = n_cap;
                 m.fit = &sl.d_out->fit; m.prm = sl.surf_prm;
                 m.table = sl.surf_table; m.cells = sl.surf_cells; m.info = sl.surf_info; m.res = sl.surf_res; m.cell = sl.surf_cell;
                 launch_surface_map(m, n_cap, s);
@@ -953,7 +952,7 @@
     gm_status st = check_slot(ctx, slot);
     if (st != GM_OK) return st;
     Slot &sl = ctx->slots[slot];
-    return fetch(ctx, slot, (const float4 *)sl.valid4, sl.last.n_valid, (float4 *)xyzw, capacity, n_out);
+    return fetch(ctx, slot, (const float4 *)sl.crop4, sl.last.n_valid, (float4 *)xyzw, capacity, n_out);
 }
 
 gm_status gm_get_normals(gm_ctx *ctx, uint32_t slot, float *nxyzc, uint32_t capacity, uint32_t *n_out)
@@ -961,7 +960,7 @@
     gm_status st = check_slot(ctx, slot);
     if (st != GM_OK) return st;
     Slot &sl = ctx->slots[slot];
-    return fetch(ctx, slot, (const float4 *)sl.vnorm4, sl.last.n_valid, (float4 *)nxyzc, capacity, n_out);
+    return fetch(ctx, slot, (const float4 *)sl.normals4, sl.last.n_valid, (float4 *)nxyzc, capacity, n_out);
 }
 
 gm_status gm_get_voxel_centroids(gm_ctx *ctx, uint32_t slot, float *xyzc, uint32_t capacity, uint32_t *n_out)
@@ -1065,9 +1064,9 @@
     sl.last.n_valid = m[1];
     sl.submitted = true;
     sl.complete = true;
-    st = fetch(ctx, 0, (const float4 *)sl.valid4, m[1], (float4 *)xyzw_out, capacity, n_out);
-    if (st != GM_OK) return st;
-    return fetch(ctx, 0, (const float4 *)sl.vnorm4, m[1], (float4 *)nxyzc_out, capacity, n_out);
+    st = fetch(ctx, 0, (const float4 *)sl.crop4, m[1], (float4 *)xyzw_out, capacity, n_out);
+    if (st != GM_OK) return st;
+    return fetch(ctx, 0, (const float4 *)sl.normals4, m[1], (float4 *)nxyzc_out, capacity, n_out);
 }
 
 gm_status gm_get_local_frame(gm_ctx *ctx, const float *nxyzc, uint32_t n, double wf, float eigenvalues[3],
@@ -1083,8 +1082,8 @@
     if (st != GM_OK) return st;
     st = reset_counters(ctx, sl);
     if (st != GM_OK) return st;
-    if (n) GM_HIP(ctx, hipMemcpyAsync(sl.vnorm4, nxyzc, (size_t)n * 16, hipMemcpyHostToDevice, sl.stream));
-    const uint32_t np = launch_scatter_partials(sl.vnorm4, nullptr, n, wf, sl, sl.stream);
+    if (n) GM_HIP(ctx, hipMemcpyAsync(sl.normals4, nxyzc, (size_t)n * 16, hipMemcpyHostToDevice, sl.stream));
+    const uint32_t np = launch_scatter_partials(sl.normals4, nullptr, n, wf, sl, sl.stream);
     launch_frame_finalize(sl.partials, np, 0, sl, sl.stream);
     GM_HIP(ctx, hipMemcpyAsync(sl.h_out, sl.d_out, sizeof(FrameOut), hipMemcpyDeviceToHost, sl.stream));
     GM_HIP(ctx, hipStreamSynchronize(sl.stream));
@@ -1095,6 +1094,38 @@
     return GM_OK;
 }
 
+gm_status gm_compact_valid_stage(gm_ctx *ctx, const float *xyzw, const float *nxyzc, uint32_t n, double wf, float *xyzw_out,
+                                 float *nxyzc_out, uint32_t capacity, uint32_t *n_out, double scatter6[6])
+{
+    Slot *slp;
+    gm_status st = begin_stage(ctx, slp);
+    if (st != GM_OK) return st;
+    if (n && (!xyzw || !nxyzc)) return fail(ctx, GM_ERR_INVALID_ARG, "rows pointer is NULL");
+    if (!(wf != 0.0)) return fail(ctx, GM_ERR_INVALID_ARG, "weighting factor must be non-zero");
+    Slot &sl = *slp;
+    st = ensure_capacity(ctx, sl, n ? n : 1u, 0, false);
+    if (st != GM_OK) return st;
+    st = reset_counters(ctx, sl);
+    if (st != GM_OK) return st;
+    if (n) {
+        GM_HIP(ctx, hipMemcpyAsync(sl.crop4, xyzw, (size_t)n * 16, hipMemcpyHostToDevice, sl.stream));
+        GM_HIP(ctx, hipMemcpyAsync(sl.normals4, nxyzc, (size_t)n * 16, hipMemcpyHostToDevice, sl.stream));
+    }
+    GM_HIP(ctx, hipMemcpyAsync(&sl.ctr->n_cropped, &n, 4, hipMemcpyHostToDevice, sl.stream));
+    uint32_t row_tile = kCpTile;
+    const uint32_t np = launch_compact_valid(sl, n, wf, sl.stream, &row_tile);
+    launch_frame_finalize(sl.tile_partials, np, row_tile, sl, sl.stream);
+    GM_HIP(ctx, hipMemcpyAsync(sl.h_out, sl.d_out, sizeof(FrameOut), hipMemcpyDeviceToHost, sl.stream));
+    GM_HIP(ctx, hipStreamSynchronize(sl.stream));
+    GM_HIP(ctx, hipGetLastError());
+    if (scatter6) for (int k = 0; k < 6; ++k) scatter6[k] = sl.h_out->scatter[k];
+    const uint32_t m = sl.h_out->ctr.n_valid;
+    if (m > n) return fail(ctx, GM_ERR_DEVICE, "gm_compact_valid_stage: more survivors than rows");
+    st = fetch(ctx, 0, (const float4 *)sl.crop4, m, (float4 *)xyzw_out, capacity, n_out);
+    if (st != GM_OK) return st;
+    return fetch(ctx, 0, (const float4 *)sl.normals4, m, (float4 *)nxyzc_out, capacity, n_out);
+}
+
 gm_status gm_voxel_grid(gm_ctx *ctx, const float *xyz, uint32_t n, double leaf, float *xyzc_out, uint32_t capacity,
                         uint32_t *n_out, uint32_t *status_flags)
 {
@@ -1115,9 +1146,9 @@
         stage[i] = make_float4(p[0], p[1], p[2], 0.f);
         for (int k = 0; k < 3; ++k) { mn = fminf(mn, p[k]); mx = fmaxf(mx, p[k]); }
     }
-    if (n) GM_HIP(ctx, hipMemcpyAsync(sl.valid4, stage, (size_t)n * 16, hipMemcpyHostToDevice, sl.stream));
+    if (n) GM_HIP(ctx, hipMemcpyAsync(sl.crop4, stage, (size_t)n * 16, hipMemcpyHostToDevice, sl.stream));
     GM_HIP(ctx, hipMemcpyAsync(&sl.ctr->vox_n, &n, 4, hipMemcpyHostToDevice, sl.stream));
-    launch_minmax(sl.valid4, nullptr, n, sl.ctr, sl.stream);
+    launch_minmax(sl.crop4, nullptr, n, sl.ctr, sl.stream);
     launch_voxel_grid(sl, n, (float)leaf, n ? voxel_key_bits(mn, mx, leaf) : 1, sl.stream);
     uint32_t V = 0, pass = 0;
     GM_HIP(ctx, hipMemcpyAsync(&V, &sl.ctr->n_voxels, 4, hipMemcpyDeviceToHost, sl.stream));
diff --git a/geometric_mapping_amd/csrc/gm_compact.hpp b/geometric_mapping_amd/csrc/gm_compact.hpp
--- a/geometric_mapping_amd/csrc/gm_compact.hpp
+++ b/geometric_mapping_amd/csrc/gm_compact.hpp
@@ -1,10 +1,15 @@
 #pragma once
+
+#include <type_traits>
 
 #include "gm_device.hpp"
 
 namespace gm {
 
 struct NoPayload {};
+
+template <class E, class = void> struct cp_in_place : std::false_type {};
+template <class E> struct cp_in_place<E, std::void_t<decltype(E::kInPlace)>> : std::bool_constant<E::kInPlace> {};
 
 #ifndef GM_CPTHREADS
 #define GM_CPTHREADS 512
@@ -30,6 +35,11 @@
 {
     static_assert(THREADS * ITEMS >= kCpMinTile, "tile below the size the record arrays are laid out for");
     constexpr uint64_t kAggregate = 1ull << 32, kInclusive = 2ull << 32;
+#ifdef GM_CP_DIAG_INPLACE_FENCE
+    constexpr int kPublish = cp_in_place<Emit>::value ? __ATOMIC_RELEASE : __ATOMIC_RELAXED;
+#else
+    constexpr int kPublish = __ATOMIC_RELAXED;
+#endif
     __shared__ uint32_t lb_sum[(THREADS / kWave)], lb_state[(THREADS / kWave)];
     __shared__ uint32_t wcnt[(THREADS / kWave)];
     const uint32_t n = n_ptr ? *n_ptr : n_host;
@@ -43,6 +53,12 @@
             if (total_out2) *total_out2 = 0;
         }
         return;
+    }
+    constexpr bool kInPlace = cp_in_place<Emit>::value;
+    uint32_t first_drop = 0xFFFFFFFFu;
+    if constexpr (kInPlace) {
+        first_drop = emit.first_drop();
+        if (first_drop == 0xFFFFFFFFu) return;
     }
     __shared__ uint32_t s_tile;
     if constexpr (Emit::kHasPrepare) emit.prepare();
@@ -59,6 +75,14 @@
     const uint32_t tile = s_tile;
     if (tile < ntiles) {
         const uint32_t base = tile * (uint32_t)(THREADS * ITEMS);
+        if constexpr (kInPlace) {
+            if (base + (uint32_t)(THREADS * ITEMS) <= first_drop) {
+                if (threadIdx.x == 0)
+                    __hip_atomic_store(&st.status[tile], tag | kInclusive | (uint64_t)(base + (uint32_t)(THREADS * ITEMS)),
+                                       kPublish, __HIP_MEMORY_SCOPE_AGENT);
+                return;
+            }
+        }
         uint64_t mask[ITEMS];
         typename Pred::Payload pay[ITEMS];
         const uint32_t wbase = base + (uint32_t)w * (uint32_t)(kWave * ITEMS);
@@ -71,6 +95,13 @@
             wtotal += (uint32_t)__popcll(mask[j]);
         }
         if (lane == 0) wcnt[w] = wtotal;
+        if constexpr (kInPlace) {
+#ifdef GM_CP_DIAG_INPLACE_FENCE
+            __builtin_amdgcn_fence(__ATOMIC_RELEASE, "agent");
+#else
+            asm volatile("s_waitcnt vmcnt(0)" ::: "memory");
+#endif
+        }
         __syncthreads();
         uint32_t total = 0, woff = 0;
 #pragma unroll
@@ -80,7 +111,7 @@
             total += c;
         }
         if (threadIdx.x == 0)
-            __hip_atomic_store(&st.status[tile], tag | (tile == 0 ? kInclusive : kAggregate) | total, __ATOMIC_RELAXED,
+            __hip_atomic_store(&st.status[tile], tag | (tile == 0 ? kInclusive : kAggregate) | total, kPublish,
                                __HIP_MEMORY_SCOPE_AGENT);
         uint32_t before = 0;
 #ifdef GM_CP_DIAG_NOLOOKBACK
@@ -118,9 +149,10 @@
                 top -= THREADS;
             }
             if (threadIdx.x == 0)
-                __hip_atomic_store(&st.status[tile], tag | kInclusive | (uint64_t)(before + total), __ATOMIC_RELAXED,
+                __hip_atomic_store(&st.status[tile], tag | kInclusive | (uint64_t)(before + total), kPublish,
                                    __HIP_MEMORY_SCOPE_AGENT);
         }
+        if constexpr (kInPlace) __builtin_amdgcn_fence(__ATOMIC_ACQUIRE, "agent");
         if (threadIdx.x == 0 && tile == ntiles - 1) {
 #ifdef GM_CP_DIAG_NOLOOKBACK
             if (total_out) *total_out = 0;
diff --git a/geometric_mapping_amd/csrc/gm_ext.hip b/geometric_mapping_amd/csrc/gm_ext.hip
--- a/geometric_mapping_amd/csrc/gm_ext.hip
+++ b/geometric_mapping_amd/csrc/gm_ext.hip
@@ -52,7 +52,7 @@
     gm_status st = prepare(ctx, slp, n, H);
     if (st != GM_OK) return st;
     Slot &sl = *slp;
-    st = upload_xyz(ctx, sl, xyz, n, sl.valid4);
+    st = upload_xyz(ctx, sl, xyz, n, sl.crop4);
     if (st != GM_OK) return st;
     st = upload_labels(ctx, sl, labels, n);
     if (st != GM_OK) return st;
@@ -68,7 +68,7 @@
         for (int k = 0; k < w; ++k) stage[8 * (size_t)h + k] = hyp[(size_t)w * h + k];
     float *dh = model == 0 ? sl.hyp_plane : sl.hyp_cyl;
     GMX_HIP(ctx, hipMemcpyAsync(dh, stage, (size_t)H * 32, hipMemcpyHostToDevice, sl.stream));
-    launch_score(model, sl.valid4, labels ? sl.labels : nullptr, want, nullptr, n, dh, sl.band, H, tau, sl.score_partial,
+    launch_score(model, sl.crop4, labels ? sl.labels : nullptr, want, nullptr, n, dh, sl.band, H, tau, sl.score_partial,
                  sl.cnt_plane, sl.best_plane, sl.stream);
     GMX_HIP(ctx, hipMemcpyAsync(counts, sl.cnt_plane, (size_t)H * 4, hipMemcpyDeviceToHost, sl.stream));
     GMX_HIP(ctx, hipStreamSynchronize(sl.stream));
@@ -116,7 +116,7 @@
     float *dh = model == 0 ? sl.hyp_plane : sl.hyp_cyl;
     GMX_HIP(ctx, hipMemcpyAsync(dh, rows.data(), rows.size() * 4, hipMemcpyHostToDevice, sl.stream));
     GMX_HIP(ctx, hipStreamSynchronize(sl.stream));
-    launch_score(model, sl.valid4, unlabelled_only ? sl.labels : nullptr, 0, &sl.ctr->n_valid, sl.last.n_valid, dh, sl.band,
+    launch_score(model, sl.crop4, unlabelled_only ? sl.labels : nullptr, 0, &sl.ctr->n_valid, sl.last.n_valid, dh, sl.band,
                  H, tau, nullptr, sl.cnt_plane, sl.score_partial + 600, sl.stream);
     GMX_HIP(ctx, hipMemcpyAsync(counts, sl.cnt_plane, (size_t)H * 4, hipMemcpyDeviceToHost, sl.stream));
     GMX_HIP(ctx, hipStreamSynchronize(sl.stream));
@@ -133,11 +133,11 @@
     gm_status st = prepare(ctx, slp, n, H);
     if (st != GM_OK) return st;
     Slot &sl = *slp;
-    st = upload_xyz(ctx, sl, xyz, n, sl.valid4);
-    if (st != GM_OK) return st;
-    st = upload_labels(ctx, sl, labels, n);
-    if (st != GM_OK) return st;
-    launch_plane_hypotheses(sl.valid4, labels ? sl.labels : nullptr, want, nullptr, n, seed, H, sl.hyp_plane, nullptr,
+    st = upload_xyz(ctx, sl, xyz, n, sl.crop4);
+    if (st != GM_OK) return st;
+    st = upload_labels(ctx, sl, labels, n);
+    if (st != GM_OK) return st;
+    launch_plane_hypotheses(sl.crop4, labels ? sl.labels : nullptr, want, nullptr, n, seed, H, sl.hyp_plane, nullptr,
                             sl.stream);
     if ((size_t)H * 32 > sl.raw_cap) {
         st = gm_ensure_capacity(ctx, sl, n, (size_t)H * 32, true);
@@ -161,12 +161,12 @@
     gm_status st = prepare(ctx, slp, n, H);
     if (st != GM_OK) return st;
     Slot &sl = *slp;
-    st = upload_xyz(ctx, sl, xyz, n, sl.valid4);
-    if (st != GM_OK) return st;
-    if (n) GMX_HIP(ctx, hipMemcpyAsync(sl.vnorm4, nxyzc, (size_t)n * 16, hipMemcpyHostToDevice, sl.stream));
-    st = upload_labels(ctx, sl, labels, n);
-    if (st != GM_OK) return st;
-    launch_cylinder_hypotheses(sl.valid4, sl.vnorm4, labels ? sl.labels : nullptr, want, nullptr, n, seed, H, sl.hyp_cyl,
+    st = upload_xyz(ctx, sl, xyz, n, sl.crop4);
+    if (st != GM_OK) return st;
+    if (n) GMX_HIP(ctx, hipMemcpyAsync(sl.normals4, nxyzc, (size_t)n * 16, hipMemcpyHostToDevice, sl.stream));
+    st = upload_labels(ctx, sl, labels, n);
+    if (st != GM_OK) return st;
+    launch_cylinder_hypotheses(sl.crop4, sl.normals4, labels ? sl.labels : nullptr, want, nullptr, n, seed, H, sl.hyp_cyl,
                                nullptr, nullptr, 0.0, sl.stream);
     if ((size_t)H * 32 > sl.raw_cap) {
         st = gm_ensure_capacity(ctx, sl, n, (size_t)H * 32, true);
@@ -190,12 +190,12 @@
     gm_status st = prepare(ctx, slp, n, 1);
     if (st != GM_OK) return st;
     Slot &sl = *slp;
-    st = upload_xyz(ctx, sl, xyz, n, sl.valid4);
-    if (st != GM_OK) return st;
-    if (n && nxyzc) GMX_HIP(ctx, hipMemcpyAsync(sl.vnorm4, nxyzc, (size_t)n * 16, hipMemcpyHostToDevice, sl.stream));
-    st = upload_labels(ctx, sl, labels, n);
-    if (st != GM_OK) return st;
-    launch_segment_moments(sl.valid4, nxyzc ? sl.vnorm4 : nullptr, labels ? sl.labels : nullptr, label, nullptr, n,
+    st = upload_xyz(ctx, sl, xyz, n, sl.crop4);
+    if (st != GM_OK) return st;
+    if (n && nxyzc) GMX_HIP(ctx, hipMemcpyAsync(sl.normals4, nxyzc, (size_t)n * 16, hipMemcpyHostToDevice, sl.stream));
+    st = upload_labels(ctx, sl, labels, n);
+    if (st != GM_OK) return st;
+    launch_segment_moments(sl.crop4, nxyzc ? sl.normals4 : nullptr, labels ? sl.labels : nullptr, label, nullptr, n,
                            sl.mom_partial, sl.mom_plane, sl.stream);
     GMX_HIP(ctx, hipMemcpyAsync(mom16, sl.mom_plane, 16 * sizeof(double), hipMemcpyDeviceToHost, sl.stream));
     GMX_HIP(ctx, hipStreamSynchronize(sl.stream));
@@ -212,11 +212,11 @@
     gm_status st = prepare(ctx, slp, m, 1);
     if (st != GM_OK) return st;
     Slot &sl = *slp;
-    st = upload_xyz(ctx, sl, xyz, n, sl.valid4);
+    st = upload_xyz(ctx, sl, xyz, n, sl.crop4);
     if (st != GM_OK) return st;
     st = upload_xyz(ctx, sl, queries, nq, sl.vox4);
     if (st != GM_OK) return st;
-    launch_nearest(sl.valid4, nullptr, n, sl.vox4, nullptr, nq, sl.nn_best, sl.vox_nn, sl.stream);
+    launch_nearest(sl.crop4, nullptr, n, sl.vox4, nullptr, nq, sl.nn_best, sl.vox_nn, sl.stream);
     if (nq) GMX_HIP(ctx, hipMemcpyAsync(idx_out, sl.vox_nn, (size_t)nq * 4, hipMemcpyDeviceToHost, sl.stream));
     GMX_HIP(ctx, hipStreamSynchronize(sl.stream));
     GMX_HIP(ctx, hipGetLastError());
@@ -287,7 +287,7 @@
     gm_status st = prepare(ctx, slp, n, 1);
     if (st != GM_OK) return st;
     Slot &sl = *slp;
-    st = upload_xyz(ctx, sl, xyz, n, sl.valid4);
+    st = upload_xyz(ctx, sl, xyz, n, sl.crop4);
     if (st != GM_OK) return st;
     st = upload_labels(ctx, sl, labels, n);
     if (st != GM_OK) return st;
@@ -296,7 +296,7 @@
     GMX_HIP(ctx, hipMemcpyAsync(sl.fit_init, row, sizeof(row), hipMemcpyHostToDevice, sl.stream));
     if (n) GMX_HIP(ctx, hipMemsetAsync(sl.inl_mask, 0, n, sl.stream));
     CylFitArgs a;
-    a.pts = sl.valid4; a.labels = labels ? sl.labels : nullptr; a.out = sl.inl_mask;
+    a.pts = sl.crop4; a.labels = labels ? sl.labels : nullptr; a.out = sl.inl_mask;
     a.want = want; a.want2 = want; a.mask_mode = 1;
     a.n_ptr = nullptr; a.n_host = n;
     a.init = sl.fit_init; a.best = nullptr;
@@ -412,7 +412,7 @@
     if (st != GM_OK) return st;
     st = gm_ensure_surface(ctx, sl);
     if (st != GM_OK) return st;
-    st = upload_xyz(ctx, sl, xyz, n, sl.valid4);
+    st = upload_xyz(ctx, sl, xyz, n, sl.crop4);
     if (st != GM_OK) return st;
     st = upload_labels(ctx, sl, labels, n);
     if (st != GM_OK) return st;
@@ -424,7 +424,7 @@
     GMX_HIP(ctx, hipMemcpyAsync(sl.surf_fit, &f, sizeof(f), hipMemcpyHostToDevice, sl.stream));
     GMX_HIP(ctx, hipMemcpyAsync(sl.surf_prm + 1, &d, sizeof(d), hipMemcpyHostToDevice, sl.stream));
     SurfArgs a;
-    a.pts = sl.valid4; a.labels = labels ? sl.labels : nullptr; a.n_ptr = nullptr; a.n_host = n;
+    a.pts = sl.crop4; a.labels = labels ? sl.labels : nullptr; a.n_ptr = nullptr; a.n_host = n;
     a.fit = sl.surf_fit; a.prm = sl.surf_prm + 1;
     a.table = sl.surf_table; a.cells = sl.surf_cells; a.info = sl.surf_info; a.res = sl.surf_res; a.cell = sl.surf_cell;
     launch_surface_map(a, n, sl.stream);
diff --git a/geometric_mapping_amd/csrc/gm_group.hip b/geometric_mapping_amd/csrc/gm_group.hip
--- a/geometric_mapping_amd/csrc/gm_group.hip
+++ b/geometric_mapping_amd/csrc/gm_group.hip
@@ -688,9 +688,9 @@
                 const uint32_t nq = V - q0 < sl.cap ? V - q0 : sl.cap;
                 if (hipMemcpyAsync(sl.vox4, &G.vox_cen[(size_t)q0 * 4], (size_t)nq * 16, hipMemcpyHostToDevice, sl.stream) != hipSuccess)
                     return gfail(grp, GM_ERR_DEVICE, "gm_group: upload of the merged centroids failed");
-                launch_nearest(sl.valid4, &sl.ctr->n_valid, sl.cap, sl.vox4, nullptr, nq, sl.nn_best, sl.vox_nn, sl.stream, sl.vnorm4, sl.vox_nrm4);
+                launch_nearest(sl.crop4, &sl.ctr->n_valid, sl.cap, sl.vox4, nullptr, nq, sl.nn_best, sl.vox_nn, sl.stream, sl.normals4, sl.vox_nrm4);
                 hipLaunchKernelGGL(k_gather_nearest, dim3((nq + 255) / 256), dim3(256), 0, sl.stream, (const int32_t *)sl.vox_nn, nq,
-                                   (const float4 *)sl.valid4, sl.spts4);
+                                   (const float4 *)sl.crop4, sl.spts4);
                 keys.resize(nq); nrm.resize((size_t)nq * 4); pts.resize((size_t)nq * 4);
                 if (hipMemcpyAsync(keys.data(), sl.nn_best, (size_t)nq * 8, hipMemcpyDeviceToHost, sl.stream) != hipSuccess ||
                     hipMemcpyAsync(nrm.data(), sl.vox_nrm4, (size_t)nq * 16, hipMemcpyDeviceToHost, sl.stream) != hipSuccess ||
@@ -803,10 +803,10 @@
             hipMemcpyAsync(f.rows8, rows8, sizeof(rows8), hipMemcpyHostToDevice, sl.stream) != hipSuccess ||
             hipMemcpyAsync(f.plane_best, &plane_best, sizeof(uint32_t), hipMemcpyHostToDevice, sl.stream) != hipSuccess)
             return fail_enqueued(GM_ERR_DEVICE, "gm_group_fit_cylinder: upload of the starting rows failed");
-        launch_label(0, sl.valid4, sl.labels, 0, 1, &sl.ctr->n_valid, sl.last.n_valid, f.rows8 + 8, nullptr, f.plane_best,
+        launch_label(0, sl.crop4, sl.labels, 0, 1, &sl.ctr->n_valid, sl.last.n_valid, f.rows8 + 8, nullptr, f.plane_best,
                      tau, 1, nullptr, nullptr, 0, sl.stream);
         CylFitArgs &a = args[r];
-        a.pts = sl.valid4; a.labels = sl.labels; a.out = sl.labels;
+        a.pts = sl.crop4; a.labels = sl.labels; a.out = sl.labels;
         a.want = 0; a.want2 = 0; a.mask_mode = 0;
         a.n_ptr = &sl.ctr->n_valid; a.n_host = sl.last.n_valid;
         a.init = f.rows8; a.best = nullptr;
diff --git a/geometric_mapping_amd/csrc/gm_internal.hpp b/geometric_mapping_amd/csrc/gm_internal.hpp
--- a/geometric_mapping_amd/csrc/gm_internal.hpp
+++ b/geometric_mapping_amd/csrc/gm_internal.hpp
@@ -43,8 +43,6 @@
     uint32_t *skeys = nullptr;
     DevArray<float4> normals4;
     DevArray<int32_t> counts;
-    DevArray<float4> valid4;
-    DevArray<float4> vnorm4;
     DevArray<uint2> tiles;
     uint32_t tiles_cap = 0;
     uint32_t tile_seg = 0;
@@ -174,7 +172,7 @@
 uint32_t max_tiles(uint32_t n_cap, const GridParams &g);
 uint32_t tile_cutter_blocks(uint32_t n_cap);
 uint32_t launch_compact_valid(Slot &sl, uint32_t n_cap, double weightingFactor, hipStream_t s, uint32_t *row_tile = nullptr);
-uint32_t launch_scatter_partials(const float4 *vnorm4, const uint32_t *n_ptr, uint32_t n_cap, double wf, Slot &sl,
+uint32_t launch_scatter_partials(const float4 *nrm4, const uint32_t *n_ptr, uint32_t n_cap, double wf, Slot &sl,
                                  hipStream_t s);
 void launch_rows_to_host(const float4 *src, float4 *dst_mapped, const uint32_t *begin_enc, const uint32_t *end_ptr, hipStream_t s);
 void launch_frame_finalize(const double *partials, uint32_t n_partials, uint32_t row_tile, Slot &sl, hipStream_t s);
diff --git a/geometric_mapping_amd/csrc/gm_wall.hip b/geometric_mapping_amd/csrc/gm_wall.hip
--- a/geometric_mapping_amd/csrc/gm_wall.hip
+++ b/geometric_mapping_amd/csrc/gm_wall.hip
@@ -307,9 +307,9 @@
     gm_status upload(const float *xyz, const uint8_t *labels, WallArgs &w)
     {
         gm_ctx *ctx = map->ctx;
-        GMW_OK(gm_upload_xyz(ctx, *sl, xyz, n, sl->valid4));
+        GMW_OK(gm_upload_xyz(ctx, *sl, xyz, n, sl->crop4));
         if (labels && n) GMW_HIP(ctx, hipMemcpyAsync(sl->labels, labels, n, hipMemcpyHostToDevice, sl->stream));
-        w.pts = sl->valid4;
+        w.pts = sl->crop4;
         w.labels = labels ? sl->labels : nullptr;
         w.n_ptr = nullptr;
         w.n_host = n;
@@ -726,7 +726,7 @@
     WallArgs w;
     GMW_OK(add_frame_args(map, pose, add_info, w));
     if (hipSetDevice(ctx->device) != hipSuccess) return gm_fail(ctx, GM_ERR_DEVICE, "hipSetDevice failed");
-    w.pts = sl.valid4;
+    w.pts = sl.crop4;
     w.labels = (ctx->cfg.flags & GM_CFG_RANSAC_PLANE) ? sl.labels : nullptr;
     w.n_ptr = &sl.ctr->n_valid;
     w.n_host = sl.n_in;
@@ -1155,7 +1155,7 @@
     ScanState scan;
     GMW_OK(check_prepare(map, slot, n_cap, sl.stream, scan));
     GMW_OK(check_wait_adds(map, slot, sl.stream));
-    a.w.pts = sl.valid4;
+    a.w.pts = sl.crop4;
     a.w.labels = (ctx->cfg.flags & GM_CFG_RANSAC_PLANE) ? sl.labels : nullptr;
     a.w.n_ptr = &sl.ctr->n_valid;
     a.w.n_host = sl.n_in;
diff --git a/geometric_mapping_amd/csrc/k_frame.hip b/geometric_mapping_amd/csrc/k_frame.hip
--- a/geometric_mapping_amd/csrc/k_frame.hip
+++ b/geometric_mapping_amd/csrc/k_frame.hip
@@ -3,19 +3,31 @@
 
 namespace gm {
 
-struct ValidPred {
-    const float4 *__restrict__ normals4;
-    uint32_t *__restrict__ first_drop_enc;
-    typedef float4 Payload;
+struct MoveRow { float4 nrm, row; };
+struct MovePred {
+    const float4 *normals4;
+    const float4 *crop4;
+    typedef MoveRow Payload;
     __device__ __forceinline__ bool operator()(uint32_t i, Payload &p) const
     {
-        p = normals4[i];
-        const bool ok = finite3(p.x, p.y, p.z);
-        if (!ok) {
-            const uint32_t enc = 0xFFFFFFFFu - i;
-            if (*first_drop_enc < enc) atomicMax(first_drop_enc, enc);
-        }
-        return ok;
+        p.nrm = normals4[i];
+        p.row = crop4[i];
+        return finite3(p.nrm.x, p.nrm.y, p.nrm.z);
+    }
+};
+struct MoveEmit {
+    static constexpr bool kHasFinish = false, kHasPrepare = false, kInPlace = true;
+    float4 *crop4;
+    float4 *normals4;
+    const uint32_t *__restrict__ first_drop_enc;
+    __device__ __forceinline__ uint32_t first_drop() const
+    {
+        const uint32_t e = *first_drop_enc;
+        return e ? 0xFFFFFFFFu - e : 0xFFFFFFFFu;
+    }
+    __device__ __forceinline__ void operator()(uint32_t src, uint32_t dst, const MoveRow &p)
+    {
+        if (dst != src) { crop4[dst] = p.row; normals4[dst] = p.nrm; }
     }
 };
 
@@ -64,27 +76,49 @@
     }
 }
 
-struct ValidEmit {
-    static constexpr bool kHasFinish = true, kHasPrepare = false;
-    const float4 *__restrict__ crop4;
-    float4 *__restrict__ valid4;
-    float4 *__restrict__ vnorm4;
-    double k_wf;
-    double *__restrict__ partials;
-    double m[6];
-    __device__ __forceinline__ void operator()(uint32_t src, uint32_t dst, const float4 &v)
-    {
-        valid4[dst] = crop4[src];
-        vnorm4[dst] = v;
-        scatter_term(v, k_wf, m);
-    }
-    __device__ __forceinline__ void finish(uint32_t tile)
-    {
-        scatter_row_store(m, partials + (size_t)tile * 6);
-#pragma unroll
-        for (int k = 0; k < 6; ++k) m[k] = 0;
-    }
-};
+template <int THREADS, int ITEMS>
+__global__ __launch_bounds__(THREADS) void k_valid_scan(const float4 *__restrict__ normals4, const uint32_t *__restrict__ n_ptr,
+                                                        double k_wf ,
+                                                        double *__restrict__ partials ,
+                                                        DevCounters *__restrict__ ctr)
+{
+    __shared__ uint32_t wcnt[THREADS / kWave];
+    const uint32_t n = *n_ptr;
+    const uint32_t tile = blockIdx.x, base = tile * (uint32_t)(THREADS * ITEMS);
+    if (base >= n) return;
+    const int w = threadIdx.x / kWave, lane = lane_id();
+    const uint32_t wbase = base + (uint32_t)w * (uint32_t)(kWave * ITEMS);
+    float4 v[ITEMS];
+#pragma unroll
+    for (int j = 0; j < ITEMS; ++j) {
+        const uint32_t i = wbase + j * kWave + lane;
+        if (i < n) v[j] = normals4[i];
+    }
+    double m[6] = {0, 0, 0, 0, 0, 0};
+    uint32_t cnt = 0;
+#pragma unroll
+    for (int j = 0; j < ITEMS; ++j) {
+        const uint32_t i = wbase + j * kWave + lane;
+        if (i < n) {
+            if (finite3(v[j].x, v[j].y, v[j].z)) {
+                scatter_term(v[j], k_wf, m);
+                ++cnt;
+            } else {
+                const uint32_t enc = 0xFFFFFFFFu - i;
+                if (ctr->first_drop_enc < enc) atomicMax(&ctr->first_drop_enc, enc);
+            }
+        }
+    }
+    cnt = wave_sum(cnt);
+    if (lane == 0) wcnt[w] = cnt;
+    scatter_row_store(m, partials + (size_t)tile * 6);
+    if (threadIdx.x == 0) {
+        uint32_t total = 0;
+#pragma unroll
+        for (int k = 0; k < THREADS / kWave; ++k) total += wcnt[k];
+        if (total) { atomicAdd(&ctr->n_valid, total); atomicAdd(&ctr->vox_n, total); }
+    }
+}
 
 __global__ __launch_bounds__(256) void k_minmax(const float4 *__restrict__ pts, const uint32_t *__restrict__ n_ptr,
                                                 uint32_t n_host, DevCounters *__restrict__ ctr)
@@ -136,23 +170,36 @@
     int th = 512, it = 8;
     if (e) sscanf(e, "%dx%d", &th, &it);
     else if (n_cap > 2000000u) { th = 1024; it = 8; }
-    const bool big = th == 1024 && it == 8;
-    const uint32_t tile = big ? 8192u : (uint32_t)kCpTile;
+    const bool big = th == 1024 && it == 8, small = th == 256 && it == 8;
+    const uint32_t tile = big ? 8192u : (small ? (uint32_t)kCpMinTile : (uint32_t)kCpTile);
     if (row_tile) *row_tile = tile;
     const uint32_t nb = (n_cap + tile - 1) / tile;
     if (nb == 0) return 0;
-    ValidPred pred{sl.normals4, &sl.ctr->first_drop_enc};
-    ValidEmit emit{sl.crop4, sl.valid4, sl.vnorm4, .001 / wf, sl.tile_partials, {0, 0, 0, 0, 0, 0}};
-    if (big)
-        hipLaunchKernelGGL((k_compact<ValidPred, ValidEmit, 1024, 8>), dim3(nb), dim3(1024), 0, s, pred, emit,
-                           (const uint32_t *)&sl.ctr->n_cropped, 0u, next_scan(sl), &sl.ctr->n_valid, &sl.ctr->vox_n);
-    else
-        hipLaunchKernelGGL((k_compact<ValidPred, ValidEmit>), dim3(nb), dim3(kCpThreads), 0, s, pred, emit,
-                           (const uint32_t *)&sl.ctr->n_cropped, 0u, next_scan(sl), &sl.ctr->n_valid, &sl.ctr->vox_n);
+    const uint32_t *n_ptr = &sl.ctr->n_cropped;
+    const float4 *nrm = sl.normals4;
+    double *rows = sl.tile_partials;
+    DevCounters *ctr = sl.ctr;
+    const double k_wf = .001 / wf;
+    MovePred pred{sl.normals4, sl.crop4};
+    MoveEmit emit{sl.crop4, sl.normals4, &sl.ctr->first_drop_enc};
+    uint32_t *const none = nullptr;
+    if (big) {
+        hipLaunchKernelGGL((k_valid_scan<1024, 8>), dim3(nb), dim3(1024), 0, s, nrm, n_ptr, k_wf, rows, ctr);
+        hipLaunchKernelGGL((k_compact<MovePred, MoveEmit, 1024, 8>), dim3(nb), dim3(1024), 0, s, pred, emit, n_ptr, 0u,
+                           next_scan(sl), none, none);
+    } else if (small) {
+        hipLaunchKernelGGL((k_valid_scan<256, 8>), dim3(nb), dim3(256), 0, s, nrm, n_ptr, k_wf, rows, ctr);
+        hipLaunchKernelGGL((k_compact<MovePred, MoveEmit, 256, 8>), dim3(nb), dim3(256), 0, s, pred, emit, n_ptr, 0u,
+                           next_scan(sl), none, none);
+    } else {
+        hipLaunchKernelGGL((k_valid_scan<kCpThreads, kCpItems>), dim3(nb), dim3(kCpThreads), 0, s, nrm, n_ptr, k_wf, rows, ctr);
+        hipLaunchKernelGGL((k_compact<MovePred, MoveEmit>), dim3(nb), dim3(kCpThreads), 0, s, pred, emit, n_ptr, 0u,
+                           next_scan(sl), none, none);
+    }
     return nb;
 }
 
-__global__ __launch_bounds__(256) void k_scatter_partials(const float4 *__restrict__ vnorm4,
+__global__ __launch_bounds__(256) void k_scatter_partials(const float4 *__restrict__ nrm4,
                                                           const uint32_t *__restrict__ n_ptr, uint32_t n_host,
                                                           double k_wf ,
                                                           double *__restrict__ partials)
@@ -160,7 +207,7 @@
     const uint32_t n = n_ptr ? *n_ptr : n_host;
     double m[6] = {0, 0, 0, 0, 0, 0};
     for (uint32_t i = blockIdx.x * blockDim.x + threadIdx.x; i < n; i += gridDim.x * blockDim.x)
-        scatter_term(vnorm4[i], k_wf, m);
+        scatter_term(nrm4[i], k_wf, m);
     scatter_row_store(m, partials + (size_t)blockIdx.x * 6);
 }
 
@@ -173,14 +220,14 @@
     frame_finalize_block(partials, nblocks, ctr, voxp, out, red, row_tile);
 }
 
-uint32_t launch_scatter_partials(const float4 *vnorm4, const uint32_t *n_ptr, uint32_t n_cap, double wf, Slot &sl,
+uint32_t launch_scatter_partials(const float4 *nrm4, const uint32_t *n_ptr, uint32_t n_cap, double wf, Slot &sl,
                                  hipStream_t s)
 {
     uint32_t nb = (n_cap + 4095) / 4096;
     if (nb < 64u) nb = (n_cap + 255) / 256 < 64u ? (n_cap + 255) / 256 : 64u;
     if (nb > (uint32_t)kScatterBlocks) nb = kScatterBlocks;
     if (nb == 0) nb = 1;
-    hipLaunchKernelGGL(k_scatter_partials, dim3(nb), dim3(256), 0, s, vnorm4, n_ptr, n_cap, .001 / wf, sl.partials);
+    hipLaunchKernelGGL(k_scatter_partials, dim3(nb), dim3(256), 0, s, nrm4, n_ptr, n_cap, .001 / wf, sl.partials);
     return nb;
 }
 
diff --git a/geometric_mapping_amd/csrc/k_voxel.hip b/geometric_mapping_amd/csrc/k_voxel.hip
--- a/geometric_mapping_amd/csrc/k_voxel.hip
+++ b/geometric_mapping_amd/csrc/k_voxel.hip
@@ -115,7 +115,7 @@
     if (n_cap == 0) return;
     uint32_t gb = (n_cap + 255) / 256;
     if (gb > 2048) gb = 2048;
-    hipLaunchKernelGGL(k_voxel_keys, dim3(gb), dim3(256), 0, s, (const float4 *)sl.valid4, (const DevCounters *)sl.ctr,
+    hipLaunchKernelGGL(k_voxel_keys, dim3(gb), dim3(256), 0, s, (const float4 *)sl.crop4, (const DevCounters *)sl.ctr,
                        (const VoxelParams *)sl.voxp, sl.keys_a);
     const int where = launch_radix_sort(sl.keys_a, sl.vals_a, sl.keys_b, sl.vals_b, &sl.ctr->vox_n, n_cap, key_bits,
                                         sl, false, s);
@@ -125,7 +125,7 @@
     HeadEmit emit{sl.seg_start};
     hipLaunchKernelGGL((k_compact<HeadPred, HeadEmit>), dim3(compact_grid(n_cap)), dim3(kCpThreads), 0, s, pred, emit,
                        (const uint32_t *)&sl.ctr->vox_n, 0u, next_scan(sl), &sl.ctr->n_voxels, (uint32_t *)nullptr);
-    hipLaunchKernelGGL(k_voxel_centroids, dim3(gb), dim3(256), 0, s, (const float4 *)sl.valid4, perm,
+    hipLaunchKernelGGL(k_voxel_centroids, dim3(gb), dim3(256), 0, s, (const float4 *)sl.crop4, perm,
                        (const uint32_t *)sl.seg_start, (const DevCounters *)sl.ctr, sl.vox4);
 }
 
diff --git a/include/gm_hip.h b/include/gm_hip.h
--- a/include/gm_hip.h
+++ b/include/gm_hip.h
@@ -128,6 +128,10 @@
 
 gm_status gm_get_local_frame(gm_ctx *ctx, const float *nxyzc, uint32_t n, double weighting_factor,
                              float eigenvalues[3], float eigenvectors[9], double scatter6[6]);
+
+gm_status gm_compact_valid_stage(gm_ctx *ctx, const float *xyzw, const float *nxyzc, uint32_t n,
+                                 double weighting_factor, float *xyzw_out, float *nxyzc_out,
+                                 uint32_t capacity, uint32_t *n_out, double scatter6[6]);
 
 gm_status gm_voxel_grid(gm_ctx *ctx, const float *xyz, uint32_t n, double leaf,
                         float *xyzc_out, uint32_t capacity, uint32_t *n_out, uint32_t *status_flags);
```

Result: faster. 5.189 billion points/s (median of 6 runs) (+1.9%).
